# facebookresearch/gtn

Hardware: AMD Instinct MI355X
Metric: CTC forward+backward losses/sec (T=1000, C=256) (higher is better)
Workload: dtype f32; 1 GPU; BASELINE config C3: compose(ctc_target, emissions)+forwardScore CTC loss fwd+bwd, T=1000, C=256, U=100, batch=512 per GPU; global_batch=512, parallelism=dp1 (utterance sharding, all_gather of losses), rccl_ranks=0

## Files before the change

gtn_amd/_capi.py:

```python
import ctypes as C
import os

c_graph = C.c_void_p
c_graph_p = C.POINTER(C.c_void_p)
c_i32_p = C.POINTER(C.c_int)
c_i64_p = C.POINTER(C.c_int64)
c_u8_p = C.POINTER(C.c_uint8)
c_f32_p = C.POINTER(C.c_float)

GRAD_FN = C.CFUNCTYPE(C.c_int, C.c_void_p, c_graph_p, C.c_int, c_graph)
CTX_FREE = C.CFUNCTYPE(None, C.c_void_p)

OK, INVALID_ARGUMENT, LOGIC_ERROR, RUNTIME_ERROR, OUT_OF_RANGE, DEVICE_ERROR = range(6)

_SIGS = {
    "gtnx_set_device": [C.c_int],
    "gtnx_get_device": [c_i32_p],
    "gtnx_set_stream": [C.c_void_p],
    "gtnx_compose_mode": [C.c_int, C.POINTER(C.c_int)],
    "gtnx_synchronize": [],
    "gtnx_memory_stats": [C.POINTER(C.c_uint64), C.POINTER(C.c_uint64)],
    "gtnx_empty_cache": [],
    "gtnx_reclaim": [],
    "gtnx_graph_create": [C.c_int, c_graph_p],
    "gtnx_graph_copy": [c_graph, c_graph_p],
    "gtnx_graph_deep_copy": [c_graph, c_graph_p],
    "gtnx_graph_destroy": [c_graph],
    "gtnx_graph_add_node": [c_graph, C.c_int, C.c_int, c_i32_p],
    "gtnx_graph_add_arc": [c_graph, C.c_int, C.c_int, C.c_int, C.c_int, C.c_float, c_i32_p],
    "gtnx_graph_add_nodes": [c_graph, C.c_int, C.c_void_p, C.c_void_p],
    "gtnx_graph_add_arcs": [c_graph, C.c_int, C.c_void_p, C.c_void_p, C.c_void_p, C.c_void_p, C.c_void_p],
    "gtnx_graph_num_nodes": [c_graph, c_i64_p],
    "gtnx_graph_num_arcs": [c_graph, c_i64_p],
    "gtnx_graph_num_start": [c_graph, c_i64_p],
    "gtnx_graph_num_accept": [c_graph, c_i64_p],
    "gtnx_graph_item": [c_graph, c_f32_p],
    "gtnx_graph_arc_sort": [c_graph, C.c_int],
    "gtnx_graph_mark_arc_sorted": [c_graph, C.c_int],
    "gtnx_graph_ilabel_sorted": [c_graph, c_i32_p],
    "gtnx_graph_olabel_sorted": [c_graph, c_i32_p],
    "gtnx_graph_weights": [c_graph, C.c_int, C.POINTER(c_f32_p)],
    "gtnx_graph_get_weights": [c_graph, C.c_void_p],
    "gtnx_graph_set_weights": [c_graph, C.c_void_p],
    "gtnx_graph_set_weights_device": [c_graph, C.c_void_p],
    "gtnx_graph_weights_device": [c_graph, C.POINTER(C.c_void_p)],
    "gtnx_graph_labels_to_array": [c_graph, C.c_void_p, C.c_int],
    "gtnx_graph_get_start": [c_graph, C.c_void_p],
    "gtnx_graph_get_accept": [c_graph, C.c_void_p],
    "gtnx_graph_is_start": [c_graph, C.c_int, c_i32_p],
    "gtnx_graph_is_accept": [c_graph, C.c_int, c_i32_p],
    "gtnx_graph_make_accept": [c_graph, C.c_int],
    "gtnx_graph_num_out": [c_graph, C.c_int, c_i64_p],
    "gtnx_graph_num_in": [c_graph, C.c_int, c_i64_p],
    "gtnx_graph_get_out": [c_graph, C.c_int, C.c_void_p],
    "gtnx_graph_get_in": [c_graph, C.c_int, C.c_void_p],
    "gtnx_graph_get_arcs": [c_graph, C.c_void_p, C.c_void_p, C.c_void_p, C.c_void_p],
    "gtnx_graph_get_arc": [c_graph, C.c_int, c_i32_p, c_i32_p, c_i32_p, c_i32_p, c_f32_p],
    "gtnx_graph_set_weight": [c_graph, C.c_int, C.c_float],
    "gtnx_graph_calc_grad": [c_graph, c_i32_p],
    "gtnx_graph_set_calc_grad": [c_graph, C.c_int],
    "gtnx_graph_is_grad_available": [c_graph, c_i32_p],
    "gtnx_graph_grad": [c_graph, c_graph_p],
    "gtnx_graph_zero_grad": [c_graph],
    "gtnx_graph_add_grad": [c_graph, C.c_void_p, C.c_int64],
    "gtnx_graph_add_grad_graph": [c_graph, c_graph],
    "gtnx_graph_id": [c_graph, C.POINTER(C.c_size_t)],
    "gtnx_graph_create_op": [c_graph_p, C.c_int, GRAD_FN, C.c_void_p, CTX_FREE, c_graph_p],
    "gtnx_graph_num_inputs": [c_graph, c_i64_p],
    "gtnx_graph_get_input": [c_graph, C.c_int, c_graph_p],
    "gtnx_graph_set_inputs": [c_graph, c_graph_p, C.c_int],
    "gtnx_graph_set_grad_fn": [c_graph, GRAD_FN, C.c_void_p, CTX_FREE],
    "gtnx_graph_has_grad_fn": [c_graph, c_i32_p],
    "gtnx_scalar_graph": [C.c_float, C.c_int, c_graph_p],
    "gtnx_linear_graph": [C.c_int, C.c_int, C.c_int, c_graph_p],
    "gtnx_linear_graph_n": [C.c_int, C.c_int, C.c_int, C.c_int, C.c_void_p, c_graph_p],
    "gtnx_linear_graph_borrow_n": [C.c_int, C.c_int, C.c_int, C.c_int, C.c_void_p, c_graph_p],
    "gtnx_negate": [c_graph, c_graph_p],
    "gtnx_add": [c_graph, c_graph, c_graph_p],
    "gtnx_subtract": [c_graph, c_graph, c_graph_p],
    "gtnx_compose": [c_graph, c_graph, c_graph_p],
    "gtnx_intersect": [c_graph, c_graph, c_graph_p],
    "gtnx_forward_score": [c_graph, c_graph_p],
    "gtnx_viterbi_score": [c_graph, c_graph_p],
    "gtnx_viterbi_path": [c_graph, c_graph_p],
    "gtnx_negate_n": [c_graph_p, C.c_int, c_graph_p],
    "gtnx_add_n": [c_graph_p, C.c_int, c_graph_p, C.c_int, c_graph_p],
    "gtnx_subtract_n": [c_graph_p, C.c_int, c_graph_p, C.c_int, c_graph_p],
    "gtnx_compose_n": [c_graph_p, C.c_int, c_graph_p, C.c_int, c_graph_p],
    "gtnx_intersect_n": [c_graph_p, C.c_int, c_graph_p, C.c_int, c_graph_p],
    "gtnx_forward_score_n": [c_graph_p, C.c_int, c_graph_p],
    "gtnx_viterbi_score_n": [c_graph_p, C.c_int, c_graph_p],
    "gtnx_viterbi_path_n": [c_graph_p, C.c_int, c_graph_p],
    "gtnx_items_n": [c_graph_p, C.c_int, C.c_void_p],
    "gtnx_items_device_n": [c_graph_p, C.c_int, C.c_void_p],
    "gtnx_grads_device_n": [c_graph_p, C.c_int, C.c_void_p, C.c_void_p],
    "gtnx_grads_bind_device_n": [c_graph_p, C.c_int, C.c_void_p, C.c_void_p],
    "gtnx_clone": [c_graph, C.c_int, c_graph_p],
    "gtnx_concat": [c_graph_p, C.c_int, c_graph_p],
    "gtnx_closure": [c_graph, c_graph_p],
    "gtnx_union": [c_graph_p, C.c_int, c_graph_p],
    "gtnx_batch_from_graphs": [c_graph_p, C.c_int, c_graph_p],
    "gtnx_batch_ctc_targets": [C.c_void_p, C.c_void_p, C.c_int, C.c_int, C.c_int, c_graph_p],
    "gtnx_batch_asg_force_align": [C.c_void_p, C.c_void_p, C.c_int, c_graph, C.c_int, c_graph_p],
    "gtnx_batch_linear": [C.c_int, C.c_int, C.c_int, C.c_int, C.c_void_p, C.c_int, c_graph_p],
    "gtnx_batch_linear_rows": [C.c_int, C.c_int, C.c_int, C.c_void_p, C.c_int, C.c_void_p, C.c_int, c_graph_p],
    "gtnx_batch_destroy": [c_graph],
    "gtnx_batch_size": [c_graph, c_i32_p],
    "gtnx_batch_get": [c_graph, C.c_int, c_graph_p],
    "gtnx_batch_negate": [c_graph, c_graph_p],
    "gtnx_batch_add": [c_graph, c_graph, c_graph_p],
    "gtnx_batch_subtract": [c_graph, c_graph, c_graph_p],
    "gtnx_batch_subtract_into": [c_graph, c_graph, C.c_void_p, c_graph_p],
    "gtnx_batch_compose": [c_graph, c_graph, c_graph_p],
    "gtnx_batch_intersect": [c_graph, c_graph, c_graph_p],
    "gtnx_batch_forward_score": [c_graph, c_graph_p],
    "gtnx_batch_viterbi_score": [c_graph, c_graph_p],
    "gtnx_batch_viterbi_path": [c_graph, c_graph_p],
    "gtnx_batch_viterbi_align": [c_graph, C.c_void_p, C.c_void_p, C.c_int64, C.c_void_p, C.c_void_p],
    "gtnx_batch_align_stats": [c_i64_p, c_i64_p],
    "gtnx_batch_viterbi_decode": [c_graph, c_graph, C.c_void_p, C.c_void_p, C.c_int64, C.c_void_p, C.c_void_p,
                                  C.c_void_p],
    "gtnx_batch_decode_stats": [c_i64_p, c_i64_p],
    "gtnx_batch_full_connect_stats": [c_i64_p, c_i64_p],
    "gtnx_batch_linear_decode": [c_graph, C.c_void_p, C.c_int, C.c_void_p, C.c_int64, C.c_void_p, C.c_void_p,
                                 C.c_void_p, C.c_void_p],
    "gtnx_batch_linear_decode_stats": [c_i64_p, c_i64_p],
    "gtnx_batch_ctc_sample": [c_graph, C.c_void_p, C.c_int, C.c_int, C.c_uint64, C.c_float, C.c_void_p, C.c_int64,
                              C.c_void_p, C.c_void_p, C.c_void_p],
    "gtnx_batch_ctc_sample_stats": [c_i64_p, c_i64_p],
    "gtnx_batch_ctc_beam_decode": [c_graph, C.c_void_p, C.c_int, C.c_int, C.c_int, C.c_int, C.c_void_p, C.c_int64,
                                   C.c_void_p, C.c_void_p],
    "gtnx_batch_ctc_beam_decode_lm": [c_graph, C.c_void_p, C.c_int, C.c_int, C.c_int, C.c_int, C.c_void_p, C.c_float,
                                      C.c_float, C.c_void_p, C.c_int64, C.c_void_p, C.c_void_p, C.c_void_p],
    "gtnx_batch_ctc_beam_decode_graph": [c_graph, C.c_void_p, C.c_int, C.c_int, C.c_int, C.c_int, C.c_void_p, C.c_float,
                                         C.c_float, C.c_void_p, C.c_int64, C.c_void_p, C.c_void_p, C.c_void_p],
    "gtnx_lm_graph_create": [c_graph, C.POINTER(C.c_void_p)],
    "gtnx_lm_graph_destroy": [C.c_void_p],
    "gtnx_lm_graph_walk": [C.c_void_p, C.c_int, C.c_int, c_f32_p, c_i32_p],
    "gtnx_lm_graph_info": [C.c_void_p, C.c_void_p],
    "gtnx_batch_ctc_beam_stats": [c_i64_p, c_i64_p],
    "gtnx_batch_linear_shape": [c_graph, c_i32_p, c_i32_p],
    "gtnx_batch_edit_distance": [C.c_void_p, C.c_int64, C.c_void_p, C.c_void_p, C.c_int64, C.c_void_p, C.c_int, C.c_int,
                                 C.c_int, C.c_int, C.c_void_p, C.c_void_p],
    "gtnx_batch_edit_distance_stats": [c_i64_p, c_i64_p],
    "gtnx_batch_ctc_score": [c_graph, C.c_void_p, C.c_int, C.c_void_p, C.c_int64, C.c_void_p, C.c_int, C.c_int, C.c_int,
                             C.c_void_p],
    "gtnx_batch_ctc_score_grad": [c_graph, C.c_void_p, C.c_int, C.c_void_p, C.c_int64, C.c_void_p, C.c_int, C.c_int,
                                  C.c_int, C.c_void_p, C.c_void_p],
    "gtnx_batch_ctc_score_stats": [c_i64_p, c_i64_p],
    "gtnx_batch_ctc_token_align": [c_graph, C.c_void_p, C.c_int, C.c_void_p, C.c_int64, C.c_void_p, C.c_int, C.c_int,
                                   C.c_int, C.c_void_p, C.c_void_p, C.c_void_p, C.c_void_p, C.c_int64, C.c_void_p,
                                   C.c_int64],
    "gtnx_batch_ctc_token_align_stats": [c_i64_p, c_i64_p],
    "gtnx_batch_asg_score": [c_graph, C.c_void_p, C.c_void_p, C.c_void_p, C.c_int64, C.c_void_p, C.c_int, C.c_int,
                             C.c_int, C.c_void_p],
    "gtnx_batch_asg_score_grad": [c_graph, C.c_void_p, C.c_void_p, C.c_void_p, C.c_int64, C.c_void_p, C.c_int, C.c_int,
                                  C.c_int, C.c_void_p, C.c_void_p, C.c_void_p],
    "gtnx_batch_asg_score_stats": [c_i64_p, c_i64_p],
    "gtnx_batch_asg_token_align": [c_graph, C.c_void_p, C.c_void_p, C.c_void_p, C.c_int64, C.c_void_p, C.c_int, C.c_int,
                                   C.c_int, C.c_void_p, C.c_void_p, C.c_void_p, C.c_void_p, C.c_int64, C.c_void_p,
                                   C.c_int64],
    "gtnx_batch_asg_token_align_stats": [c_i64_p, c_i64_p],
    "gtnx_batch_asg_beam_decode": [c_graph, C.c_void_p, C.c_void_p, C.c_int, C.c_int, C.c_int, C.c_void_p, C.c_int64,
                                   C.c_void_p, C.c_void_p],
    "gtnx_batch_asg_beam_decode_graph": [c_graph, C.c_void_p, C.c_void_p, C.c_int, C.c_int, C.c_int, C.c_void_p,
                                         C.c_float, C.c_float, C.c_void_p, C.c_int64, C.c_void_p, C.c_void_p, C.c_void_p],
    "gtnx_batch_asg_beam_stats": [c_i64_p, c_i64_p],
    "gtnx_batch_backward": [c_graph, C.c_int],
    "gtnx_batch_items": [c_graph, C.c_void_p],
    "gtnx_batch_items_device": [c_graph, C.c_void_p],
    "gtnx_batch_grads_bind_device": [c_graph, C.c_void_p, C.c_void_p],
    "gtnx_batch_grads_device": [c_graph, C.c_void_p, C.c_void_p],
    "gtnx_backward": [c_graph, C.c_int],
    "gtnx_backward_with_grad": [c_graph, c_graph, C.c_int],
    "gtnx_backward_n": [c_graph_p, C.c_int, C.c_int],
    "gtnx_equal": [c_graph, c_graph, c_i32_p],
    "gtnx_isomorphic": [c_graph, c_graph, c_i32_p],
    "gtnx_remove": [c_graph, C.c_int, C.c_int, c_graph_p],
    "gtnx_graph_load_buffer": [C.c_void_p, C.c_size_t, c_graph_p],
    "gtnx_parallel_enter": [],
    "gtnx_parallel_leave": [],
    "gtnx_parallel_flush": [],
    "gtnx_prof_enable": [C.c_int],
    "gtnx_prof_reset": [],
    "gtnx_prof_get": [C.c_char_p, C.POINTER(C.c_double), c_i64_p, C.POINTER(C.c_double)],
# ... 54 lines not shown
```

gtn_amd/criteria/criteria_capi.cpp:

```cpp
#include <cstring>
#include <string>

#include <map>
#include <mutex>

#include "asg_criterion.h"
#include "ctc_criterion.h"
#include "edit_distance.h"

#define GTN_EXPORT extern "C" __attribute__((visibility("default")))

namespace {
thread_local std::string g_err;

template <class F>
int guarded(F&& body) {
  try {
    body();
    return 0;
  } catch (const std::exception& e) {
    g_err = e.what();
    return -1;
  }
}
// ... 44 lines not shown
  return guarded([&] {
    gtn::criteria::ctcDecodeBatch(emissions, B, T, C, blank, frames, labels, scores, collapsed, starts, lengths);
  });
}

GTN_EXPORT int gtn_ctc_sample_n(const void* emissions, int B, int T, int C, int blank, const int* frames,
                                int num_samples, unsigned long long seed, float temperature, void* tokens,
                                void* lengths, void* logq, void* labels) {
  return guarded([&] {
    gtn::criteria::ctcSampleBatch(emissions, B, T, C, blank, frames, num_samples, seed, temperature, tokens, lengths,
                                  logq, labels);
  });
}

GTN_EXPORT int gtn_ctc_beam_decode_n(const void* emissions, int B, int T, int C, int blank, const int* frames,
                                     int beam_size, int cutoff_top_n, int nbest, void* tokens, void* lengths,
                                     void* scores) {
  return guarded([&] {
    gtn::criteria::ctcBeamDecodeBatch(emissions, B, T, C, blank, frames, beam_size, cutoff_top_n, nbest, tokens, lengths,
                                      scores);
  });
}

GTN_EXPORT int gtn_ctc_beam_decode_lm_n(const void* emissions, int B, int T, int C, int blank, const int* frames,
                                        int beam_size, int cutoff_top_n, int nbest, const void* lm, float lm_weight,
                                        float insertion_bonus, void* tokens, void* lengths, void* scores,
                                        void* am_scores) {
  return guarded([&] {
    gtn::criteria::ctcBeamDecodeBatch(emissions, B, T, C, blank, frames, beam_size, cutoff_top_n, nbest, lm, lm_weight,
                                      insertion_bonus, tokens, lengths, scores, am_scores);
  });
}

GTN_EXPORT int gtn_ctc_beam_decode_graph_n(const void* emissions, int B, int T, int C, int blank, const int* frames,
                                           int beam_size, int cutoff_top_n, int nbest, void* lm_graph, float lm_weight,
                                           float insertion_bonus, void* tokens, void* lengths, void* scores,
                                           void* am_scores) {
  return guarded([&] {
    gtn::criteria::ctcBeamDecodeBatch(emissions, B, T, C, blank, frames, beam_size, cutoff_top_n, nbest,
                                      static_cast<gtnx_lm_graph_t>(lm_graph), lm_weight, insertion_bonus, tokens, lengths,
                                      scores, am_scores);
  });
}

GTN_EXPORT int gtn_ctc_score_n(const void* emissions, int B, int T, int C, int blank, const int* frames,
                               const void* tokens, const void* lengths, int N, int L, int max_length, void* scores) {
  return guarded([&] {
    if (!scores) throw std::invalid_argument("gtn_ctc_score_n: null scores");
    gtn::criteria::ctcScoreBatch(emissions, B, T, C, blank, frames, tokens, lengths, N, L, max_length, scores);
  });
}

GTN_EXPORT int gtn_ctc_score_grad_n(const void* emissions, int B, int T, int C, int blank, const int* frames,
                                    const void* tokens, const void* lengths, int N, int L, int max_length,
                                    const void* weights, void* grad) {
  return guarded([&] {
    if (!weights || !grad) throw std::invalid_argument("gtn_ctc_score_grad_n: null weights or grad");
    gtn::criteria::ctcScoreBatch(emissions, B, T, C, blank, frames, tokens, lengths, N, L, max_length, nullptr, weights,
                                 grad);
  });
}

GTN_EXPORT int gtn_ctc_token_align_n(const void* emissions, int B, int T, int C, int blank, const int* frames,
                                     const void* tokens, const void* lengths, int N, int L, int max_length,
                                     void* scores, void* starts, void* ends, void* token_scores, void* frame_tokens) {
  return guarded([&] {
    gtn::criteria::ctcTokenAlignBatch(emissions, B, T, C, blank, frames, tokens, lengths, N, L, max_length, scores,
                                      starts, ends, token_scores, frame_tokens);
  });
}

GTN_EXPORT int gtn_edit_distance_n(const void* hyp, const void* hyp_lengths, const void* ref, const void* ref_lengths,
                                   int B, int N, int L, int U, void* dist, void* ops) {
  return guarded([&] { gtn::criteria::editDistanceBatch(hyp, hyp_lengths, ref, ref_lengths, B, N, L, U, dist, ops); });
}

GTN_EXPORT int gtn_ctc_loss_target_grads_n(const void* emissions, const int* targets, const int* lengths, int B, int T,
                                           int C, int blank, void* loss, void* grad, void* target_grad,
                                           const int64_t* target_grad_offsets) {
  return guarded([&] {
    gtn::Batch ctcs;
    gtn::criteria::ctcLossBatch(emissions, targets, lengths, B, T, C, blank, loss, grad, true, nullptr, &ctcs);
    if (target_grad) ctcs.gradsToDevice(target_grad, target_grad_offsets);
  });
}

namespace {
void asg_loss_impl(const void* emissions, const int* targets, const int* lengths, int B, int T, int N, const void* trans_w,
                   const int* frames, void* loss, void* grad_em, void* grad_trans) {
  if (frames)
    for (int b = 0; b < B; ++b)
      if (frames[b] < 1 || frames[b] > T) throw std::invalid_argument("[gtn_asg_loss_frames_n] a frame count outside 1 .. T");
  std::lock_guard<std::mutex> lk(g_loss_transitions.mu);
  gtn::Graph& trans = transitions_for(g_loss_transitions, N, grad_trans != nullptr);
  trans.setCalcGrad(grad_trans != nullptr);
  trans.zeroGrad();
  trans.setWeightsDevice(trans_w);
  gtn::criteria::asgLossBatch(emissions, targets, lengths, B, T, N, trans, loss, grad_em, frames);
  if (grad_trans) {
    gtnx_graph_t h = trans.handle();
    int64_t off = 0;
    gtn::detail::check(gtnx_grads_device_n(&h, 1, grad_trans, &off));
  }
}
}

GTN_EXPORT int gtn_asg_loss_n(const void* emissions, const int* targets, const int* lengths, int B, int T, int N,
                              const void* trans_w, void* loss, void* grad_em, void* grad_trans) {
  return guarded([&] { asg_loss_impl(emissions, targets, lengths, B, T, N, trans_w, nullptr, loss, grad_em, grad_trans); });
}

GTN_EXPORT int gtn_asg_loss_frames_n(const void* emissions, const int* targets, const int* lengths, int B, int T, int N,
                                     const void* trans_w, const int* frames, void* loss, void* grad_em,
                                     void* grad_trans) {
  return guarded([&] {
    if (!frames) throw std::invalid_argument("[gtn_asg_loss_frames_n] null frame counts");
    asg_loss_impl(emissions, targets, lengths, B, T, N, trans_w, frames, loss, grad_em, grad_trans);
  });
}

GTN_EXPORT int gtn_asg_align_n(const void* emissions, const int* targets, const int* lengths, int B, int T, int N,
                               const void* trans_w, const int* frames, void* labels, void* tokens, void* scores) {
  return guarded([&] {
    std::lock_guard<std::mutex> lk(g_nograd_transitions.mu);
    gtn::Graph& trans = transitions_for(g_nograd_transitions, N, false);
    trans.setWeightsDevice(trans_w);
    gtn::criteria::asgAlignBatch(emissions, targets, lengths, B, T, N, trans, frames, labels, tokens, scores);
  });
}

GTN_EXPORT int gtn_asg_decode_n(const void* emissions, int B, int T, int N, const void* trans_w, const int* frames,
                                void* labels, void* scores, void* collapsed, void* lengths) {
  return guarded([&] {
    std::lock_guard<std::mutex> lk(g_nograd_transitions.mu);
    gtn::Graph& trans = transitions_for(g_nograd_transitions, N, false);
    trans.setWeightsDevice(trans_w);
    gtn::criteria::asgDecodeBatch(emissions, B, T, N, trans, frames, labels, scores, collapsed, lengths);
  });
}

GTN_EXPORT int gtn_asg_score_n(const void* emissions, int B, int T, int C, const void* table, const int* frames,
                               const void* tokens, const void* lengths, int N, int L, int max_length, void* scores) {
  return guarded([&] {
    if (!scores) throw std::invalid_argument("gtn_asg_score_n: null scores");
    gtn::criteria::asgScoreBatch(emissions, B, T, C, table, frames, tokens, lengths, N, L, max_length, scores);
  });
}

GTN_EXPORT int gtn_asg_beam_decode_n(const void* emissions, int B, int T, int C, const void* table, const int* frames,
                                     int beam_size, int cutoff_top_n, int nbest, void* tokens, void* lengths,
                                     void* scores) {
  return guarded([&] {
    gtn::criteria::asgBeamDecodeBatch(emissions, B, T, C, table, frames, beam_size, cutoff_top_n, nbest, tokens, lengths,
                                      scores);
  });
}

GTN_EXPORT int gtn_asg_beam_decode_graph_n(const void* emissions, int B, int T, int C, const void* table,
                                           const int* frames, int beam_size, int cutoff_top_n, int nbest, void* lm_graph,
                                           float lm_weight, float insertion_bonus, void* tokens, void* lengths,
                                           void* scores, void* am_scores) {
  return guarded([&] {
    gtn::criteria::asgBeamDecodeBatch(emissions, B, T, C, table, frames, beam_size, cutoff_top_n, nbest,
                                      static_cast<gtnx_lm_graph_t>(lm_graph), lm_weight, insertion_bonus, tokens, lengths,
                                      scores, am_scores);
  });
// ... 21 lines not shown
```

gtn_amd/criteria/ctc_criterion.h:

```cpp
#pragma once

#include <chrono>
#include <cstdint>
#include <stdexcept>
#include <vector>

#include "gtn/gtn.h"

namespace gtn {
namespace criteria {

inline Graph ctcTargetGraph(const std::vector<int>& target, int blank = 0, bool calcGrad = true) {
  const int L = 2 * (int)target.size() + 1;
  std::vector<uint8_t> st(L, 0), ac(L, 0);
  std::vector<int> src, dst, lab;
  src.reserve(3 * L);
  dst.reserve(3 * L);
  lab.reserve(3 * L);
  for (int l = 0; l < L; l++) {
    const int idx = (l - 1) / 2;
    st[l] = l == 0;
    ac[l] = l == L - 1 || l + 2 == L;
    const int label = l % 2 ? target[idx] : blank;
    src.push_back(l), dst.push_back(l), lab.push_back(label);
    if (l > 0) src.push_back(l - 1), dst.push_back(l), lab.push_back(label);
    if (l % 2 && l > 1 && label != target[idx - 1]) src.push_back(l - 2), dst.push_back(l), lab.push_back(label);
  }
  Graph ctc(calcGrad);
  detail::check(gtnx_graph_add_nodes(ctc.handle(), L, st.data(), ac.data()));
  detail::check(gtnx_graph_add_arcs(ctc.handle(), (int)src.size(), src.data(), dst.data(), lab.data(), lab.data(), nullptr));
  ctc.arcSort();
  return ctc;
}

struct CtcStepTimes {
  double build = 0, linear = 0, intersect = 0, forward = 0, backward = 0;
};

inline void ctcLossBatch(
    const void* emissions,
    const int* labels,
    const int* lengths,
    int B,
    int T,
    int C,
    int blank,
    void* lossDev,
    void* gradDev,
    bool targetGrad = true,
    CtcStepTimes* times = nullptr,
    Batch* targetsOut = nullptr,
    const int* frames = nullptr) {
  auto now = [] { return std::chrono::steady_clock::now(); };
  auto ms = [](auto a, auto b) { return std::chrono::duration<double, std::milli>(b - a).count(); };
  if (frames)
    for (int b = 0; b < B; ++b)
      if (frames[b] < 1 || frames[b] > T) throw std::invalid_argument("[ctcLossBatch] a frame count outside 1 .. T");
  auto t0 = now();
  Batch ctcs = Batch::ctcTargets(labels, lengths, B, blank, targetGrad);
  auto t1 = now();
  Batch ems = Batch::linear(B, T, C, emissions, gradDev != nullptr, true, frames);
  std::vector<int64_t> off(B);
  for (int b = 0; b < B; ++b) off[b] = (int64_t)b * T * C;
  if (gradDev) ems.bindGrads(gradDev, off.data());
  auto t2 = now();
  Batch comp = batched::intersect(ctcs, ems);
  auto t3 = now();
  Batch score = batched::forwardScore(comp);
  Batch norm = batched::forwardScore(ems);
  Batch losses = batched::subtract(norm, score, lossDev);
  auto t4 = now();
  if (gradDev) batched::backward(losses);
  auto t5 = now();
  if (times) *times = {ms(t0, t1), ms(t1, t2), ms(t2, t3), ms(t3, t4), ms(t4, t5)};
  losses.itemsToDevice(lossDev);
  if (gradDev) ems.gradsToDevice(gradDev, off.data());
  if (targetsOut) *targetsOut = std::move(ctcs);
}

inline void ctcLossBatch(
    const void* emissions,
    const std::vector<std::vector<int>>& targets,
    int T,
    int C,
    int blank,
    void* lossDev,
    void* gradDev,
    bool targetGrad = true,
    CtcStepTimes* times = nullptr) {
  std::vector<int> flat, len;
  for (auto& t : targets) {
    flat.insert(flat.end(), t.begin(), t.end());
    len.push_back((int)t.size());
  }
  ctcLossBatch(emissions, flat.data(), len.data(), (int)targets.size(), T, C, blank, lossDev, gradDev, targetGrad, times);
}

inline void ctcAlignBatch(
    const void* emissions,
    const int* targets,
    const int* lengths,
    int B,
    int T,
    int C,
    int blank,
    const int* frames,
    void* labels,
    void* tokens,
    void* scores) {
  Batch ctcs = Batch::ctcTargets(targets, lengths, B, blank, false);
  Batch ems = Batch::linear(B, T, C, emissions, false, true);
  Batch comp = batched::intersect(ctcs, ems);
  batched::viterbiAlign(comp, static_cast<int*>(labels), T, static_cast<int*>(tokens), static_cast<float*>(scores), frames);
}

inline void ctcDecodeBatch(
    const void* emissions,
    int B,
    int T,
    int C,
    int blank,
    const int* frames,
    void* labelsDev,
    void* scoresDev,
    void* collapsedDev,
    void* startsDev,
    void* lengthsDev) {
  Batch ems = Batch::linear(B, T, C, emissions, false, true);
  batched::linearDecode(ems, static_cast<int*>(labelsDev), T, static_cast<float*>(scoresDev), frames, blank,
                        static_cast<int*>(collapsedDev), static_cast<int*>(startsDev), static_cast<int*>(lengthsDev));
}

inline void ctcSampleBatch(
    const void* emissions,
    int B,
    int T,
    int C,
    int blank,
    const int* frames,
    int numSamples,
    uint64_t seed,
    float temperature,
    void* tokensDev,
    void* lengthsDev,
    void* logqDev,
    void* labelsDev) {
  Batch ems = Batch::linear(B, T, C, emissions, false, true);
  batched::ctcSample(ems, static_cast<int*>(tokensDev), T, static_cast<int*>(lengthsDev), static_cast<float*>(logqDev),
                     static_cast<int*>(labelsDev), blank, numSamples, seed, temperature, frames);
}

inline void ctcBeamDecodeBatch(
    const void* emissions,
    int B,
    int T,
    int C,
    int blank,
    const int* frames,
    int beamSize,
// ... 116 lines not shown
```

gtn_amd/csrc/band.hip:

```cpp
#include <hip/hip_runtime.h>

#include <algorithm>
#include <cstdlib>
#include <stdexcept>
#include <type_traits>

#include "kernels.h"

#ifdef GTNX_BAND_TIMING
__device__ long long g_band_timing[256];
#endif

namespace gtnx {
namespace {

constexpr float NEGF = -1.0e30f;
constexpr float DEADF = -1.0e29f;
constexpr float LOG2E = 1.44269504088896340736f;
constexpr double LN2 = 0.693147180559945309417;
constexpr int BW = 256;
constexpr int WG = 512;
constexpr int WGB = 768;
constexpr int NBE = 5;
constexpr int NBG = 7;
constexpr int NBGE = 8;
#ifndef GTNX_BWD_SPLIT
#define GTNX_BWD_SPLIT 0
#endif
#ifndef GTNX_FWD_COPY_DEPTH
#define GTNX_FWD_COPY_DEPTH 2
#endif
#ifndef GTNX_FWD_COPY_ROTATE
#define GTNX_FWD_COPY_ROTATE 1
#endif
#ifndef GTNX_FWD_DEPTH
#define GTNX_FWD_DEPTH 2
#endif

#ifdef GTNX_BAND_TIMING
#define GTNX_TM(slot)                 \
  do {                                \
    const long long now_ = clock64(); \
    tm_acc[slot] += now_ - tm_last;   \
    tm_last = now_;                   \
  } while (0)
#define GTNX_TM_INIT(base)                       \
  const int tm_base = base;                      \
  long long tm_acc[8] = {0, 0, 0, 0, 0, 0, 0, 0}; \
  long long tm_n = 0;                            \
  long long tm_last = clock64()
#define GTNX_TM_TICK() tm_n += 1
#define GTNX_TM_DUMP()                                                      \
  do {                                                                      \
    if (blockIdx.x == 0 && (threadIdx.x & 63) == 0) {                       \
      for (int i_ = 0; i_ < 7; ++i_) g_band_timing[tm_base + (threadIdx.x >> 6) * 7 + i_] += tm_acc[i_]; \
      if (threadIdx.x == 0) g_band_timing[tm_base + 127] += tm_n;           \
    }                                                                       \
  } while (0)
#else
#define GTNX_TM(slot) do { } while (0)
#define GTNX_TM_INIT(base) do { } while (0)
#define GTNX_TM_TICK() do { } while (0)
#define GTNX_TM_DUMP() do { } while (0)
#endif

__device__ __forceinline__ void lds_barrier() { asm volatile("s_waitcnt lgkmcnt(0)\n\ts_barrier" ::: "memory"); }
#ifdef GTNX_EXP_FAKE_MATH
__device__ __forceinline__ float ex2(float x) { return __builtin_fmaf(x, 0.001f, 1.0f); }
__device__ __forceinline__ float lg2(float x) { return __builtin_fmaf(x, 0.001f, -0.001f); }
#else
__device__ __forceinline__ float ex2(float x) { return __builtin_amdgcn_exp2f(x); }
__device__ __forceinline__ float lg2(float x) { return __builtin_amdgcn_logf(x); }
#endif

__device__ __forceinline__ void settle(float& x) { asm volatile("" : "+v"(x)); }
__device__ __forceinline__ void settle(int& x) { asm volatile("" : "+v"(x)); }
__device__ __forceinline__ float uniform(float x) {
  return __int_as_float(__builtin_amdgcn_readfirstlane(__float_as_int(x)));
}
__device__ __forceinline__ double uniform(double x) {
  const long long b = __double_as_longlong(x);
  const unsigned lo = __builtin_amdgcn_readfirstlane(unsigned(b)), hi = __builtin_amdgcn_readfirstlane(unsigned(b >> 32));
  return __longlong_as_double((long long)(((unsigned long long)hi << 32) | lo));
}

__device__ __forceinline__ float wave_shr1(float x, float fill) {
  return __int_as_float(__builtin_amdgcn_update_dpp(__float_as_int(fill), __float_as_int(x), 0x138, 0xf, 0xf, false));
}
__device__ __forceinline__ float wave_shl1(float x, float fill) {
  return __int_as_float(__builtin_amdgcn_update_dpp(__float_as_int(fill), __float_as_int(x), 0x130, 0xf, 0xf, false));
}
#define GTNX_DPP6(op)                                                         \
  "s_nop 1\n\t" op " %0, %0, %0 row_shr:1 row_mask:0xf bank_mask:0xf\n\t"     \
  "s_nop 1\n\t" op " %0, %0, %0 row_shr:2 row_mask:0xf bank_mask:0xf\n\t"     \
  "s_nop 1\n\t" op " %0, %0, %0 row_shr:4 row_mask:0xf bank_mask:0xf\n\t"     \
  "s_nop 1\n\t" op " %0, %0, %0 row_shr:8 row_mask:0xf bank_mask:0xf\n\t"     \
  "s_nop 1\n\t" op " %0, %0, %0 row_bcast:15 row_mask:0xa bank_mask:0xf\n\t"  \
  "s_nop 1\n\t" op " %0, %0, %0 row_bcast:31 row_mask:0xc bank_mask:0xf\n\t"  \
  "s_nop 1"
__device__ __forceinline__ float wave_max(float x) {
  asm volatile(GTNX_DPP6("v_max_f32_dpp") : "+v"(x));
  return __int_as_float(__builtin_amdgcn_readlane(__float_as_int(x), 63));
}
__device__ __forceinline__ float wave_sum63(float x) {
  asm volatile(GTNX_DPP6("v_add_f32_dpp") : "+v"(x));
  return x;
}
__device__ __forceinline__ float wave_sum(float x) {
  return __int_as_float(__builtin_amdgcn_readlane(__float_as_int(wave_sum63(x)), 63));
}
#define GTNX_DPP2(ctl)                                                  \
  "v_add_f32_dpp %0, %0, %0 " ctl "\n\tv_add_f32_dpp %1, %1, %1 " ctl "\n\ts_nop 0\n\t"
__device__ __forceinline__ void wave_sum63x2(float& a, float& b) {
  asm volatile("s_nop 1\n\t"
               GTNX_DPP2("row_shr:1 row_mask:0xf bank_mask:0xf")
               GTNX_DPP2("row_shr:2 row_mask:0xf bank_mask:0xf")
               GTNX_DPP2("row_shr:4 row_mask:0xf bank_mask:0xf")
               GTNX_DPP2("row_shr:8 row_mask:0xf bank_mask:0xf")
               GTNX_DPP2("row_bcast:15 row_mask:0xa bank_mask:0xf")
               GTNX_DPP2("row_bcast:31 row_mask:0xc bank_mask:0xf")
               : "+v"(a), "+v"(b));
}
__device__ __forceinline__ void row_sum15x2(float& a, float& b) {
  asm volatile("s_nop 1\n\t"
               GTNX_DPP2("row_shr:1 row_mask:0xf bank_mask:0xf")
               GTNX_DPP2("row_shr:2 row_mask:0xf bank_mask:0xf")
               GTNX_DPP2("row_shr:4 row_mask:0xf bank_mask:0xf")
               GTNX_DPP2("row_shr:8 row_mask:0xf bank_mask:0xf")
               : "+v"(a), "+v"(b));
}
#define GTNX_ROR4(op)                                                        \
  "s_nop 1\n\t" op " %0, %0, %0 row_ror:8 row_mask:0xf bank_mask:0xf\n\t"    \
  "s_nop 1\n\t" op " %0, %0, %0 row_ror:4 row_mask:0xf bank_mask:0xf\n\t"    \
  "s_nop 1\n\t" op " %0, %0, %0 row_ror:2 row_mask:0xf bank_mask:0xf\n\t"    \
  "s_nop 1\n\t" op " %0, %0, %0 row_ror:1 row_mask:0xf bank_mask:0xf\n\t"    \
  "s_nop 1"
__device__ __forceinline__ float row16_max(float x) {
  asm volatile(GTNX_ROR4("v_max_f32_dpp") : "+v"(x));
  return x;
}
__device__ __forceinline__ float row16_sum(float x) {
  asm volatile(GTNX_ROR4("v_add_f32_dpp") : "+v"(x));
  return x;
}
__device__ __forceinline__ float lse3(float x0, float x1, float x2) {
  const float mx = fmaxf(fmaxf(x0, x1), x2);
  const float md = __builtin_amdgcn_fmed3f(x0, x1, x2);
  const float mn = fminf(fminf(x0, x1), x2);
  return mx + lg2(1.0f + ex2(md - mx) + ex2(mn - mx));
}

template <int NPL>
struct NodeRegs {
  int lab[NPL];
  float wi[3][NPL];
  float wo[3][NPL];
  int ao[3][NPL];
  bool has_in[NPL];
  bool start[NPL], accept[NPL];
};
template <int NPL, bool WANT_OUT>
__device__ __forceinline__ void load_nodes(const BandPair& P, int m0, NodeRegs<NPL>& g) {
  const GTNX_G gtnx_i4* nodes = reinterpret_cast<const GTNX_G gtnx_i4*>(P.nodes);
#pragma unroll
  for (int j = 0; j < NPL; ++j) {
    const int m = m0 + j;
    g.lab[j] = 0;
    g.start[j] = g.accept[j] = g.has_in[j] = false;
#pragma unroll
    for (int k = 0; k < 3; ++k) {
      g.wi[k][j] = g.wo[k][j] = NEGF;
      g.ao[k][j] = -1;
    }
    if (m < P.N) {
      const gtnx_i4 q = nodes[m];
      g.lab[j] = q.x >= 0 ? q.x : 0;
      const uint8_t f = P.nflags[m];
      g.start[j] = (f & NF_START) != 0;
      g.accept[j] = (f & NF_ACCEPT) != 0;
      const int a[3] = {q.y, q.z, q.w};
#pragma unroll
      for (int k = 0; k < 3; ++k)
        if (a[k] >= 0) {
          g.has_in[j] = true;
          g.wi[k][j] = P.w ? fmaxf(P.w[a[k]] * LOG2E, NEGF) : 0.0f;
        }
    }
    if (WANT_OUT) {
#pragma unroll
      for (int k = 0; k < 3; ++k) {
        if (m + k < P.N) {
          const gtnx_i4 q = nodes[m + k];
          const int a = k == 0 ? q.y : (k == 1 ? q.z : q.w);
          if (a >= 0) {
            g.ao[k][j] = a;
            g.wo[k][j] = P.w ? fmaxf(P.w[a] * LOG2E, NEGF) : 0.0f;
          }
        }
      }
    }
  }
}

__device__ __forceinline__ float em2(float x) { return fmaxf(x * LOG2E, NEGF); }

__device__ __forceinline__ int row_of(int e, int W, float invW) {
  int r = int(float(e) * invW);
  if (r * W > e) --r;
  if ((r + 1) * W <= e) ++r;
  return r;
}

template <int NS, int LN = BW>
struct Stage {
  float v[NS];
  template <bool VEC>
  __device__ __forceinline__ void issue(const GTNX_G float* src, int cnt, int tid) {
    if (cnt <= 0) return;
#pragma unroll
    for (int i = 0; i < NS / 4; ++i) {
      if (i > 0 && 4 * i * LN >= cnt) break;
      const int e = min(4 * (i * LN + tid), cnt - 4);
      const gtnx_f4 q = *reinterpret_cast<const GTNX_G gtnx_f4*>(reinterpret_cast<const GTNX_G char*>(src) + unsigned(4 * e));
      v[4 * i] = q.x;
      v[4 * i + 1] = q.y;
      v[4 * i + 2] = q.z;
      v[4 * i + 3] = q.w;
    }
  }
  int off[NS / 4];
  __device__ __forceinline__ void init_offsets(int W, int stride, int K, int tid, bool reverse = true) {
    const float invW = 1.0f / float(W);
#pragma unroll
    for (int i = 0; i < NS / 4; ++i) {
      const int e = 4 * (i * LN + tid);
      const int r = row_of(min(e, 4096), W, invW);
      off[i] = (reverse ? K - 1 - r : r) * stride + (e - r * W);
    }
  }
  template <class F>
  __device__ __forceinline__ void each_vec(int cnt, int shift, int tid, F&& f) const {
#pragma unroll
    for (int i = 0; i < NS / 4; ++i) {
      if (i > 0 && 4 * i * LN >= cnt) break;
      if (4 * (i * LN + tid) < cnt) f(i, off[i] - shift, gtnx_f4{v[4 * i], v[4 * i + 1], v[4 * i + 2], v[4 * i + 3]});
    }
  }
  __device__ __forceinline__ void settle_all() {
#pragma unroll
    for (int i = 0; i < NS; ++i) asm volatile("" : "+v"(v[i]));
  }
  template <bool VEC, class F>
  __device__ __forceinline__ void each(int cnt, int W, int tid, F&& f) const {
    const float invW = 1.0f / float(W);
    if constexpr (VEC) {
#pragma unroll
      for (int i = 0; i < NS / 4; ++i) {
        if (i > 0 && 4 * i * LN >= cnt) break;
        const int e = 4 * (i * LN + tid);
        if (e < cnt) {
          const int r = row_of(e, W, invW);
          f(i, e, r, e - r * W, gtnx_f4{v[4 * i], v[4 * i + 1], v[4 * i + 2], v[4 * i + 3]});
        }
      }
    } else {
#pragma unroll
      for (int i = 0; i < NS / 4; ++i) {
        if (i > 0 && 4 * i * LN >= cnt) break;
        if (4 * (i * LN + tid) < cnt) {
          const int e = min(4 * (i * LN + tid), cnt - 4);
          const int r0 = row_of(e, W, invW), c0 = e - r0 * W;
#pragma unroll
          for (int k = 0; k < 4; ++k) {
            int r = r0, col = c0 + k;
            if (col >= W) {
              col -= W;
              ++r;
            }
            f(i, e + k, r, col, gtnx_f4{v[4 * i + k], 0.0f, 0.0f, 0.0f});
          }
        }
      }
    }
  }
};

struct BandLds {
  int CS;
  int o_ering, o_aring, o_oring, o_snode, o_misc, total;
};
__host__ __device__ inline BandLds band_lds(int C, int K, int NSmax, bool backward) {
  BandLds L;
  L.CS = C + 4;
  int o = 0;
  L.o_ering = o;
  o += (backward ? NBGE : NBE) * K * L.CS;
  o = (o + 3) & ~3;
  L.o_aring = o;
  o += backward ? NBE * K * NSmax : 0;
  o = (o + 3) & ~3;
  L.o_oring = o;
  o += backward ? max(NBG * K * NSmax, 2 * C) : 0;
  o = (o + 3) & ~3;
  L.o_snode = o;
  o += backward ? 512 : 0;
  L.o_misc = o;
  o += 160 + 32 + 8 + 2 * NBE * K * 4 + 40 * K + 8 + 512;
  L.total = o;
  return L;
}
struct BandMisc {
  double *offr, *red, *find, *aofr;
  float *bndr, *fin, *lsep;
};
template <int K>
__device__ __forceinline__ BandMisc band_misc(float* lds, const BandLds& L) {
  BandMisc m;
  m.offr = reinterpret_cast<double*>(lds + L.o_misc);
  m.red = m.offr + 80;
  m.find = m.red + 16;
  m.aofr = m.find + 4;
  m.bndr = lds + L.o_misc + 200 + 2 * NBE * K * 4;
  m.fin = m.bndr + 40 * K;
  m.lsep = m.fin + 8;
  return m;
}

__device__ __forceinline__ float wave_max_of(const float* v, int n) {
  float mx = v[0];
  for (int j = 1; j < n; ++j) mx = fmaxf(mx, v[j]);
  return wave_max(mx);
}

template <int NPL, bool UNIT, int K, bool VEC>
__global__ __launch_bounds__(WG) void band_forward_kernel(const BandPair* __restrict__ pairs, int NSmax) {
#define GTNX_BAND_PAIR pairs[blockIdx.x]
#include "band_forward_body.inc"
#undef GTNX_BAND_PAIR
}
template <int NPL, bool UNIT, int K, bool VEC>
__global__ __launch_bounds__(WG) void band_forward_one_kernel(BandPair one, int NSmax) {
#define GTNX_BAND_PAIR one
#include "band_forward_body.inc"
#undef GTNX_BAND_PAIR
}

__device__ __forceinline__ BandPair band_patched(BandPair P, const BandPatch& pt) {
  if (pt.on) {
    const int b = P.bidx;
    P.delta = pt.delta + b;
    P.delta_norm = pt.delta_norm ? pt.delta_norm + b : nullptr;
    P.rowlse = pt.rowlse ? pt.rowlse + int64_t(b) * pt.M : nullptr;
    P.norm = nullptr;
    P.em_copy = nullptr;
    P.grad_em = pt.grad_em ? pt.grad_em + int64_t(b) * pt.A : nullptr;
    P.grad_fixed = pt.grad_fixed ? pt.grad_fixed + P.goff : nullptr;
  }
  return P;
}
template <int NPL, bool UNIT, bool GRADG, int K, bool VEC, bool BIG>
__global__ __launch_bounds__(WGB, BIG ? 3 : 6) void band_backward_kernel(const BandPair* __restrict__ pairs, int NSmax, BandPatch patch) {
#define GTNX_BAND_PAIR band_patched(pairs[blockIdx.x], patch)
#include "band_backward_body.inc"
#undef GTNX_BAND_PAIR
}
template <int NPL, bool UNIT, bool GRADG, int K, bool VEC, bool BIG>
__global__ __launch_bounds__(WGB, BIG ? 3 : 6) void band_backward_one_kernel(BandPair one, int NSmax) {
#define GTNX_BAND_PAIR one
#include "band_backward_body.inc"
#undef GTNX_BAND_PAIR
}


__global__ __launch_bounds__(512) void ctc_targets_kernel(const CtcTargetArgs* __restrict__ args, int blank) {
  const CtcTargetArgs a = args[blockIdx.x];
  __shared__ __attribute__((aligned(16))) int tl[256 + 4];
  __shared__ __attribute__((aligned(16))) int tk[256 + 4];
  const int N = a.N, U = (N - 1) >> 1, m = threadIdx.x;
  if (m < 260) {
    const int v = m < U ? a.labels[m] : 0x7fffffff;
    tl[m] = v;
    tk[m] = (m > 0 && m < U && v != a.labels[m - 1]) ? 1 : 0;
  }
  __syncthreads();
  if (m >= N) return;
  const bool odd = (m & 1) != 0;
  const int my = odd ? tl[(m - 1) >> 1] : blank;
  const int skip = odd ? tk[(m - 1) >> 1] : 0;
  const int mi = (m - 1) >> 1;
  const int before = odd ? mi : (m >> 1);
  int rank = 0, skips = 0;
  for (int o = 0; o < U; o += 4) {
    const gtnx_i4 l4 = *reinterpret_cast<const gtnx_i4*>(tl + o), k4 = *reinterpret_cast<const gtnx_i4*>(tk + o);
    const int lo[4] = {l4.x, l4.y, l4.z, l4.w}, ko[4] = {k4.x, k4.y, k4.z, k4.w};
#pragma unroll
    for (int k = 0; k < 4; ++k) {
      const bool front = o + k < before;
      rank += (lo[k] < my || (lo[k] == my && front)) ? 1 : 0;
      skips += front ? ko[k] : 0;
    }
  }
  rank += blank < my ? U + 1 : (blank == my ? (m + 1) >> 1 : 0);
  const int base = (m > 0 ? 2 * m - 1 : 0) + skips;
  GTNX_G BandNode* nd = const_cast<GTNX_G BandNode*>(a.nodes);
  nd[m].lab = my;
  nd[m].aid[0] = base;
  nd[m].aid[1] = m > 0 ? base + 1 : -1;
  nd[m].aid[2] = skip ? base + 2 : -1;
  a.nflags[m] = uint8_t((m == 0 ? NF_START : 0) | (m + 2 >= N ? NF_ACCEPT : 0));
  a.snode[rank] = m;
  a.slab[rank] = my;
  if (m == N - 1 && a.n_arcs) a.n_arcs[0] = base + 1 + (m > 0 ? 1 : 0) + skip;
}

__global__ __launch_bounds__(512) void band_viterbi_kernel(const BandDecode* __restrict__ pairs) {
  const BandDecode P = pairs[blockIdx.x];
  const int T = P.T, C = P.C, N = P.N, NS = P.NS;
  extern __shared__ float lds[];
  const float NINF = -__builtin_inff();
  float* a0 = lds;
  float* a1 = lds + 516;
  float* stage = lds + 1032;
  const int m = threadIdx.x;
  const GTNX_G gtnx_i4* nodes = reinterpret_cast<const GTNX_G gtnx_i4*>(P.nodes);
  int lab = 0;
  float wi[3] = {NINF, NINF, NINF};
  bool accept = false, start = false;
  if (m < N) {
    const gtnx_i4 q = nodes[m];
    lab = q.x >= 0 ? q.x : 0;
    const int a[3] = {q.y, q.z, q.w};
#pragma unroll
    for (int k = 0; k < 3; ++k)
      if (a[k] >= 0) wi[k] = P.w ? P.w[a[k]] : 0.0f;
    const uint8_t f = P.nflags[m];
    start = (f & NF_START) != 0;
    accept = (f & NF_ACCEPT) != 0;
  }
  if (m < 2) a0[m] = a1[m] = NINF;
  a0[2 + m] = start ? 0.0f : NINF;
  a1[2 + m] = NINF;
  int tie = 0;
  const int R = max(1, min(64, P.stage_floats / C));
  float* cur = a0;
  float* nxt = a1;
  __syncthreads();
  for (int t0 = 0; t0 < T; t0 += R) {
    const int rows = min(R, T - t0);
    for (int e = threadIdx.x; e < rows * C; e += blockDim.x) stage[e] = P.em[int64_t(t0) * C + e];
    __syncthreads();
    for (int i = 0; i < rows; ++i) {
      const float e = stage[i * C + lab];
      const float c0 = cur[2 + m] + (wi[0] + e), c1 = cur[1 + m] + (wi[1] + e), c2 = cur[m] + (wi[2] + e);
      float best = c0;
      int k = 0;
      if (c1 > best) best = c1, k = 1;
      if (c2 > best) best = c2, k = 2;
      if (best > NINF && ((k != 0 && c0 == best) || (k != 1 && c1 == best) || (k != 2 && c2 == best))) tie = 1;
      if (m < NS) P.bp[int64_t(t0 + i) * NS + m] = uint8_t(best > NINF ? k : 3);
      nxt[2 + m] = m < N ? best : NINF;
      __syncthreads();
      float* sw = cur;
      cur = nxt;
      nxt = sw;
    }
  }
  __shared__ float red_v[8];
  __shared__ int red_m[8], s_best, s_tie;
  float v = accept ? cur[2 + m] : NINF;
  int bm = (m < N && accept && v > NINF) ? m : 1 << 30;
  const float wmx = wave_max(v);
  if (!(v == wmx)) bm = 1 << 30;
  int cnt = (bm != (1 << 30)) ? 1 : 0;
  for (int o = 32; o > 0; o >>= 1) {
    bm = min(bm, __shfl_xor(bm, o));
    cnt += __shfl_xor(cnt, o);
  }
  if ((threadIdx.x & 63) == 0) {
    red_v[threadIdx.x >> 6] = wmx;
    red_m[threadIdx.x >> 6] = bm;
  }
  if (cnt > 1) tie = 1;
  if (threadIdx.x == 0) s_tie = 0;
  __syncthreads();
  if (threadIdx.x == 0) {
    float bv = NINF;
    int bn = -1;
    for (int w = 0; w < 8; ++w) {
      if (red_m[w] == (1 << 30)) continue;
      if (red_v[w] > bv) bv = red_v[w], bn = red_m[w];
      else if (red_v[w] == bv && bv > NINF) s_tie = 1;
    }
    s_best = bn;
    P.score[0] = bv;
  }
// ... 505 lines not shown
```

gtn_amd/csrc/band_backward_body.inc:

```
  constexpr int RNk = K >= 4 ? 4 : K;
  constexpr int NP = K / RNk;
  const BandPair P = GTNX_BAND_PAIR;
  const int T = P.T, C = P.C, NS = P.NS;
  extern __shared__ float lds[];
  const BandLds L = band_lds(C, K, NSmax, true);
  float* ering = lds + L.o_ering;
  float* aring = lds + L.o_aring;
  float* oring = lds + L.o_oring;
  int* snode = reinterpret_cast<int*>(lds + L.o_snode);
  const BandMisc M = band_misc<K>(lds, L);
  float* lser = M.lsep;
  const int CS = L.CS;
  const int wv = __builtin_amdgcn_readfirstlane(threadIdx.x >> 6);
  const bool sweeper = wv < 4;
  const int l = threadIdx.x & 63;
  const int nblocks = (T + K - 1) / K;
  const int nticks = nblocks + 5;
  const GTNX_G double* ao = P.aoff;
  const double z2 = uniform(ao[0]);
  const bool dead = !(z2 > double(DEADF));
  const float ds = uniform(P.delta[0]);
  const bool want_em = P.grad_em != nullptr;
  GTNX_TM_INIT(128);
  constexpr bool SPLIT = !BIG && K >= 2 && GTNX_BWD_SPLIT;
// ... 28 lines not shown
  auto rowsum_do = [&](const RowSumRegs& R, int c, int cg , int r, auto steady_tag) -> float {
    constexpr bool STEADY = decltype(steady_tag)::value;
    if (!want_em || (K < 4 && r >= K)) return 0.0f;
    if constexpr (!STEADY) {
      if (r >= rows_of_k(c)) return 0.0f;
    }
    const bool dead_r = STEADY ? false : dead;
    const float* ob = oring + (cg * K + r) * NSmax;
    gtnx_f4 v[NPL];
#pragma unroll
    for (int q = 0; q < NPL; ++q) v[q] = *reinterpret_cast<const gtnx_f4*>(ob + min(256 * q + 4 * l, NSmax - 4));
    const float em_hot = ering[(ge_of(c) * K + r) * CS + max(P.hot, 0)];
    const float ls_hot = lser[cg * K + r];
    float all = (v[0].x * R.in[0] + v[0].y * R.in[0]) + (v[0].z * R.in[0] + v[0].w * R.in[0]);
    float hotp = (v[0].x * R.hot[0].x + v[0].y * R.hot[0].y) + (v[0].z * R.hot[0].z + v[0].w * R.hot[0].w);
#pragma unroll
    for (int q = 1; q < NPL; ++q) {
      all += (v[q].x * R.in[q] + v[q].y * R.in[q]) + (v[q].z * R.in[q] + v[q].w * R.in[q]);
      hotp += (v[q].x * R.hot[q].x + v[q].y * R.hot[q].y) + (v[q].z * R.hot[q].z + v[q].w * R.hot[q].w);
    }
    if (dead_r) all = hotp = 0.0f;
    wave_sum63x2(all, hotp);
    all = __int_as_float(__builtin_amdgcn_readlane(__float_as_int(all), 63));
    const bool have = all != 0.0f && !dead_r;
    const float f = have ? ds * __builtin_amdgcn_rcpf(all) : 1.0f;
    if (l == 63 && P.hot >= 0) {
      const float sm = dn_k * ex2(em_hot - ls_hot);
      P.grad_em[int64_t(T - 1 - c * K - r) * C + P.hot] = (dead_r ? 0.0f : hotp * f) + sm;
    }
    if (l == 0) rnorm_k[cg * K + r] = f;
    return have ? f : 0.0f;
  };
#ifndef GTNX_BWD_ROWSUM4
#define GTNX_BWD_ROWSUM4 1
#endif
  constexpr bool RS4 = !BIG && !SPLIT && K == 4 && NPL == 1 && GTNX_BWD_ROWSUM4;
  struct RowSum4Regs {
    float in;
    gtnx_f4 hot[4];
    int po;
    int eo, go;
  };
  auto rowsum4_init = [&](RowSum4Regs& R) {
    const int r = l >> 4, nb = 16 * (l & 15);
    R.in = nb < NSmax ? 1.0f : 0.0f;
    R.po = r * NSmax + min(nb, NSmax - 16);
#pragma unroll
    for (int k = 0; k < 4; ++k) {
      float hm[4];
#pragma unroll
      for (int e = 0; e < 4; ++e) {
        const int m = nb + 4 * k + e;
        int lab = -1;
        if (m < P.N) lab = P.nodes[m].lab;
        settle(lab);
        hm[e] = (P.hot >= 0 && lab == P.hot) ? 1.0f : 0.0f;
      }
      R.hot[k] = gtnx_f4{hm[0], hm[1], hm[2], hm[3]};
    }
    R.eo = r * CS + max(P.hot, 0);
    R.go = (K - 1 - r) * C + max(P.hot, 0);
  };
  auto rowsum4_do = [&](const RowSum4Regs& R, int c, int cg , auto steady_tag) {
    constexpr bool STEADY = decltype(steady_tag)::value;
    const int rows = STEADY ? K : rows_of_k(c);
    if (!want_em || rows <= 0) return;
    const bool dead_r = STEADY ? false : dead;
    typedef float f2v __attribute__((ext_vector_type(2)));
    const float* ob = oring + cg * K * NSmax + R.po;
    gtnx_f4 v[4];
#pragma unroll
    for (int k = 0; k < 4; ++k) v[k] = *reinterpret_cast<const gtnx_f4*>(ob + 4 * k);
    const float em_hot = ering[ge_of(c) * K * CS + R.eo];
    const float ls_hot = lser[cg * K + (l >> 4)];
    f2v a2 = f2v{v[0].x, v[0].y} + f2v{v[0].z, v[0].w};
    f2v h2 = f2v{v[0].x, v[0].y} * f2v{R.hot[0].x, R.hot[0].y};
    h2 = __builtin_elementwise_fma(f2v{v[0].z, v[0].w}, f2v{R.hot[0].z, R.hot[0].w}, h2);
#pragma unroll
    for (int k = 1; k < 4; ++k) {
      a2 += f2v{v[k].x, v[k].y} + f2v{v[k].z, v[k].w};
      h2 = __builtin_elementwise_fma(f2v{v[k].x, v[k].y}, f2v{R.hot[k].x, R.hot[k].y}, h2);
      h2 = __builtin_elementwise_fma(f2v{v[k].z, v[k].w}, f2v{R.hot[k].z, R.hot[k].w}, h2);
    }
    float all = (a2.x + a2.y) * R.in, hotp = h2.x + h2.y;
    if (dead_r) all = hotp = 0.0f;
    row_sum15x2(all, hotp);
    const bool have = all != 0.0f && !dead_r;
    const float f = have ? ds * __builtin_amdgcn_rcpf(all) : 1.0f;
    if ((l & 15) == 15 && (STEADY || (l >> 4) < rows)) {
      if (P.hot >= 0) {
        const float sm = dn_k * ex2(em_hot - ls_hot);
        const GTNX_G char* gb = reinterpret_cast<const GTNX_G char*>(P.grad_em + int64_t(T - c * K - K) * C);
        *reinterpret_cast<GTNX_G float*>(const_cast<GTNX_G char*>(gb) + unsigned(4 * R.go)) = (dead_r ? 0.0f : hotp * f) + sm;
      }
      rnorm_k[cg * K + (l >> 4)] = f;
    }
  };
  constexpr int NCS = 8 / K;
  struct DrainRegs {
    int s[NCS], e[NCS], n0[NCS], n1[NCS];
    float m0[NCS], m1[NCS];
    bool more_any;
  };
  auto drain_init = [&](DrainRegs& D, int hid) {
    const int* cls = reinterpret_cast<const int*>(oring);
#pragma unroll
    for (int q = 0; q < NCS; ++q) {
      const int cc = hid + q * BW;
      D.s[q] = D.e[q] = 0;
      if (cc < C && cc != P.hot) {
        D.s[q] = cls[cc];
        D.e[q] = cls[C + cc];
      }
      const int cnt = D.e[q] - D.s[q];
      D.n0[q] = cnt > 0 ? snode[D.s[q]] : 0;
      D.n1[q] = cnt > 1 ? snode[D.s[q] + 1] : 0;
      D.m0[q] = cnt > 0 ? 1.0f : 0.0f;
      D.m1[q] = cnt > 1 ? 1.0f : 0.0f;
    }
    D.more_any = false;
#pragma unroll
    for (int q = 0; q < NCS; ++q) D.more_any = D.more_any || __builtin_amdgcn_ballot_w64(D.e[q] - D.s[q] > 2) != 0;
  };
  auto drain_rows = [&](const DrainRegs& D, int hid, int c, int cg , auto full_tag, auto dead_tag, auto r0_tag, auto r1_tag) {
    constexpr bool FULL = decltype(full_tag)::value;
    constexpr bool DEADU = decltype(dead_tag)::value;
    constexpr int R0 = decltype(r0_tag)::value, R1 = decltype(r1_tag)::value;
    const int rows = FULL ? K : rows_of_k(c);
    const float* ob = oring + cg * K * NSmax;
    const float* eb = ering + ge_of(c) * K * CS;
    const float* lb = lser + cg * K;
    const float* fb = rnorm_k + cg * K;
    GTNX_G float* dst = P.grad_em + int64_t(T - 1 - c * K) * C;
#pragma unroll
    for (int q = 0; q < NCS; ++q) {
      if (q > 0 && q * BW >= C) break;
      const int cc = hid + q * BW;
      const bool mine = cc < C && cc != P.hot;
      float p0[K], p1[K], e[K], ls[K], f[K];
#pragma unroll
      for (int r = R0; r < R1; ++r) {
        if constexpr (!DEADU) {
          p0[r] = ob[r * NSmax + D.n0[q]];
          p1[r] = ob[r * NSmax + D.n1[q]];
        }
        e[r] = eb[r * CS + min(cc, C - 1)];
      }
      if constexpr (K == 4) {
        const gtnx_f4 l4 = *reinterpret_cast<const gtnx_f4*>(lb), f4 = *reinterpret_cast<const gtnx_f4*>(fb);
        ls[0] = l4.x, ls[1] = l4.y, ls[2] = l4.z, ls[3] = l4.w;
        f[0] = f4.x, f[1] = f4.y, f[2] = f4.z, f[3] = f4.w;
      } else {
#pragma unroll
        for (int r = R0; r < R1; ++r) {
          ls[r] = lb[r];
          f[r] = fb[r];
        }
      }
      float sum[K];
      if constexpr (!DEADU) {
#pragma unroll
      for (int r = R0; r < R1; ++r) sum[r] = p0[r] * D.m0[q] + p1[r] * D.m1[q];
      }
      if (!DEADU && D.more_any) {
        for (int i = D.s[q] + 2; i < D.e[q]; ++i) {
          const float* o = ob + snode[i];
#pragma unroll
// ... 509 lines not shown
```

gtn_amd/csrc/band_forward_body.inc:

```
#ifndef GTNX_FWD_SHIFT_ROWS
#define GTNX_FWD_SHIFT_ROWS 4
#endif
  constexpr int RNk = K >= GTNX_FWD_SHIFT_ROWS ? GTNX_FWD_SHIFT_ROWS : (K >= 4 ? 4 : K);
  constexpr int NP = K / RNk;
  constexpr int D = 8 / K > GTNX_FWD_DEPTH ? 8 / K : GTNX_FWD_DEPTH;
  const BandPair P = GTNX_BAND_PAIR;
  const int T = P.T, C = P.C, NS = P.NS;
  extern __shared__ float lds[];
  const BandLds L = band_lds(C, K, NSmax, false);
  float* ering = lds + L.o_ering;
  const BandMisc M = band_misc<K>(lds, L);
  const int CS = L.CS;
  const int wv = __builtin_amdgcn_readfirstlane(threadIdx.x >> 6);
  const bool sweeper = wv < 4;
  const int l = threadIdx.x & 63;
  const int nblocks = (T + K - 1) / K;
  const int nticks = nblocks + 3;
  GTNX_TM_INIT(0);

  if (sweeper) {
    __builtin_amdgcn_s_setprio(1);
    const int w = wv;
    const int m0 = threadIdx.x * NPL;
    NodeRegs<NPL> g;
// ... 87 lines not shown
              if (UNIT) {
                x0 = a[j];
                x1 = s1;
                x2 = s2 + g.wi[2][j];
              } else {
                x0 = a[j] + g.wi[0][j];
                x1 = s1 + g.wi[1][j];
                x2 = s2 + g.wi[2][j];
              }
              nw[j] = lse3(x0, x1, x2) + ev[i][j];
            }
            if ((i + 1) % RNk == 0) {
              const float mx = wave_max_of(nw, NPL);
              if (mx > DEADF) {
#pragma unroll
                for (int j = 0; j < NPL; ++j) nw[j] -= mx;
                off += double(mx);
              } else if (w > 0) {
                off = offp[(i + 1) / RNk];
              }
              if (l == 0) {
                const int p = (t0 + i + 1) / RNk;
                off_own[p & 15] = off;
                P.aoff[1 + p * 4 + w] = off;
              }
            }
#pragma unroll
            for (int j = 0; j < NPL; ++j) hist[i][j] = a[j] = nw[j];
          }
        }
        {
          const GTNX_G char* const brow = arow;
          arow += int64_t(NS) * 4 * rows;
#ifdef GTNX_EXP_NO_ALPHA_STORE
          if (writer && beta < 0) {
#else
          if (writer) {
#endif
#pragma unroll
            for (int i = 0; i < K; ++i)
              if (FULL || i < rows) {
                const GTNX_G char* ri = brow + int64_t(NS) * 4 * (i + 1);
#pragma unroll
                for (int j = 0; j < NPL; ++j) *reinterpret_cast<GTNX_G float*>(const_cast<GTNX_G char*>(ri) + (aoffb + 4u * j)) = hist[i][j];
              }
          }
        }
        if (NPL == 1 ? l >= 62 : l == 63) {
#pragma unroll
          for (int i = 0; i < K; ++i)
            if (FULL || i < rows) {
              float* bp = bnd_own + ((((beta & 3) * K + i + 1) & (4 * K - 1))) * 2;
              if (NPL == 1) {
                bp[63 - l] = hist[i][0];
              } else {
                bp[0] = hist[i][NPL - 1];
                bp[1] = hist[i][0];
              }
            }
        }
      };
      if (beta >= 0 && beta < nblocks) {
        if (beta * K + K <= T) block(std::true_type{});
        else block(std::false_type{});
      }
      GTNX_TM(5);
      lds_barrier();
      GTNX_TM(6);
      GTNX_TM_TICK();
    }
    float f = NEGF;
#pragma unroll
    for (int j = 0; j < NPL; ++j) f = fmaxf(f, g.accept[j] ? a[j] : NEGF);
    const float mx = wave_max(f);
    float s = 0.0f;
#pragma unroll
    for (int j = 0; j < NPL; ++j) s += g.accept[j] ? ex2(a[j] - mx) : 0.0f;
    s = wave_sum(s);
    if (l == 0) {
      M.fin[2 * w] = mx;
      M.fin[2 * w + 1] = s;
      M.find[w] = off;
    }
  } else {
    const int hid = threadIdx.x - BW;
    constexpr bool vec = VEC;
    const bool want_lse = P.norm != nullptr || P.rowlse != nullptr;
    Stage<8> st[D];
    auto rows_of = [&](int c) { return c < nblocks ? min(K, T - c * K) : 0; };
    auto issue = [&](Stage<8>& s, int c) { s.template issue<VEC>(P.em + int64_t(c) * K * C, rows_of(c) * C, hid); };
    GTNX_G float* const em_copy = P.em_copy;
    auto land = [&](const Stage<8>& s, int c, int c5 , auto copy_tag) {
      constexpr bool COPY = decltype(copy_tag)::value;
      float* base = ering + c5 * K * CS;
      GTNX_G float* cdst = em_copy + int64_t(c) * K * C;
      s.template each<VEC>(rows_of(c) * C, C, hid, [&](int, int e, int r, int col, gtnx_f4 q) {
        float* d = base + r * CS + col;
        if (vec) *reinterpret_cast<gtnx_f4*>(d) = gtnx_f4{em2(q.x), em2(q.y), em2(q.z), em2(q.w)};
        else d[0] = em2(q.x);
        if (COPY) {
          if (vec) __builtin_nontemporal_store(q, reinterpret_cast<GTNX_G gtnx_f4*>(cdst + e));
          else __builtin_nontemporal_store(q.x, cdst + e);
        }
      });
    };
    constexpr int LPR = BW / K, G16 = LPR / 16;
    const int EPL = (C + LPR - 1) / LPR;
    double normacc = 0.0;
    auto lse_a_n = [&](int c, int c5 , auto nconst) {
      constexpr int NE = decltype(nconst)::value;
      const int rows = rows_of(c), rr = hid / LPR, sub = hid - rr * LPR;
      if (rows <= 0) return;
      const float* e = ering + (c5 * K + min(rr, rows - 1)) * CS + sub * EPL;
      float x[NE];
      float m = NEGF;
      if (VEC && (EPL & 3) == 0) {
#pragma unroll
        for (int i = 0; i < NE; i += 4) {
          const bool in = i < EPL && sub * EPL + i < C;
          const gtnx_f4 q = in ? *reinterpret_cast<const gtnx_f4*>(e + i) : gtnx_f4{NEGF, NEGF, NEGF, NEGF};
          x[i] = q.x, x[i + 1] = q.y, x[i + 2] = q.z, x[i + 3] = q.w;
          m = fmaxf(fmaxf(m, fmaxf(q.x, q.y)), fmaxf(q.z, q.w));
        }
      } else {
#pragma unroll
        for (int i = 0; i < NE; ++i) {
          x[i] = (i < EPL && sub * EPL + i < C) ? e[i] : NEGF;
          m = fmaxf(m, x[i]);
        }
      }
      m = row16_max(m);
      float sum = 0.0f;
#pragma unroll
      for (int i = 0; i < NE; ++i) sum += (i < EPL) ? ex2(x[i] - m) : 0.0f;
      sum = row16_sum(sum);
      if ((hid & 15) == 0 && rr < rows) {
        float* p = M.lsep + (c & 1) * 256 + (rr * 8 + (sub >> 4)) * 2;
        p[0] = m;
        p[1] = sum;
      }
    };
    auto lse_a = [&](int c, int c5) {
      if (EPL <= 4) lse_a_n(c, c5, std::integral_constant<int, 4>{});
      else if (EPL <= 8) lse_a_n(c, c5, std::integral_constant<int, 8>{});
      else lse_a_n(c, c5, std::integral_constant<int, 16>{});
    };
    auto lse_b = [&](int c) {
      const int rows = rows_of(c);
      if (hid < rows) {
        const float* p = M.lsep + (c & 1) * 256 + hid * 16;
        float Mx = p[0];
#pragma unroll
        for (int k = 1; k < G16; ++k) Mx = fmaxf(Mx, p[2 * k]);
        float S = 0.0f;
#pragma unroll
        for (int k = 0; k < G16; ++k) S += p[2 * k + 1] * ex2(p[2 * k] - Mx);
        const float l2 = Mx + lg2(S);
        if (P.rowlse) P.rowlse[c * K + hid] = l2;
        normacc += double(l2);
      }
    };
    auto run = [&](auto copy_tag) {
      issue(st[0], 0);
      land(st[0], 0, 0, copy_tag);
#pragma unroll
      for (int c = 1; c <= D; ++c) issue(st[c % D], c);
// ... 87 lines not shown
```

gtn_amd/csrc/batch.cpp:

```cpp
#include "batch.h"

#include <algorithm>
#include <atomic>
#include <cstdlib>
#include <cstring>
#include <limits>
#include <unordered_map>
#include <unordered_set>

namespace gtnx {

namespace {

std::atomic<uint64_t> g_batch_seq{1};

struct CompMode {
  int old;
  CompMode() : old(compose_mode_hint(2)) {}
  ~CompMode() { compose_mode_hint(old); }
};

BatchP make_batch(Batch::Kind k, int n, bool cg) {
  auto b = std::make_shared<Batch>();
  b->kind = k;
// ... 362 lines not shown
  std::vector<uint8_t> st(size_t(L), 0), ac(size_t(L), 0);
  std::vector<int> src, dst, lab;
  src.reserve(size_t(3 * L));
  dst.reserve(size_t(3 * L));
  lab.reserve(size_t(3 * L));
  for (int l = 0; l < L; ++l) {
    const int idx = (l - 1) / 2;
    st[size_t(l)] = l == 0;
    ac[size_t(l)] = l == L - 1 || l + 2 == L;
    const int label = l % 2 ? t[idx] : blank;
    src.push_back(l), dst.push_back(l), lab.push_back(label);
    if (l > 0) src.push_back(l - 1), dst.push_back(l), lab.push_back(label);
    if (l % 2 && l > 1 && label != t[idx - 1]) src.push_back(l - 2), dst.push_back(l), lab.push_back(label);
  }
  Graph g(cg);
  g.add_nodes(L, st.data(), ac.data());
  g.add_arcs(int(src.size()), src.data(), dst.data(), lab.data(), lab.data(), nullptr);
  g.arc_sort(false);
  return g;
}
}

BatchP batch_ctc_targets(const int* labels, const int* lengths, int n, int blank, bool calc_grad) {
  GTNX_HOST_T("batch.ctc_targets");
  if (n < 0) throw_invalid("[gtnx_batch_ctc_targets] negative batch size");
  BatchP b = make_batch(Batch::CTC_TARGETS, n, calc_grad);
  b->blank = blank;
  b->lab_off.resize(size_t(n) + 1);
  b->lab_off[0] = 0;
  for (int i = 0; i < n; ++i) {
    if (lengths[i] < 0) throw_invalid("[gtnx_batch_ctc_targets] negative length");
    b->lab_off[size_t(i) + 1] = b->lab_off[size_t(i)] + lengths[i];
    b->max_nodes = std::max(b->max_nodes, 2 * lengths[i] + 1);
  }
  const size_t total = size_t(b->lab_off[size_t(n)]);
  b->labels.assign(labels, labels + total);
  int mn = blank;
  b->max_label = blank;
  for (size_t i = 0; i < total; ++i) {
    b->max_label = std::max(b->max_label, labels[i]);
    mn = std::min(mn, labels[i]);
  }
  if (mn < 0 || b->max_nodes > band_max_nodes() || n == 0) {
    std::vector<Graph> gs;
    gs.reserve(size_t(n));
    for (int i = 0; i < n; ++i)
      gs.push_back(ctc_target_graph_host(labels + b->lab_off[size_t(i)], lengths[i], blank, calc_grad));
    return batch_from_graphs(std::move(gs));
  }
  Runtime& rt = Runtime::get();
  const size_t lab_bytes = align_up(sizeof(int) * (total ? total : 1), 256);
  const size_t arg_bytes = align_up(sizeof(CtcTargetArgs) * size_t(n), 256);
  size_t bytes = lab_bytes + arg_bytes;
  b->rec_off.resize(size_t(n));
  for (int i = 0; i < n; ++i) {
    const size_t N = size_t(2 * lengths[i] + 1);
    b->rec_off[size_t(i)] = bytes;
    bytes += align_up(sizeof(BandNode) * N, 64) + align_up(N, 64) + 2 * align_up(4 * N, 64) + 64;
  }
  b->rec_mem = rt.alloc(bytes);
  PinnedMemP pin = rt.alloc_pinned(lab_bytes + arg_bytes);
  std::memcpy(pin->ptr, labels, sizeof(int) * total);
  CtcTargetArgs* args = reinterpret_cast<CtcTargetArgs*>(static_cast<char*>(pin->ptr) + lab_bytes);
  for (int i = 0; i < n; ++i) {
    const size_t N = size_t(2 * lengths[i] + 1);
    char* base = b->rec_mem->as<char>(b->rec_off[size_t(i)]);
    CtcTargetArgs& a = args[size_t(i)];
    a.labels = b->rec_mem->as<int>() + b->lab_off[size_t(i)];
    a.nodes = reinterpret_cast<BandNode*>(base);
    base += align_up(sizeof(BandNode) * N, 64);
    a.nflags = reinterpret_cast<uint8_t*>(base);
    base += align_up(N, 64);
    a.snode = reinterpret_cast<int*>(base);
    base += align_up(4 * N, 64);
    a.slab = reinterpret_cast<int*>(base);
    base += align_up(4 * N, 64);
    a.n_arcs = reinterpret_cast<int*>(base);
    a.N = int(N);
    a.pad = 0;
  }
  rt.h2d_pinned(b->rec_mem->ptr, pin->ptr, lab_bytes + arg_bytes);
  launch_ctc_targets(reinterpret_cast<const CtcTargetArgs*>(b->rec_mem->as<char>(lab_bytes)), n, blank, rt.stream());
  return b;
}


BatchP batch_asg_force_align(const int* labels, const int* lengths, int n, Graph& transitions, int n_labels) {
  if (n < 0) throw_invalid("[gtnx_batch_asg_force_align] negative batch size");
  if (transitions.num_nodes() != int64_t(n_labels) + 1 || transitions.num_arcs() != int64_t(n_labels) * (n_labels + 1))
    throw_invalid("[gtnx_batch_asg_force_align] the transitions graph must have the asgTransitions(N) layout");
  BatchP b = make_batch(Batch::CTC_TARGETS, n, transitions.calc_grad());
  b->fal = true;
  b->trans = transitions;
  b->trans_labels = n_labels;
  b->lab_off.resize(size_t(n) + 1);
  b->lab_off[0] = 0;
  int max_u = 0;
  for (int i = 0; i < n; ++i) {
    if (lengths[i] < 0) throw_invalid("[gtnx_batch_asg_force_align] negative length");
    b->lab_off[size_t(i) + 1] = b->lab_off[size_t(i)] + lengths[i];
    max_u = std::max(max_u, lengths[i]);
  }
  b->max_nodes = max_u + 1;
  const size_t total = size_t(b->lab_off[size_t(n)]);
  b->labels.assign(labels, labels + total);
  int mn = 0;
  for (size_t i = 0; i < total; ++i) {
    b->max_label = std::max(b->max_label, labels[i]);
    mn = std::min(mn, labels[i]);
  }
  if (mn < 0 || b->max_label >= n_labels || b->max_nodes > band_max_nodes() || n == 0) {
    b->kind = Batch::GRAPHS;
    batch_materialise(*b);
    return b;
  }
  Runtime& rt = Runtime::get();
  std::vector<Weights*> ws{transitions.w.get()};
  ensure_weights_device_batch(ws);
  size_t bytes = align_up(sizeof(int) * (total ? total : 1), 256);
  b->rec_off.resize(size_t(n));
  b->w_off.resize(size_t(n));
  b->map_off.resize(size_t(n));
  for (int i = 0; i < n; ++i) {
    const size_t N = size_t(lengths[i]) + 1, A = 2 * size_t(lengths[i]);
    b->rec_off[size_t(i)] = bytes;
    bytes += align_up(sizeof(BandNode) * N, 64) + align_up(N, 64) + 2 * align_up(4 * N, 64);
    b->w_off[size_t(i)] = bytes;
    bytes += align_up(4 * (A ? A : 1), 64);
    b->map_off[size_t(i)] = bytes;
    bytes += align_up(4 * (A ? A : 1), 64);
  }
  b->rec_mem = rt.alloc(bytes);
  {
    PinnedMemP pin = rt.alloc_pinned(sizeof(int) * (total ? total : 1));
    std::memcpy(pin->ptr, labels, sizeof(int) * total);
    rt.h2d_pinned(b->rec_mem->ptr, pin->ptr, sizeof(int) * total);
  }
  std::vector<AsgFalArgs> args;
  args.resize(size_t(n));
  for (int i = 0; i < n; ++i) {
    const size_t N = size_t(lengths[i]) + 1;
    char* base = b->rec_mem->as<char>(b->rec_off[size_t(i)]);
    AsgFalArgs& a = args[size_t(i)];
    a.labels = b->rec_mem->as<int>() + b->lab_off[size_t(i)];
    a.trans_w = transitions.w->dev;
    a.nodes = reinterpret_cast<BandNode*>(base);
    base += align_up(sizeof(BandNode) * N, 64);
    a.nflags = reinterpret_cast<uint8_t*>(base);
    base += align_up(N, 64);
    a.snode = reinterpret_cast<int*>(base);
    base += align_up(4 * N, 64);
    a.slab = reinterpret_cast<int*>(base);
    a.w = b->rec_mem->as<float>(b->w_off[size_t(i)]);
    a.arc_map = b->rec_mem->as<int>(b->map_off[size_t(i)]);
    a.U = lengths[i];
    a.pad = 0;
  }
  DevMemP d = upload_vec(args);
  launch_asg_fal_targets(d->as<AsgFalArgs>(), n, n_labels, rt.stream());
  auto op = std::make_shared<BFalOp>();
  op->seq = g_batch_seq.fetch_add(1);
  b->op = op;
  return b;
}

BatchP batch_linear(int n, int M, int C, bool calc_grad, const void* dev, bool borrow, const int* rows) {
// ... 782 lines not shown
```

gtn_amd/csrc/batch.h:

```cpp
#pragma once

#include <memory>
#include <vector>

#include "ops.h"

namespace gtnx {

struct Batch;
using BatchP = std::shared_ptr<Batch>;

struct BatchOp {
  uint64_t seq = 0;
  std::vector<BatchP> inputs;
  virtual void backward(Batch& out) = 0;
  virtual ~BatchOp() {}
};

struct Batch {
  enum Kind { GRAPHS, CTC_TARGETS, LINEAR, PRODUCT, SCALAR };
  Kind kind = GRAPHS;
  int n = 0;
  bool calc_grad = false;

  bool materialised = false;
  std::vector<Graph> graphs;
  bool leaf = false;
  struct Origin {
    std::shared_ptr<void> home;
    size_t begin, end;
  };
  std::vector<Origin> origins;
  void (*give_back)(const std::shared_ptr<void>& home, std::vector<Graph>* part) = nullptr;
  std::vector<float> host_vals;
  bool host_vals_valid = false;
  PinnedMemP host_pin;
  void* host_ev = nullptr;

  std::vector<int> labels, lab_off;
  int blank = 0;
  int max_label = -1, max_nodes = 0;
  DevMemP rec_mem;
  std::vector<size_t> rec_off;
  bool fal = false;
  Graph trans;
  int trans_labels = 0;
  std::vector<size_t> w_off, map_off;
  int M = 0, C = 0;
  DevMemP w_mem;
  float* w_dev = nullptr;
  std::shared_ptr<PendingCopy> w_pend;
  DevMemP nc_mem;
  float* nc_norm = nullptr;
  float* nc_rowlse = nullptr;
  std::vector<int> rows;
  int64_t pad_floats = 0;
  DevMemP pad_mem;
  int rows_of(int b) const { return rows.empty() ? M : rows[size_t(b)]; }
  BatchP fixed, chain;
  bool chain_first = false, intersect = false;
  bool wide = false;
  bool full = false;
  DevMemP v_mem;
  float* v_dev = nullptr;

  std::shared_ptr<BatchOp> op;
  bool tape_cleared = false;
  DevMemP g_mem;
  float* g_dev = nullptr;
  std::vector<int64_t> g_off;
  DevMemP dest_mem;
  float* dest = nullptr;

  int64_t elem_size(int b) const;
  ~Batch();
};

BatchP batch_from_graphs(std::vector<Graph> gs);
BatchP batch_ctc_targets(const int* labels, const int* lengths, int n, int blank, bool calc_grad);
BatchP batch_asg_force_align(const int* labels, const int* lengths, int n, Graph& transitions, int n_labels);
BatchP batch_linear(int n, int M, int C, bool calc_grad, const void* dev, bool borrow, const int* rows = nullptr);
BatchP batch_compose(const BatchP& a, const BatchP& b, bool intersect);
BatchP batch_shortest_distance(const BatchP& x, bool tropical);
void batch_full_connect_stats(int64_t* fast, int64_t* fallback);
BatchP batch_viterbi_path(const BatchP& x);
void batch_viterbi_align(const BatchP& x, const int* frames, int* labels_dev, int64_t row_stride, int* tokens_dev,
                         float* scores_dev);
void batch_align_stats(int64_t* fast, int64_t* fallback);
void batch_viterbi_decode(const BatchP& ems, Graph& transitions, const int* frames, int* labels_dev, int64_t row_stride,
                          float* scores_dev, int* collapsed_dev, int* lengths_dev);
void batch_decode_stats(int64_t* fast, int64_t* fallback);
void batch_linear_decode(const BatchP& ems, const int* frames, int blank, int* labels_dev, int64_t row_stride,
                         float* scores_dev, int* collapsed_dev, int* starts_dev, int* lengths_dev);
void batch_linear_decode_stats(int64_t* fast, int64_t* fallback);
void batch_ctc_sample(const BatchP& ems, const int* frames, int blank, int N, uint64_t seed, float temperature,
                      int* tokens_dev, int64_t row_stride, int* lengths_dev, float* logq_dev, int* labels_dev);
void batch_ctc_sample_stats(int64_t* calls, int64_t* utterances);
void batch_ctc_beam_decode(const BatchP& ems, const int* frames, int blank, int beam, int topn, int nbest,
                           int* tokens_dev, int64_t row_stride, int* lengths_dev, float* scores_dev);
struct CtcBeamLm {
  const float* table_dev;
  float weight, bonus;
  float* am_scores_dev;
  const void* graph = nullptr;
};
void batch_ctc_beam_decode(const BatchP& ems, const int* frames, int blank, int beam, int topn, int nbest,
                           const CtcBeamLm* lm, int* tokens_dev, int64_t row_stride, int* lengths_dev, float* scores_dev);
void batch_ctc_beam_stats(int64_t* calls, int64_t* utterances);
void batch_asg_beam_decode(const BatchP& ems, const int* frames, const float* table_dev, int beam, int topn, int nbest,
                           int* tokens_dev, int64_t row_stride, int* lengths_dev, float* scores_dev);
struct AsgBeamLm {
  const void* graph;
  float weight, bonus;
  float* am_scores_dev;
};
void batch_asg_beam_decode(const BatchP& ems, const int* frames, const float* table_dev, int beam, int topn, int nbest,
                           const AsgBeamLm* lm, int* tokens_dev, int64_t row_stride, int* lengths_dev,
                           float* scores_dev);
void batch_asg_beam_stats(int64_t* calls, int64_t* utterances);
void batch_edit_distance(const int* hyp_dev, int64_t hyp_stride, const int* hyp_len_dev, const int* ref_dev,
                         int64_t ref_stride, const int* ref_len_dev, int B, int N, int L, int U, int* dist_dev,
                         int* ops_dev);
void batch_edit_distance_stats(int64_t* calls, int64_t* pairs);
void batch_ctc_score(const BatchP& ems, const int* frames, int blank, const int* tokens_dev, int64_t row_stride,
                     const int* lengths_dev, int N, int L, int max_length, float* scores_dev);
void batch_ctc_score_grad(const BatchP& ems, const int* frames, int blank, const int* tokens_dev, int64_t row_stride,
                          const int* lengths_dev, int N, int L, int max_length, const float* weights_dev,
                          float* grad_dev);
void batch_ctc_score_stats(int64_t* calls, int64_t* pairs);
void batch_ctc_token_align(const BatchP& ems, const int* frames, int blank, const int* tokens_dev, int64_t row_stride,
                           const int* lengths_dev, int N, int L, int max_length, float* scores_dev, int* starts_dev,
                           int* ends_dev, float* token_scores_dev, int64_t out_stride, int* frame_tokens_dev,
                           int64_t frame_stride);
void batch_ctc_token_align_stats(int64_t* calls, int64_t* pairs);
void batch_asg_score(const BatchP& ems, const int* frames, const float* table_dev, const int* tokens_dev,
                     int64_t row_stride, const int* lengths_dev, int N, int L, int max_length, float* scores_dev);
void batch_asg_score_grad(const BatchP& ems, const int* frames, const float* table_dev, const int* tokens_dev,
                          int64_t row_stride, const int* lengths_dev, int N, int L, int max_length,
                          const float* weights_dev, float* grad_em_dev, float* grad_table_dev);
void batch_asg_score_stats(int64_t* calls, int64_t* pairs);
void batch_asg_token_align(const BatchP& ems, const int* frames, const float* table_dev, const int* tokens_dev,
                           int64_t row_stride, const int* lengths_dev, int N, int L, int max_length, float* scores_dev,
                           int* starts_dev, int* ends_dev, float* token_scores_dev, int64_t out_stride,
                           int* frame_tokens_dev, int64_t frame_stride);
void batch_asg_token_align_stats(int64_t* calls, int64_t* pairs);
BatchP batch_scalar(ScalarKind k, const BatchP& a, const BatchP& b, void* items_dev = nullptr);
void batch_backward(const BatchP& root, bool retain);
void batch_items_host(const BatchP& x, float* out);
void batch_items_device(const BatchP& x, void* dev_out);
void batch_grads_device(const BatchP& x, void* dev_out, const int64_t* offsets);
void batch_grads_bind(const BatchP& x, void* dev_out, const int64_t* offsets);
Graph batch_get(const BatchP& x, int i);
float batch_item_host(const BatchP& x, int i);
void batch_prefetch_items(const BatchP& x);
BatchP batch_ctc_targets_from_graphs(const std::vector<Graph>& gs);
BatchP batch_linear_from_graphs(const std::vector<Graph>& gs);
void batch_materialise(Batch& x);

}
```

gtn_amd/csrc/capi.cpp:

```cpp
#include <atomic>
#include <chrono>
#include <condition_variable>
#include <cstdlib>
#include <cstring>
#include <mutex>
#include <string>
#include <vector>

#include "batch.h"
#include "lm_graph.h"
#include "ops.h"
#include "ops_internal.h"
#include "region.h"

#define GTNX_API extern "C" __attribute__((visibility("default")))

using namespace gtnx;

namespace {
thread_local std::string g_err;

gtnx_status_t fail(gtnx_status_t s, const std::string& m) {
  g_err = m;
  return s;
// ... 663 lines not shown
BINARY_FN(gtnx_intersect, op_compose(va, vb, true), RO_INTERSECT)
UNARY_FN(gtnx_forward_score, op_shortest_distance(v, false), true, RO_FS)
UNARY_FN(gtnx_viterbi_score, op_shortest_distance(v, true), true, RO_VS)
UNARY_FN(gtnx_viterbi_path, op_viterbi_path(v), true, RO_VP)

GTNX_API gtnx_status_t gtnx_items_n(const gtnx_graph_t* g, int n, float* out) {
  return guard([&] {
    bool all = n > 0;
    for (int i = 0; i < n && all; ++i) {
      Graph& raw = RAW(g[i]);
      all = raw.s->pending && region_item(raw, out + i);
    }
    if (all) return;
    auto v = vec(g, n);
    items_host(v, out);
  });
}
GTNX_API gtnx_status_t gtnx_items_device_n(const gtnx_graph_t* g, int n, void* out) {
  return guard([&] {
    std::vector<Graph*> hs(static_cast<size_t>(n > 0 ? n : 0));
    for (int i = 0; i < n; ++i) hs[size_t(i)] = &RAW(g[i]);
    if (region_items_device(hs.data(), n, out)) return;
    auto v = vec(g, n);
    items_device(v, out);
  });
}
GTNX_API gtnx_status_t gtnx_grads_device_n(const gtnx_graph_t* g, int n, void* out, const int64_t* offsets) {
  return guard([&] {
    auto v = vec(g, n);
    grads_device(v, out, offsets);
  });
}
GTNX_API gtnx_status_t gtnx_grads_bind_device_n(const gtnx_graph_t* g, int n, void* out, const int64_t* offsets) {
  return guard([&] {
    auto v = vec(g, n);
    grads_bind_device(v, out, offsets);
  });
}

GTNX_API gtnx_status_t gtnx_clone(gtnx_graph_t g, int projection, gtnx_graph_t* out) {
  return guard([&] {
    if (projection < 0 || projection > 2) throw_invalid("[gtnx_clone] projection must be 0, 1 or 2");
    std::vector<Graph> v{G(g)};
    *out = H(op_rational(RAT_CLONE, v, projection));
  });
}
GTNX_API gtnx_status_t gtnx_concat(const gtnx_graph_t* g, int n, gtnx_graph_t* out) {
  return guard([&] {
    auto v = vec(g, n);
    *out = H(op_rational(RAT_CONCAT, v, 0));
  });
}
GTNX_API gtnx_status_t gtnx_closure(gtnx_graph_t g, gtnx_graph_t* out) {
  return guard([&] {
    std::vector<Graph> v{G(g)};
    *out = H(op_rational(RAT_CLOSURE, v, 0));
  });
}
GTNX_API gtnx_status_t gtnx_union(const gtnx_graph_t* g, int n, gtnx_graph_t* out) {
  return guard([&] {
    auto v = vec(g, n);
    *out = H(op_rational(RAT_UNION, v, 0));
  });
}

GTNX_API gtnx_status_t gtnx_remove(gtnx_graph_t g, int ilabel, int olabel, gtnx_graph_t* out) {
  return guard([&] { *out = H(op_remove(G(g), ilabel, olabel)); });
}

namespace {
inline BatchP& BH(gtnx_batch_t h) {
  if (!h) throw_invalid("null batch handle");
  return *reinterpret_cast<BatchP*>(h);
}
inline gtnx_batch_t HB(BatchP b) { return reinterpret_cast<gtnx_batch_t>(new BatchP(std::move(b))); }
}
GTNX_API gtnx_status_t gtnx_batch_from_graphs(const gtnx_graph_t* g, int n, gtnx_batch_t* out) {
  return guard([&] { *out = HB(batch_from_graphs(vec(g, n, true))); });
}
GTNX_API gtnx_status_t gtnx_batch_ctc_targets(const int* labels, const int* lengths, int n, int blank, int cg,
                                              gtnx_batch_t* out) {
  return guard([&] { *out = HB(batch_ctc_targets(labels, lengths, n, blank, cg != 0)); });
}
GTNX_API gtnx_status_t gtnx_batch_asg_force_align(const int* labels, const int* lengths, int n, gtnx_graph_t transitions,
                                                  int n_labels, gtnx_batch_t* out) {
  return guard([&] { *out = HB(batch_asg_force_align(labels, lengths, n, G(transitions), n_labels)); });
}
GTNX_API gtnx_status_t gtnx_batch_linear(int n, int M, int N, int cg, const void* dev, int borrow, gtnx_batch_t* out) {
  return guard([&] { *out = HB(batch_linear(n, M, N, cg != 0, dev, borrow != 0)); });
}
GTNX_API gtnx_status_t gtnx_batch_linear_rows(int n, int M, int N, const int* rows, int cg, const void* dev, int borrow,
                                             gtnx_batch_t* out) {
  return guard([&] { *out = HB(batch_linear(n, M, N, cg != 0, dev, borrow != 0, rows)); });
}
GTNX_API gtnx_status_t gtnx_batch_destroy(gtnx_batch_t b) {
  return guard([&] {
    auto* p = reinterpret_cast<BatchP*>(b);
    if (!p) return;
    if (Runtime::initialized())
      Runtime::get().defer_delete(p, [](void* q) { delete static_cast<BatchP*>(q); },
                                  (*p && (*p)->materialised) ? size_t((*p)->n > 0 ? (*p)->n : 1) : 1);
    else
      delete p;
  });
}
GTNX_API gtnx_status_t gtnx_batch_size(gtnx_batch_t b, int* out) {
  return guard([&] { *out = BH(b)->n; });
}
GTNX_API gtnx_status_t gtnx_batch_get(gtnx_batch_t b, int i, gtnx_graph_t* out) {
  return guard([&] { *out = H(batch_get(BH(b), i)); });
}
GTNX_API gtnx_status_t gtnx_batch_negate(gtnx_batch_t a, gtnx_batch_t* out) {
  return guard([&] { *out = HB(batch_scalar(SK_NEGATE, BH(a), nullptr)); });
}
GTNX_API gtnx_status_t gtnx_batch_add(gtnx_batch_t a, gtnx_batch_t b, gtnx_batch_t* out) {
  return guard([&] { *out = HB(batch_scalar(SK_ADD, BH(a), BH(b))); });
}
GTNX_API gtnx_status_t gtnx_batch_subtract(gtnx_batch_t a, gtnx_batch_t b, gtnx_batch_t* out) {
  return guard([&] { *out = HB(batch_scalar(SK_SUBTRACT, BH(a), BH(b))); });
}
GTNX_API gtnx_status_t gtnx_batch_subtract_into(gtnx_batch_t a, gtnx_batch_t b, void* items_device, gtnx_batch_t* out) {
  return guard([&] { *out = HB(batch_scalar(SK_SUBTRACT, BH(a), BH(b), items_device)); });
}
GTNX_API gtnx_status_t gtnx_batch_compose(gtnx_batch_t a, gtnx_batch_t b, gtnx_batch_t* out) {
  return guard([&] { *out = HB(batch_compose(BH(a), BH(b), false)); });
}
GTNX_API gtnx_status_t gtnx_batch_intersect(gtnx_batch_t a, gtnx_batch_t b, gtnx_batch_t* out) {
  return guard([&] { *out = HB(batch_compose(BH(a), BH(b), true)); });
}
GTNX_API gtnx_status_t gtnx_batch_forward_score(gtnx_batch_t a, gtnx_batch_t* out) {
  return guard([&] { *out = HB(batch_shortest_distance(BH(a), false)); });
}
GTNX_API gtnx_status_t gtnx_batch_viterbi_score(gtnx_batch_t a, gtnx_batch_t* out) {
  return guard([&] { *out = HB(batch_shortest_distance(BH(a), true)); });
}
GTNX_API gtnx_status_t gtnx_batch_full_connect_stats(int64_t* fast, int64_t* fallback) {
  return guard([&] { batch_full_connect_stats(fast, fallback); });
}
GTNX_API gtnx_status_t gtnx_batch_viterbi_path(gtnx_batch_t a, gtnx_batch_t* out) {
  return guard([&] { *out = HB(batch_viterbi_path(BH(a))); });
}
GTNX_API gtnx_status_t gtnx_batch_viterbi_align(gtnx_batch_t a, const int* frames, void* labels_device, int64_t row_stride,
                                                void* tokens_device, void* scores_device) {
  return guard([&] {
    batch_viterbi_align(BH(a), frames, static_cast<int*>(labels_device), row_stride, static_cast<int*>(tokens_device),
                        static_cast<float*>(scores_device));
  });
}
GTNX_API gtnx_status_t gtnx_batch_align_stats(int64_t* fast, int64_t* fallback) {
  return guard([&] { batch_align_stats(fast, fallback); });
}
GTNX_API gtnx_status_t gtnx_batch_viterbi_decode(gtnx_batch_t ems, gtnx_graph_t transitions, const int* frames,
                                                 void* labels_device, int64_t row_stride, void* scores_device,
                                                 void* collapsed_device, void* lengths_device) {
  return guard([&] {
    batch_viterbi_decode(BH(ems), G(transitions), frames, static_cast<int*>(labels_device), row_stride,
                         static_cast<float*>(scores_device), static_cast<int*>(collapsed_device),
                         static_cast<int*>(lengths_device));
  });
}
GTNX_API gtnx_status_t gtnx_batch_decode_stats(int64_t* fast, int64_t* fallback) {
  return guard([&] { batch_decode_stats(fast, fallback); });
}
GTNX_API gtnx_status_t gtnx_batch_linear_decode(gtnx_batch_t ems, const int* frames, int blank, void* labels_device,
                                                int64_t row_stride, void* scores_device, void* collapsed_device,
                                                void* starts_device, void* lengths_device) {
// ... 325 lines not shown
```

gtn_amd/csrc/kernels.h:

```cpp
#pragma once

#include <hip/hip_runtime.h>

#include <cstdint>

#include <atomic>
#include <cstdint>
struct gtnx_first_on_device {
  std::atomic<uint64_t>& done;
  uint64_t bit;
  bool first;
  explicit gtnx_first_on_device(std::atomic<uint64_t>& d) : done(d) {
    int dev = 0;
    (void)hipGetDevice(&dev);
    bit = uint64_t(1) << (dev & 63);
    first = !(done.load(std::memory_order_acquire) & bit);
  }
  gtnx_first_on_device(const gtnx_first_on_device&) = delete;
  ~gtnx_first_on_device() {
    if (first) done.fetch_or(bit, std::memory_order_acq_rel);
  }
  explicit operator bool() const { return first; }
};

// ... 392 lines not shown
  const GTNX_G uint8_t* nflags;
  const GTNX_G float* em;
  GTNX_G unsigned* bp;
  GTNX_G int* labels;
  GTNX_G int* tokens;
  GTNX_G float* score;
  int N, T, T_full, C;
  int p, pad;
};
int align_npl(int max_nodes);
bool band_align_ok(int max_nodes, int max_labels, int vec);
void launch_band_align(const AlignArgs* d_args, int n, int max_nodes, hipStream_t st);
struct AsgAlignArgs {
  const GTNX_G BandNode* nodes;
  const GTNX_G uint8_t* nflags;
  const GTNX_G float* w;
  const GTNX_G float* em;
  GTNX_G unsigned* bp;
  GTNX_G int* labels;
  GTNX_G int* tokens;
  GTNX_G float* score;
  int N, T, T_full, C;
};
int asg_align_npl(int max_nodes);
int asg_align_max_labels();
bool asg_align_ok(int max_nodes, int max_labels, int vec);
size_t asg_align_plane_bytes(int T, int npl);
void launch_asg_align(const AsgAlignArgs* d_args, int n, int max_nodes, hipStream_t st);
struct RationalSeg {
  DGraph g;
  int node_off, arc_off;
  int conn_off;
  int keep_start, keep_accept;
  int pad;
};
struct RationalOut {
  int N, A;
  GTNX_G int* src;
  GTNX_G int* dst;
  GTNX_G int* il;
  GTNX_G int* ol;
  GTNX_G float* w;
  GTNX_G uint8_t* nflags;
  GTNX_G int* start_list;
  GTNX_G int* accept_list;
  GTNX_G int* out_off;
  GTNX_G int* out_list;
  GTNX_G int* in_off;
  GTNX_G int* in_list;
};
size_t rational_csr_temp_bytes(int N, int A);
void launch_rational_build(const RationalSeg* d_segs, int nseg, int max_A, int max_N, int max_conn, const RationalOut& out,
                           int projection, int closure, void* temp, hipStream_t st);
void launch_rational_adjacency(const RationalOut& out, void* temp, hipStream_t st);
struct RemoveArgs {
  DGraph g;
  int ilabel, olabel;
  const GTNX_G int* new_id;
  const GTNX_G int* roots;
  int K, root0, rows;
  GTNX_G int* stamp;
  GTNX_G int* queue;
  GTNX_G int* arc_cnt;
  const GTNX_G int* arc_off;
  RationalOut out;
};
void launch_remove_keep(const DGraph& g, int ilabel, int olabel, int* keep, hipStream_t st);
void launch_remove_roots(const int* keep, const int* new_id, int N, int* roots, hipStream_t st);
void launch_remove_walk(const RemoveArgs& a, bool emit, hipStream_t st);
size_t scan_temp_bytes(int n);
void launch_exclusive_scan(const int* in, int* out, int n, void* temp, size_t temp_bytes, hipStream_t st);
void launch_rational_load(const void* rows, const float* w, const uint8_t* flags, const RationalOut& out, void* temp,
                          hipStream_t st);
struct CtcTargetArgs {
  const GTNX_G int* labels;
  GTNX_G BandNode* nodes;
  GTNX_G uint8_t* nflags;
  GTNX_G int* snode;
  GTNX_G int* slab;
  GTNX_G int* n_arcs;
  int N, pad;
};
void launch_ctc_targets(const CtcTargetArgs* d_args, int n, int blank, hipStream_t st);
struct AsgFalArgs {
  const GTNX_G int* labels;
  const GTNX_G float* trans_w;
  GTNX_G BandNode* nodes;
  GTNX_G uint8_t* nflags;
  GTNX_G int* snode;
  GTNX_G int* slab;
  GTNX_G float* w;
  GTNX_G int* arc_map;
  int U, pad;
};
void launch_asg_fal_targets(const AsgFalArgs* d_args, int n, int n_labels, hipStream_t st);
void launch_asg_fal_scatter(const float* g, const int* maps, const int64_t* tab , int n_seq, int64_t longest,
                            float* trans_grad, hipStream_t st);
int band_max_nodes();
int band_max_labels();
int band_min_labels();
int band_npl(int max_nodes);
int band_row_stride(int N, int npl);
int band_forward_lgrn(int C);
bool band_one_ok(int npl, int C, int max_NS, bool vec, bool backward);
void launch_band_forward(const BandPair* d_pairs, int n, int npl, int C, int max_NS, bool unit, bool vec, hipStream_t st,
                         const BandPair* one = nullptr);
void launch_band_backward(const BandPair* d_pairs, int n, int npl, int C, int max_NS, bool unit, bool gradg, bool vec,
                          hipStream_t st, const BandPair* one = nullptr, const BandPatch* patch = nullptr);
void launch_lazy_dense_prep(const LazyGroup& g, float* E, float* cmax, hipStream_t st);
void launch_lazy_dense_step(const LazyGroup& g, int t, int backward, hipStream_t st, const float* vin = nullptr,
                            float* vout = nullptr);
void launch_lazy_dense_fixed_grad(const LazyGroup& g, hipStream_t st);
size_t maxplus_w_floats(const LazyGroup& g);
void launch_maxplus_prep(const LazyGroup& g, hipStream_t st);
void launch_maxplus_step(const LazyGroup& g, int t, hipStream_t st);
void launch_maxplus_path(const LazyGroup& g, int* path_arc, int* path_il, int* path_ol, float* path_w, int* path_len,
                         hipStream_t st);
void launch_asg_decode(const LazyGroup& g, const int* d_frames, int* labels, int64_t row_stride, float* scores,
                       int* collapsed, int* lengths, hipStream_t st);
void launch_lazy_mfma_prep(const LazyGroup& g, hipStream_t st);
void launch_lazy_mfma_init(const LazyGroup& g, int which, hipStream_t st);
void launch_lazy_mfma_step(const LazyGroup& g, int t, int backward, hipStream_t st);
size_t lazy_mfma_chain_sync_ints(const LazyGroup& g);
bool launch_lazy_mfma_chain(const LazyGroup& g, int backward, int* zeroed_sync, int cus, hipStream_t st);
void launch_lazy_mfma_keys(float* keys, int64_t n, hipStream_t st);
void launch_lazy_mfma_rowmax(const LazyGroup& g, int which, hipStream_t st);
void launch_lazy_mfma_score(const LazyGroup& g, hipStream_t st);
size_t lazy_mfma_fixed_grad_scratch_bytes(const LazyGroup& g);
void launch_lazy_mfma_fixed_grad(const LazyGroup& g, void* pair_consts , hipStream_t st, void* partials = nullptr,
                                 size_t partials_bytes = 0);

void launch_fill_i32(int* p, int v, size_t n, hipStream_t st);
void launch_fill_f32(float* p, float v, size_t n, hipStream_t st);
void launch_scalar_seed(float* root, float* g0, float s0, int acc0, float* g1, float s1, int acc1, size_t n, hipStream_t st);
struct ScalarArgs {
  const GTNX_G float* a;
  const GTNX_G float* b;
  GTNX_G float* out;
  GTNX_G float* mirror;
};
void launch_scalar_combine(const ScalarArgs* d_args, int n, float sa, float sb, hipStream_t st);
void launch_copy_small(void* dst, const void* src, size_t bytes, hipStream_t st);
void launch_scalar_combine_one(const ScalarArgs& a, float sa, float sb, hipStream_t st);
struct ScalarFanArgs {
  const GTNX_G float* d;
  GTNX_G float* seed;
  GTNX_G float* o0;
  GTNX_G float* o1;
};
void launch_scalar_fan(const ScalarFanArgs* d_args, int n, float s0, float s1, hipStream_t st);
void launch_scalar_fan_one(const ScalarFanArgs& a, float s0, float s1, hipStream_t st);
struct AxpyArgs {
  GTNX_G float* dst;
  const GTNX_G float* src;
  int64_t n;
  float scale;
};
void launch_axpy_batch(const AxpyArgs* d_args, int n, int64_t maxn, int atomic, hipStream_t st);
struct CopySeg {
  void* dst;
  const void* src;
  int64_t bytes;
};
void launch_copy_segments(const CopySeg* d_segs, int n, int64_t max_bytes, hipStream_t st);
void launch_gather_scalars(const float* const* d_ptrs, float* out, int n, hipStream_t st);
void launch_vec_axpby(float* out, const float* a, const float* b, size_t n, float sa, float sb, int accumulate, hipStream_t st);
// ... 186 lines not shown
```

include/gtn/batch.h:

```cpp
#pragma once
#include <cstdint>
#include <utility>
#include <vector>

#include "gtn/functions.h"

namespace gtn {

class Batch {
 public:
  Batch() = default;
  explicit Batch(const std::vector<Graph>& graphs) {
    auto h = detail::handles(graphs);
    detail::check(gtnx_batch_from_graphs(h.data(), static_cast<int>(h.size()), &h_));
  }
  Batch(const Batch&) = delete;
  Batch& operator=(const Batch&) = delete;
  Batch(Batch&& o) noexcept : h_(o.h_) { o.h_ = nullptr; }
  Batch& operator=(Batch&& o) noexcept {
    if (this != &o) {
      reset();
      h_ = o.h_;
      o.h_ = nullptr;
    }
// ... 160 lines not shown
    detail::check(gtnx_lm_graph_walk(h_, state, label, &w, &nx));
    if (weight) *weight = w;
    if (nextState) *nextState = nx;
    return nx >= 0;
  }
  Info info() const {
    gtnx_lm_graph_info_t i;
    detail::check(gtnx_lm_graph_info(h_, &i));
    return Info{i.num_states, i.num_arcs, i.start_state, i.longest_epsilon_chain};
  }
  gtnx_lm_graph_t handle() const { return h_; }

 private:
  gtnx_lm_graph_t h_ = nullptr;
};
inline void ctcBeamDecode(const Batch& ems, const LmGraph& lm, float lmWeight, float insertionBonus, int* tokensDevice,
                          int64_t rowStride, int* lengthsDevice, float* scoresDevice, float* amScoresDevice = nullptr,
                          int blank = 0, int beamSize = 16, int cutoffTopN = 16, int nbest = 1,
                          const int* frames = nullptr) {
  detail::check(gtnx_batch_ctc_beam_decode_graph(ems.handle(), frames, blank, beamSize, cutoffTopN, nbest, lm.handle(),
                                                 lmWeight, insertionBonus, tokensDevice, rowStride, lengthsDevice,
                                                 scoresDevice, amScoresDevice));
}
inline void editDistance(const int* hypDevice, int64_t hypStride, const int* hypLengthsDevice, const int* refDevice,
                         int64_t refStride, const int* refLengthsDevice, int B, int N, int L, int U, int* distDevice,
                         int* opsDevice = nullptr) {
  detail::check(gtnx_batch_edit_distance(hypDevice, hypStride, hypLengthsDevice, refDevice, refStride, refLengthsDevice,
                                         B, N, L, U, distDevice, opsDevice));
}
inline void ctcScore(const Batch& ems, const int* tokensDevice, int64_t rowStride, const int* lengthsDevice, int N, int L,
                     int maxLength, float* scoresDevice, int blank = 0, const int* frames = nullptr) {
  detail::check(gtnx_batch_ctc_score(ems.handle(), frames, blank, tokensDevice, rowStride, lengthsDevice, N, L, maxLength,
                                     scoresDevice));
}
inline void ctcScoreGrad(const Batch& ems, const int* tokensDevice, int64_t rowStride, const int* lengthsDevice, int N,
                         int L, int maxLength, const float* weightsDevice, float* gradDevice, int blank = 0,
                         const int* frames = nullptr) {
  detail::check(gtnx_batch_ctc_score_grad(ems.handle(), frames, blank, tokensDevice, rowStride, lengthsDevice, N, L,
                                          maxLength, weightsDevice, gradDevice));
}
inline void asgScore(const Batch& ems, const float* tableDevice, const int* tokensDevice, int64_t rowStride,
                     const int* lengthsDevice, int N, int L, int maxLength, float* scoresDevice,
                     const int* frames = nullptr) {
  detail::check(gtnx_batch_asg_score(ems.handle(), frames, tableDevice, tokensDevice, rowStride, lengthsDevice, N, L,
                                     maxLength, scoresDevice));
}
inline void asgScoreGrad(const Batch& ems, const float* tableDevice, const int* tokensDevice, int64_t rowStride,
                         const int* lengthsDevice, int N, int L, int maxLength, const float* weightsDevice,
                         float* gradEmissionsDevice, float* gradTableDevice, const int* frames = nullptr) {
  detail::check(gtnx_batch_asg_score_grad(ems.handle(), frames, tableDevice, tokensDevice, rowStride, lengthsDevice, N,
                                          L, maxLength, weightsDevice, gradEmissionsDevice, gradTableDevice));
}
inline void asgBeamDecode(const Batch& ems, const float* tableDevice, int* tokensDevice, int64_t rowStride,
                          int* lengthsDevice, float* scoresDevice, int beamSize = 16, int cutoffTopN = 16, int nbest = 1,
                          const int* frames = nullptr) {
  detail::check(gtnx_batch_asg_beam_decode(ems.handle(), frames, tableDevice, beamSize, cutoffTopN, nbest, tokensDevice,
                                           rowStride, lengthsDevice, scoresDevice));
}
inline void asgBeamDecode(const Batch& ems, const float* tableDevice, const LmGraph& lm, float lmWeight,
                          float insertionBonus, int* tokensDevice, int64_t rowStride, int* lengthsDevice,
                          float* scoresDevice, float* amScoresDevice = nullptr, int beamSize = 16, int cutoffTopN = 16,
                          int nbest = 1, const int* frames = nullptr) {
  detail::check(gtnx_batch_asg_beam_decode_graph(ems.handle(), frames, tableDevice, beamSize, cutoffTopN, nbest,
                                                 lm.handle(), lmWeight, insertionBonus, tokensDevice, rowStride,
                                                 lengthsDevice, scoresDevice, amScoresDevice));
}
inline void ctcTokenAlign(const Batch& ems, const int* tokensDevice, int64_t rowStride, const int* lengthsDevice, int N,
                          int L, int maxLength, float* scoresDevice, int* startsDevice, int* endsDevice,
                          float* tokenScoresDevice, int64_t outStride, int* frameTokensDevice = nullptr,
                          int64_t frameStride = 0, int blank = 0, const int* frames = nullptr) {
  detail::check(gtnx_batch_ctc_token_align(ems.handle(), frames, blank, tokensDevice, rowStride, lengthsDevice, N, L,
                                           maxLength, scoresDevice, startsDevice, endsDevice, tokenScoresDevice,
                                           outStride, frameTokensDevice, frameStride));
}
inline void asgTokenAlign(const Batch& ems, const float* tableDevice, const int* tokensDevice, int64_t rowStride,
                          const int* lengthsDevice, int N, int L, int maxLength, float* scoresDevice, int* startsDevice,
                          int* endsDevice, float* tokenScoresDevice, int64_t outStride,
                          int* frameTokensDevice = nullptr, int64_t frameStride = 0, const int* frames = nullptr) {
  detail::check(gtnx_batch_asg_token_align(ems.handle(), frames, tableDevice, tokensDevice, rowStride, lengthsDevice, N,
                                           L, maxLength, scoresDevice, startsDevice, endsDevice, tokenScoresDevice,
                                           outStride, frameTokensDevice, frameStride));
}
inline void backward(const Batch& a, bool retainGraph = false) { detail::check(gtnx_batch_backward(a.handle(), retainGraph)); }
}

}
```

include/gtn_amd.h:

```cpp
#ifndef GTN_AMD_H
#define GTN_AMD_H

#include <stddef.h>
#include <stdint.h>

#ifdef __cplusplus
extern "C" {
#endif

typedef int gtnx_status_t;
#define GTNX_OK 0
#define GTNX_INVALID_ARGUMENT 1
#define GTNX_LOGIC_ERROR 2
#define GTNX_RUNTIME_ERROR 3
#define GTNX_OUT_OF_RANGE 4
#define GTNX_DEVICE_ERROR 5

typedef struct gtnx_graph_s* gtnx_graph_t;

#define GTNX_EPSILON (-1)

const char* gtnx_last_error(void);
const char* gtnx_version(void);
const char* gtnx_backend(void);
// ... 27 lines not shown
gtnx_status_t gtnx_graph_num_start(gtnx_graph_t g, int64_t* out);
gtnx_status_t gtnx_graph_num_accept(gtnx_graph_t g, int64_t* out);
gtnx_status_t gtnx_graph_item(gtnx_graph_t g, float* out);
gtnx_status_t gtnx_graph_arc_sort(gtnx_graph_t g, int olabel);
gtnx_status_t gtnx_graph_mark_arc_sorted(gtnx_graph_t g, int olabel);
gtnx_status_t gtnx_graph_ilabel_sorted(gtnx_graph_t g, int* out);
gtnx_status_t gtnx_graph_olabel_sorted(gtnx_graph_t g, int* out);
gtnx_status_t gtnx_graph_weights(gtnx_graph_t g, int mutable_, float** out);
gtnx_status_t gtnx_graph_get_weights(gtnx_graph_t g, float* out);
gtnx_status_t gtnx_graph_set_weights(gtnx_graph_t g, const float* weights);
gtnx_status_t gtnx_graph_set_weights_device(gtnx_graph_t g, const void* device_weights);
gtnx_status_t gtnx_graph_weights_device(gtnx_graph_t g, void** out);
gtnx_status_t gtnx_graph_labels_to_array(gtnx_graph_t g, int* out, int ilabel);
gtnx_status_t gtnx_graph_get_start(gtnx_graph_t g, int* out);
gtnx_status_t gtnx_graph_get_accept(gtnx_graph_t g, int* out);
gtnx_status_t gtnx_graph_is_start(gtnx_graph_t g, int node, int* out);
gtnx_status_t gtnx_graph_is_accept(gtnx_graph_t g, int node, int* out);
gtnx_status_t gtnx_graph_make_accept(gtnx_graph_t g, int node);
gtnx_status_t gtnx_graph_num_out(gtnx_graph_t g, int node, int64_t* out);
gtnx_status_t gtnx_graph_num_in(gtnx_graph_t g, int node, int64_t* out);
gtnx_status_t gtnx_graph_get_out(gtnx_graph_t g, int node, int* out);
gtnx_status_t gtnx_graph_get_in(gtnx_graph_t g, int node, int* out);
gtnx_status_t gtnx_graph_get_arcs(gtnx_graph_t g, int* src, int* dst, int* ilabel, int* olabel);
gtnx_status_t gtnx_graph_get_arc(gtnx_graph_t g, int arc, int* src, int* dst,
                                 int* ilabel, int* olabel, float* weight);
gtnx_status_t gtnx_graph_set_weight(gtnx_graph_t g, int arc, float weight);
gtnx_status_t gtnx_graph_calc_grad(gtnx_graph_t g, int* out);
gtnx_status_t gtnx_graph_set_calc_grad(gtnx_graph_t g, int calc_grad);
gtnx_status_t gtnx_graph_is_grad_available(gtnx_graph_t g, int* out);
gtnx_status_t gtnx_graph_grad(gtnx_graph_t g, gtnx_graph_t* out);
gtnx_status_t gtnx_graph_zero_grad(gtnx_graph_t g);
gtnx_status_t gtnx_graph_add_grad(gtnx_graph_t g, const float* host_grad, int64_t n);
gtnx_status_t gtnx_graph_add_grad_graph(gtnx_graph_t g, gtnx_graph_t other);
gtnx_status_t gtnx_graph_id(gtnx_graph_t g, uintptr_t* out);
typedef gtnx_status_t (*gtnx_grad_fn)(void* ctx, gtnx_graph_t* inputs, int n_inputs, gtnx_graph_t deltas);
gtnx_status_t gtnx_graph_create_op(gtnx_graph_t* inputs, int n_inputs, gtnx_grad_fn grad_fn,
                                   void* ctx, void (*ctx_free)(void*), gtnx_graph_t* out);
gtnx_status_t gtnx_graph_num_inputs(gtnx_graph_t g, int64_t* out);
gtnx_status_t gtnx_graph_get_input(gtnx_graph_t g, int i, gtnx_graph_t* out);
gtnx_status_t gtnx_graph_set_inputs(gtnx_graph_t g, const gtnx_graph_t* inputs, int n);
gtnx_status_t gtnx_graph_set_grad_fn(gtnx_graph_t g, gtnx_grad_fn grad_fn, void* ctx,
                                     void (*ctx_free)(void*));
gtnx_status_t gtnx_graph_has_grad_fn(gtnx_graph_t g, int* out);

gtnx_status_t gtnx_scalar_graph(float value, int calc_grad, gtnx_graph_t* out);
gtnx_status_t gtnx_linear_graph(int M, int N, int calc_grad, gtnx_graph_t* out);
gtnx_status_t gtnx_linear_graph_n(int B, int M, int N, int calc_grad,
                                  const void* device_weights, gtnx_graph_t* out );
gtnx_status_t gtnx_linear_graph_borrow_n(int B, int M, int N, int calc_grad,
                                         const void* device_weights, gtnx_graph_t* out );

gtnx_status_t gtnx_negate(gtnx_graph_t g, gtnx_graph_t* out);
gtnx_status_t gtnx_add(gtnx_graph_t a, gtnx_graph_t b, gtnx_graph_t* out);
gtnx_status_t gtnx_subtract(gtnx_graph_t a, gtnx_graph_t b, gtnx_graph_t* out);
gtnx_status_t gtnx_compose(gtnx_graph_t a, gtnx_graph_t b, gtnx_graph_t* out);
gtnx_status_t gtnx_intersect(gtnx_graph_t a, gtnx_graph_t b, gtnx_graph_t* out);
gtnx_status_t gtnx_forward_score(gtnx_graph_t g, gtnx_graph_t* out);
gtnx_status_t gtnx_viterbi_score(gtnx_graph_t g, gtnx_graph_t* out);
gtnx_status_t gtnx_viterbi_path(gtnx_graph_t g, gtnx_graph_t* out);

gtnx_status_t gtnx_negate_n(const gtnx_graph_t* g, int n, gtnx_graph_t* out);
gtnx_status_t gtnx_add_n(const gtnx_graph_t* a, int na, const gtnx_graph_t* b, int nb, gtnx_graph_t* out);
gtnx_status_t gtnx_subtract_n(const gtnx_graph_t* a, int na, const gtnx_graph_t* b, int nb, gtnx_graph_t* out);
gtnx_status_t gtnx_compose_n(const gtnx_graph_t* a, int na, const gtnx_graph_t* b, int nb, gtnx_graph_t* out);
gtnx_status_t gtnx_intersect_n(const gtnx_graph_t* a, int na, const gtnx_graph_t* b, int nb, gtnx_graph_t* out);
gtnx_status_t gtnx_forward_score_n(const gtnx_graph_t* g, int n, gtnx_graph_t* out);
gtnx_status_t gtnx_viterbi_score_n(const gtnx_graph_t* g, int n, gtnx_graph_t* out);
gtnx_status_t gtnx_viterbi_path_n(const gtnx_graph_t* g, int n, gtnx_graph_t* out);
gtnx_status_t gtnx_items_n(const gtnx_graph_t* g, int n, float* out);
gtnx_status_t gtnx_items_device_n(const gtnx_graph_t* g, int n, void* device_out);
gtnx_status_t gtnx_grads_device_n(const gtnx_graph_t* g, int n, void* device_out, const int64_t* offsets);
gtnx_status_t gtnx_grads_bind_device_n(const gtnx_graph_t* g, int n, void* device_out, const int64_t* offsets);

gtnx_status_t gtnx_clone(gtnx_graph_t g, int projection , gtnx_graph_t* out);
gtnx_status_t gtnx_concat(const gtnx_graph_t* g, int n, gtnx_graph_t* out);
gtnx_status_t gtnx_closure(gtnx_graph_t g, gtnx_graph_t* out);
gtnx_status_t gtnx_union(const gtnx_graph_t* g, int n, gtnx_graph_t* out);
gtnx_status_t gtnx_remove(gtnx_graph_t g, int ilabel, int olabel, gtnx_graph_t* out);

typedef struct gtnx_batch_s* gtnx_batch_t;
gtnx_status_t gtnx_batch_from_graphs(const gtnx_graph_t* g, int n, gtnx_batch_t* out);
gtnx_status_t gtnx_batch_ctc_targets(const int* labels, const int* lengths, int n, int blank, int calc_grad,
                                     gtnx_batch_t* out);
gtnx_status_t gtnx_batch_asg_force_align(const int* labels, const int* lengths, int n, gtnx_graph_t transitions,
                                         int n_labels, gtnx_batch_t* out);
gtnx_status_t gtnx_batch_linear(int n, int M, int N, int calc_grad, const void* device_weights, int borrow,
                                gtnx_batch_t* out);
gtnx_status_t gtnx_batch_linear_rows(int n, int M, int N, const int* rows, int calc_grad, const void* device_weights,
                                     int borrow, gtnx_batch_t* out);
gtnx_status_t gtnx_batch_destroy(gtnx_batch_t b);
gtnx_status_t gtnx_batch_size(gtnx_batch_t b, int* out);
gtnx_status_t gtnx_batch_get(gtnx_batch_t b, int i, gtnx_graph_t* out);
gtnx_status_t gtnx_batch_negate(gtnx_batch_t a, gtnx_batch_t* out);
gtnx_status_t gtnx_batch_add(gtnx_batch_t a, gtnx_batch_t b, gtnx_batch_t* out);
gtnx_status_t gtnx_batch_subtract(gtnx_batch_t a, gtnx_batch_t b, gtnx_batch_t* out);
gtnx_status_t gtnx_batch_subtract_into(gtnx_batch_t a, gtnx_batch_t b, void* items_device, gtnx_batch_t* out);
gtnx_status_t gtnx_batch_compose(gtnx_batch_t a, gtnx_batch_t b, gtnx_batch_t* out);
gtnx_status_t gtnx_batch_intersect(gtnx_batch_t a, gtnx_batch_t b, gtnx_batch_t* out);
gtnx_status_t gtnx_batch_forward_score(gtnx_batch_t a, gtnx_batch_t* out);
gtnx_status_t gtnx_batch_viterbi_score(gtnx_batch_t a, gtnx_batch_t* out);
gtnx_status_t gtnx_batch_viterbi_path(gtnx_batch_t a, gtnx_batch_t* out);
gtnx_status_t gtnx_batch_viterbi_align(gtnx_batch_t a, const int* frames, void* labels_device, int64_t row_stride,
                                       void* tokens_device, void* scores_device);
gtnx_status_t gtnx_batch_align_stats(int64_t* fast, int64_t* fallback);
gtnx_status_t gtnx_batch_viterbi_decode(gtnx_batch_t ems, gtnx_graph_t transitions, const int* frames,
                                        void* labels_device, int64_t row_stride, void* scores_device,
                                        void* collapsed_device, void* lengths_device);
gtnx_status_t gtnx_batch_decode_stats(int64_t* fast, int64_t* fallback);
gtnx_status_t gtnx_batch_full_connect_stats(int64_t* fast, int64_t* fallback);
gtnx_status_t gtnx_batch_linear_decode(gtnx_batch_t ems, const int* frames, int blank, void* labels_device,
                                       int64_t row_stride, void* scores_device, void* collapsed_device,
                                       void* starts_device, void* lengths_device);
gtnx_status_t gtnx_batch_linear_decode_stats(int64_t* fast, int64_t* fallback);
gtnx_status_t gtnx_batch_ctc_sample(gtnx_batch_t ems, const int* frames, int blank, int num_samples, uint64_t seed,
                                    float temperature, void* tokens_device, int64_t row_stride, void* lengths_device,
                                    void* logq_device , void* labels_device );
gtnx_status_t gtnx_batch_ctc_sample_stats(int64_t* calls, int64_t* utterances);
gtnx_status_t gtnx_batch_ctc_beam_decode(gtnx_batch_t ems, const int* frames, int blank, int beam_size,
                                         int cutoff_top_n, int nbest, void* tokens_device, int64_t row_stride,
                                         void* lengths_device, void* scores_device);
gtnx_status_t gtnx_batch_ctc_beam_decode_lm(gtnx_batch_t ems, const int* frames, int blank, int beam_size,
                                            int cutoff_top_n, int nbest, const void* lm_device, float lm_weight,
                                            float insertion_bonus, void* tokens_device, int64_t row_stride,
                                            void* lengths_device, void* scores_device,
                                            void* am_scores_device );
typedef struct gtnx_lm_graph_s* gtnx_lm_graph_t;
typedef struct {
  int64_t num_states;
  int64_t num_arcs;
  int32_t start_state;
  int32_t longest_epsilon_chain;
} gtnx_lm_graph_info_t;
gtnx_status_t gtnx_lm_graph_create(gtnx_graph_t g, gtnx_lm_graph_t* out);
gtnx_status_t gtnx_lm_graph_destroy(gtnx_lm_graph_t lm);
gtnx_status_t gtnx_lm_graph_walk(gtnx_lm_graph_t lm, int state, int label, float* weight, int* next_state);
gtnx_status_t gtnx_lm_graph_info(gtnx_lm_graph_t lm, gtnx_lm_graph_info_t* out);
gtnx_status_t gtnx_batch_ctc_beam_decode_graph(gtnx_batch_t ems, const int* frames, int blank, int beam_size,
                                               int cutoff_top_n, int nbest, gtnx_lm_graph_t lm_graph, float lm_weight,
                                               float insertion_bonus, void* tokens_device, int64_t row_stride,
                                               void* lengths_device, void* scores_device,
                                               void* am_scores_device );
gtnx_status_t gtnx_batch_ctc_beam_stats(int64_t* calls, int64_t* utterances);
gtnx_status_t gtnx_batch_edit_distance(const void* hyp_device, int64_t hyp_stride, const void* hyp_lengths_device,
                                       const void* ref_device, int64_t ref_stride, const void* ref_lengths_device,
                                       int B, int N, int L, int U, void* dist_device, void* ops_device);
gtnx_status_t gtnx_batch_edit_distance_stats(int64_t* calls, int64_t* pairs);
gtnx_status_t gtnx_batch_ctc_score(gtnx_batch_t ems, const int* frames, int blank, const void* tokens_device,
                                   int64_t row_stride, const void* lengths_device, int N, int L, int max_length,
                                   void* scores_device);
gtnx_status_t gtnx_batch_ctc_score_grad(gtnx_batch_t ems, const int* frames, int blank, const void* tokens_device,
                                        int64_t row_stride, const void* lengths_device, int N, int L, int max_length,
                                        const void* weights_device, void* grad_device);
gtnx_status_t gtnx_batch_ctc_score_stats(int64_t* calls, int64_t* pairs);
gtnx_status_t gtnx_batch_ctc_token_align(gtnx_batch_t ems, const int* frames, int blank, const void* tokens_device,
                                         int64_t row_stride, const void* lengths_device, int N, int L, int max_length,
                                         void* scores_device, void* starts_device, void* ends_device,
                                         void* token_scores_device, int64_t out_stride, void* frame_tokens_device,
                                         int64_t frame_stride);
gtnx_status_t gtnx_batch_ctc_token_align_stats(int64_t* calls, int64_t* pairs);
gtnx_status_t gtnx_batch_asg_score(gtnx_batch_t ems, const int* frames, const void* table_device,
                                   const void* tokens_device, int64_t row_stride, const void* lengths_device, int N,
                                   int L, int max_length, void* scores_device);
gtnx_status_t gtnx_batch_asg_score_grad(gtnx_batch_t ems, const int* frames, const void* table_device,
                                        const void* tokens_device, int64_t row_stride, const void* lengths_device,
                                        int N, int L, int max_length, const void* weights_device,
                                        void* grad_emissions_device, void* grad_table_device);
// ... 55 lines not shown
```

Measured before the change: 936,700 losses/s.

## Fuse CTC target build, forward and backward into one step kernel

Adds a fused CTC loss step path that builds the CTC target records, runs the banded forward pass and then the backward pass inside a single kernel launch per utterance. The loss is written directly and emission gradients are produced without building intermediate graph batches. It targets the per-stage host work, separate launches and global round trips of the graph-based pipeline. It is taken by default when all frames are full and the shape fits a supported cell, with an environment switch to disable it. It adds a large template kernel with high LDS use and a separate code path to keep consistent with the general one.

```diff
diff --git a/gtn_amd/_capi.py b/gtn_amd/_capi.py
--- a/gtn_amd/_capi.py
+++ b/gtn_amd/_capi.py
@@ -101,6 +101,10 @@
     "gtnx_union": [c_graph_p, C.c_int, c_graph_p],
     "gtnx_batch_from_graphs": [c_graph_p, C.c_int, c_graph_p],
     "gtnx_batch_ctc_targets": [C.c_void_p, C.c_void_p, C.c_int, C.c_int, C.c_int, c_graph_p],
+    "gtnx_batch_ctc_loss_step": [C.c_void_p, C.c_void_p, C.c_void_p, C.c_int, C.c_int, C.c_int, C.c_int, C.c_void_p,
+                                 C.c_void_p, C.c_int, C.c_void_p],
+    "gtnx_batch_ctc_loss_step_ok": [C.c_void_p, C.c_void_p, C.c_int, C.c_int, C.c_int, C.c_int, C.c_void_p, C.c_void_p,
+                                    C.POINTER(C.c_int)],
     "gtnx_batch_asg_force_align": [C.c_void_p, C.c_void_p, C.c_int, c_graph, C.c_int, c_graph_p],
     "gtnx_batch_linear": [C.c_int, C.c_int, C.c_int, C.c_int, C.c_void_p, C.c_int, c_graph_p],
     "gtnx_batch_linear_rows": [C.c_int, C.c_int, C.c_int, C.c_void_p, C.c_int, C.c_void_p, C.c_int, c_graph_p],
diff --git a/gtn_amd/criteria/criteria_capi.cpp b/gtn_amd/criteria/criteria_capi.cpp
--- a/gtn_amd/criteria/criteria_capi.cpp
+++ b/gtn_amd/criteria/criteria_capi.cpp
@@ -150,6 +150,15 @@
     gtn::Batch ctcs;
     gtn::criteria::ctcLossBatch(emissions, targets, lengths, B, T, C, blank, loss, grad, true, nullptr, &ctcs);
     if (target_grad) ctcs.gradsToDevice(target_grad, target_grad_offsets);
+  });
+}
+
+GTN_EXPORT int gtn_ctc_loss_step_n(const void* emissions, const int* targets, const int* lengths, int B, int T, int C,
+                                   int blank, const int* frames, void* loss, void* grad, int target_grad,
+                                   void* target_grad_dev) {
+  return guarded([&] {
+    gtn::criteria::ctcLossBatch(emissions, targets, lengths, B, T, C, blank, loss, grad, target_grad != 0, nullptr, nullptr,
+                                frames, target_grad_dev);
   });
 }
 
diff --git a/gtn_amd/criteria/ctc_criterion.h b/gtn_amd/criteria/ctc_criterion.h
--- a/gtn_amd/criteria/ctc_criterion.h
+++ b/gtn_amd/criteria/ctc_criterion.h
@@ -2,6 +2,7 @@
 
 #include <chrono>
 #include <cstdint>
+#include <cstdlib>
 #include <stdexcept>
 #include <vector>
 
@@ -50,12 +51,28 @@
     bool targetGrad = true,
     CtcStepTimes* times = nullptr,
     Batch* targetsOut = nullptr,
-    const int* frames = nullptr) {
+    const int* frames = nullptr,
+    void* targetGradDev = nullptr) {
   auto now = [] { return std::chrono::steady_clock::now(); };
   auto ms = [](auto a, auto b) { return std::chrono::duration<double, std::milli>(b - a).count(); };
   if (frames)
     for (int b = 0; b < B; ++b)
       if (frames[b] < 1 || frames[b] > T) throw std::invalid_argument("[ctcLossBatch] a frame count outside 1 .. T");
+  if (gradDev && !targetsOut && B > 0) {
+    bool full = true;
+    for (int b = 0; frames && b < B && full; ++b) full = frames[b] == T;
+    const char* sw = std::getenv("GTNX_CTC_STEP_FUSED");
+    int ok = 0;
+    if (full && !(sw && sw[0] == '0' && sw[1] == 0))
+      detail::check(gtnx_batch_ctc_loss_step_ok(labels, lengths, B, T, C, blank, emissions, gradDev, &ok));
+    if (ok) {
+      auto t0 = now();
+      detail::check(gtnx_batch_ctc_loss_step(emissions, labels, lengths, B, T, C, blank, lossDev, gradDev, targetGrad ? 1 : 0,
+                                             targetGrad ? targetGradDev : nullptr));
+      if (times) *times = {0, 0, 0, ms(t0, now()), 0};
+      return;
+    }
+  }
   auto t0 = now();
   Batch ctcs = Batch::ctcTargets(labels, lengths, B, blank, targetGrad);
   auto t1 = now();
@@ -75,6 +92,18 @@
   if (times) *times = {ms(t0, t1), ms(t1, t2), ms(t2, t3), ms(t3, t4), ms(t4, t5)};
   losses.itemsToDevice(lossDev);
   if (gradDev) ems.gradsToDevice(gradDev, off.data());
+  if (targetGradDev && targetGrad && gradDev) {
+    std::vector<int64_t> goff(static_cast<size_t>(B));
+    int64_t run = 0, lo = 0;
+    for (int b = 0; b < B; ++b) {
+      const int U = lengths[b];
+      goff[static_cast<size_t>(b)] = run;
+      run += 4 * int64_t(U) + 1;
+      for (int u = 1; u < U; ++u) run += labels[lo + u] != labels[lo + u - 1] ? 1 : 0;
+      lo += U;
+    }
+    ctcs.gradsToDevice(targetGradDev, goff.data());
+  }
   if (targetsOut) *targetsOut = std::move(ctcs);
 }
 
diff --git a/gtn_amd/csrc/band.hip b/gtn_amd/csrc/band.hip
--- a/gtn_amd/csrc/band.hip
+++ b/gtn_amd/csrc/band.hip
@@ -14,323 +14,7 @@
 namespace gtnx {
 namespace {
 
-constexpr float NEGF = -1.0e30f;
-constexpr float DEADF = -1.0e29f;
-constexpr float LOG2E = 1.44269504088896340736f;
-constexpr double LN2 = 0.693147180559945309417;
-constexpr int BW = 256;
-constexpr int WG = 512;
-constexpr int WGB = 768;
-constexpr int NBE = 5;
-constexpr int NBG = 7;
-constexpr int NBGE = 8;
-#ifndef GTNX_BWD_SPLIT
-#define GTNX_BWD_SPLIT 0
-#endif
-#ifndef GTNX_FWD_COPY_DEPTH
-#define GTNX_FWD_COPY_DEPTH 2
-#endif
-#ifndef GTNX_FWD_COPY_ROTATE
-#define GTNX_FWD_COPY_ROTATE 1
-#endif
-#ifndef GTNX_FWD_DEPTH
-#define GTNX_FWD_DEPTH 2
-#endif
-
-#ifdef GTNX_BAND_TIMING
-#define GTNX_TM(slot)                 \
-  do {                                \
-    const long long now_ = clock64(); \
-    tm_acc[slot] += now_ - tm_last;   \
-    tm_last = now_;                   \
-  } while (0)
-#define GTNX_TM_INIT(base)                       \
-  const int tm_base = base;                      \
-  long long tm_acc[8] = {0, 0, 0, 0, 0, 0, 0, 0}; \
-  long long tm_n = 0;                            \
-  long long tm_last = clock64()
-#define GTNX_TM_TICK() tm_n += 1
-#define GTNX_TM_DUMP()                                                      \
-  do {                                                                      \
-    if (blockIdx.x == 0 && (threadIdx.x & 63) == 0) {                       \
-      for (int i_ = 0; i_ < 7; ++i_) g_band_timing[tm_base + (threadIdx.x >> 6) * 7 + i_] += tm_acc[i_]; \
-      if (threadIdx.x == 0) g_band_timing[tm_base + 127] += tm_n;           \
-    }                                                                       \
-  } while (0)
-#else
-#define GTNX_TM(slot) do { } while (0)
-#define GTNX_TM_INIT(base) do { } while (0)
-#define GTNX_TM_TICK() do { } while (0)
-#define GTNX_TM_DUMP() do { } while (0)
-#endif
-
-__device__ __forceinline__ void lds_barrier() { asm volatile("s_waitcnt lgkmcnt(0)\n\ts_barrier" ::: "memory"); }
-#ifdef GTNX_EXP_FAKE_MATH
-__device__ __forceinline__ float ex2(float x) { return __builtin_fmaf(x, 0.001f, 1.0f); }
-__device__ __forceinline__ float lg2(float x) { return __builtin_fmaf(x, 0.001f, -0.001f); }
-#else
-__device__ __forceinline__ float ex2(float x) { return __builtin_amdgcn_exp2f(x); }
-__device__ __forceinline__ float lg2(float x) { return __builtin_amdgcn_logf(x); }
-#endif
-
-__device__ __forceinline__ void settle(float& x) { asm volatile("" : "+v"(x)); }
-__device__ __forceinline__ void settle(int& x) { asm volatile("" : "+v"(x)); }
-__device__ __forceinline__ float uniform(float x) {
-  return __int_as_float(__builtin_amdgcn_readfirstlane(__float_as_int(x)));
-}
-__device__ __forceinline__ double uniform(double x) {
-  const long long b = __double_as_longlong(x);
-  const unsigned lo = __builtin_amdgcn_readfirstlane(unsigned(b)), hi = __builtin_amdgcn_readfirstlane(unsigned(b >> 32));
-  return __longlong_as_double((long long)(((unsigned long long)hi << 32) | lo));
-}
-
-__device__ __forceinline__ float wave_shr1(float x, float fill) {
-  return __int_as_float(__builtin_amdgcn_update_dpp(__float_as_int(fill), __float_as_int(x), 0x138, 0xf, 0xf, false));
-}
-__device__ __forceinline__ float wave_shl1(float x, float fill) {
-  return __int_as_float(__builtin_amdgcn_update_dpp(__float_as_int(fill), __float_as_int(x), 0x130, 0xf, 0xf, false));
-}
-#define GTNX_DPP6(op)                                                         \
-  "s_nop 1\n\t" op " %0, %0, %0 row_shr:1 row_mask:0xf bank_mask:0xf\n\t"     \
-  "s_nop 1\n\t" op " %0, %0, %0 row_shr:2 row_mask:0xf bank_mask:0xf\n\t"     \
-  "s_nop 1\n\t" op " %0, %0, %0 row_shr:4 row_mask:0xf bank_mask:0xf\n\t"     \
-  "s_nop 1\n\t" op " %0, %0, %0 row_shr:8 row_mask:0xf bank_mask:0xf\n\t"     \
-  "s_nop 1\n\t" op " %0, %0, %0 row_bcast:15 row_mask:0xa bank_mask:0xf\n\t"  \
-  "s_nop 1\n\t" op " %0, %0, %0 row_bcast:31 row_mask:0xc bank_mask:0xf\n\t"  \
-  "s_nop 1"
-__device__ __forceinline__ float wave_max(float x) {
-  asm volatile(GTNX_DPP6("v_max_f32_dpp") : "+v"(x));
-  return __int_as_float(__builtin_amdgcn_readlane(__float_as_int(x), 63));
-}
-__device__ __forceinline__ float wave_sum63(float x) {
-  asm volatile(GTNX_DPP6("v_add_f32_dpp") : "+v"(x));
-  return x;
-}
-__device__ __forceinline__ float wave_sum(float x) {
-  return __int_as_float(__builtin_amdgcn_readlane(__float_as_int(wave_sum63(x)), 63));
-}
-#define GTNX_DPP2(ctl)                                                  \
-  "v_add_f32_dpp %0, %0, %0 " ctl "\n\tv_add_f32_dpp %1, %1, %1 " ctl "\n\ts_nop 0\n\t"
-__device__ __forceinline__ void wave_sum63x2(float& a, float& b) {
-  asm volatile("s_nop 1\n\t"
-               GTNX_DPP2("row_shr:1 row_mask:0xf bank_mask:0xf")
-               GTNX_DPP2("row_shr:2 row_mask:0xf bank_mask:0xf")
-               GTNX_DPP2("row_shr:4 row_mask:0xf bank_mask:0xf")
-               GTNX_DPP2("row_shr:8 row_mask:0xf bank_mask:0xf")
-               GTNX_DPP2("row_bcast:15 row_mask:0xa bank_mask:0xf")
-               GTNX_DPP2("row_bcast:31 row_mask:0xc bank_mask:0xf")
-               : "+v"(a), "+v"(b));
-}
-__device__ __forceinline__ void row_sum15x2(float& a, float& b) {
-  asm volatile("s_nop 1\n\t"
-               GTNX_DPP2("row_shr:1 row_mask:0xf bank_mask:0xf")
-               GTNX_DPP2("row_shr:2 row_mask:0xf bank_mask:0xf")
-               GTNX_DPP2("row_shr:4 row_mask:0xf bank_mask:0xf")
-               GTNX_DPP2("row_shr:8 row_mask:0xf bank_mask:0xf")
-               : "+v"(a), "+v"(b));
-}
-#define GTNX_ROR4(op)                                                        \
-  "s_nop 1\n\t" op " %0, %0, %0 row_ror:8 row_mask:0xf bank_mask:0xf\n\t"    \
-  "s_nop 1\n\t" op " %0, %0, %0 row_ror:4 row_mask:0xf bank_mask:0xf\n\t"    \
-  "s_nop 1\n\t" op " %0, %0, %0 row_ror:2 row_mask:0xf bank_mask:0xf\n\t"    \
-  "s_nop 1\n\t" op " %0, %0, %0 row_ror:1 row_mask:0xf bank_mask:0xf\n\t"    \
-  "s_nop 1"
-__device__ __forceinline__ float row16_max(float x) {
-  asm volatile(GTNX_ROR4("v_max_f32_dpp") : "+v"(x));
-  return x;
-}
-__device__ __forceinline__ float row16_sum(float x) {
-  asm volatile(GTNX_ROR4("v_add_f32_dpp") : "+v"(x));
-  return x;
-}
-__device__ __forceinline__ float lse3(float x0, float x1, float x2) {
-  const float mx = fmaxf(fmaxf(x0, x1), x2);
-  const float md = __builtin_amdgcn_fmed3f(x0, x1, x2);
-  const float mn = fminf(fminf(x0, x1), x2);
-  return mx + lg2(1.0f + ex2(md - mx) + ex2(mn - mx));
-}
-
-template <int NPL>
-struct NodeRegs {
-  int lab[NPL];
-  float wi[3][NPL];
-  float wo[3][NPL];
-  int ao[3][NPL];
-  bool has_in[NPL];
-  bool start[NPL], accept[NPL];
-};
-template <int NPL, bool WANT_OUT>
-__device__ __forceinline__ void load_nodes(const BandPair& P, int m0, NodeRegs<NPL>& g) {
-  const GTNX_G gtnx_i4* nodes = reinterpret_cast<const GTNX_G gtnx_i4*>(P.nodes);
-#pragma unroll
-  for (int j = 0; j < NPL; ++j) {
-    const int m = m0 + j;
-    g.lab[j] = 0;
-    g.start[j] = g.accept[j] = g.has_in[j] = false;
-#pragma unroll
-    for (int k = 0; k < 3; ++k) {
-      g.wi[k][j] = g.wo[k][j] = NEGF;
-      g.ao[k][j] = -1;
-    }
-    if (m < P.N) {
-      const gtnx_i4 q = nodes[m];
-      g.lab[j] = q.x >= 0 ? q.x : 0;
-      const uint8_t f = P.nflags[m];
-      g.start[j] = (f & NF_START) != 0;
-      g.accept[j] = (f & NF_ACCEPT) != 0;
-      const int a[3] = {q.y, q.z, q.w};
-#pragma unroll
-      for (int k = 0; k < 3; ++k)
-        if (a[k] >= 0) {
-          g.has_in[j] = true;
-          g.wi[k][j] = P.w ? fmaxf(P.w[a[k]] * LOG2E, NEGF) : 0.0f;
-        }
-    }
-    if (WANT_OUT) {
-#pragma unroll
-      for (int k = 0; k < 3; ++k) {
-        if (m + k < P.N) {
-          const gtnx_i4 q = nodes[m + k];
-          const int a = k == 0 ? q.y : (k == 1 ? q.z : q.w);
-          if (a >= 0) {
-            g.ao[k][j] = a;
-            g.wo[k][j] = P.w ? fmaxf(P.w[a] * LOG2E, NEGF) : 0.0f;
-          }
-        }
-      }
-    }
-  }
-}
-
-__device__ __forceinline__ float em2(float x) { return fmaxf(x * LOG2E, NEGF); }
-
-__device__ __forceinline__ int row_of(int e, int W, float invW) {
-  int r = int(float(e) * invW);
-  if (r * W > e) --r;
-  if ((r + 1) * W <= e) ++r;
-  return r;
-}
-
-template <int NS, int LN = BW>
-struct Stage {
-  float v[NS];
-  template <bool VEC>
-  __device__ __forceinline__ void issue(const GTNX_G float* src, int cnt, int tid) {
-    if (cnt <= 0) return;
-#pragma unroll
-    for (int i = 0; i < NS / 4; ++i) {
-      if (i > 0 && 4 * i * LN >= cnt) break;
-      const int e = min(4 * (i * LN + tid), cnt - 4);
-      const gtnx_f4 q = *reinterpret_cast<const GTNX_G gtnx_f4*>(reinterpret_cast<const GTNX_G char*>(src) + unsigned(4 * e));
-      v[4 * i] = q.x;
-      v[4 * i + 1] = q.y;
-      v[4 * i + 2] = q.z;
-      v[4 * i + 3] = q.w;
-    }
-  }
-  int off[NS / 4];
-  __device__ __forceinline__ void init_offsets(int W, int stride, int K, int tid, bool reverse = true) {
-    const float invW = 1.0f / float(W);
-#pragma unroll
-    for (int i = 0; i < NS / 4; ++i) {
-      const int e = 4 * (i * LN + tid);
-      const int r = row_of(min(e, 4096), W, invW);
-      off[i] = (reverse ? K - 1 - r : r) * stride + (e - r * W);
-    }
-  }
-  template <class F>
-  __device__ __forceinline__ void each_vec(int cnt, int shift, int tid, F&& f) const {
-#pragma unroll
-    for (int i = 0; i < NS / 4; ++i) {
-      if (i > 0 && 4 * i * LN >= cnt) break;
-      if (4 * (i * LN + tid) < cnt) f(i, off[i] - shift, gtnx_f4{v[4 * i], v[4 * i + 1], v[4 * i + 2], v[4 * i + 3]});
-    }
-  }
-  __device__ __forceinline__ void settle_all() {
-#pragma unroll
-    for (int i = 0; i < NS; ++i) asm volatile("" : "+v"(v[i]));
-  }
-  template <bool VEC, class F>
-  __device__ __forceinline__ void each(int cnt, int W, int tid, F&& f) const {
-    const float invW = 1.0f / float(W);
-    if constexpr (VEC) {
-#pragma unroll
-      for (int i = 0; i < NS / 4; ++i) {
-        if (i > 0 && 4 * i * LN >= cnt) break;
-        const int e = 4 * (i * LN + tid);
-        if (e < cnt) {
-          const int r = row_of(e, W, invW);
-          f(i, e, r, e - r * W, gtnx_f4{v[4 * i], v[4 * i + 1], v[4 * i + 2], v[4 * i + 3]});
-        }
-      }
-    } else {
-#pragma unroll
-      for (int i = 0; i < NS / 4; ++i) {
-        if (i > 0 && 4 * i * LN >= cnt) break;
-        if (4 * (i * LN + tid) < cnt) {
-          const int e = min(4 * (i * LN + tid), cnt - 4);
-          const int r0 = row_of(e, W, invW), c0 = e - r0 * W;
-#pragma unroll
-          for (int k = 0; k < 4; ++k) {
-            int r = r0, col = c0 + k;
-            if (col >= W) {
-              col -= W;
-              ++r;
-            }
-            f(i, e + k, r, col, gtnx_f4{v[4 * i + k], 0.0f, 0.0f, 0.0f});
-          }
-        }
-      }
-    }
-  }
-};
-
-struct BandLds {
-  int CS;
-  int o_ering, o_aring, o_oring, o_snode, o_misc, total;
-};
-__host__ __device__ inline BandLds band_lds(int C, int K, int NSmax, bool backward) {
-  BandLds L;
-  L.CS = C + 4;
-  int o = 0;
-  L.o_ering = o;
-  o += (backward ? NBGE : NBE) * K * L.CS;
-  o = (o + 3) & ~3;
-  L.o_aring = o;
-  o += backward ? NBE * K * NSmax : 0;
-  o = (o + 3) & ~3;
-  L.o_oring = o;
-  o += backward ? max(NBG * K * NSmax, 2 * C) : 0;
-  o = (o + 3) & ~3;
-  L.o_snode = o;
-  o += backward ? 512 : 0;
-  L.o_misc = o;
-  o += 160 + 32 + 8 + 2 * NBE * K * 4 + 40 * K + 8 + 512;
-  L.total = o;
-  return L;
-}
-struct BandMisc {
-  double *offr, *red, *find, *aofr;
-  float *bndr, *fin, *lsep;
-};
-template <int K>
-__device__ __forceinline__ BandMisc band_misc(float* lds, const BandLds& L) {
-  BandMisc m;
-  m.offr = reinterpret_cast<double*>(lds + L.o_misc);
-  m.red = m.offr + 80;
-  m.find = m.red + 16;
-  m.aofr = m.find + 4;
-  m.bndr = lds + L.o_misc + 200 + 2 * NBE * K * 4;
-  m.fin = m.bndr + 40 * K;
-  m.lsep = m.fin + 8;
-  return m;
-}
-
-__device__ __forceinline__ float wave_max_of(const float* v, int n) {
-  float mx = v[0];
-  for (int j = 1; j < n; ++j) mx = fmaxf(mx, v[j]);
-  return wave_max(mx);
-}
+#include "band_device.inc"
 
 template <int NPL, bool UNIT, int K, bool VEC>
 __global__ __launch_bounds__(WG) void band_forward_kernel(const BandPair* __restrict__ pairs, int NSmax) {
@@ -376,41 +60,7 @@
   const CtcTargetArgs a = args[blockIdx.x];
   __shared__ __attribute__((aligned(16))) int tl[256 + 4];
   __shared__ __attribute__((aligned(16))) int tk[256 + 4];
-  const int N = a.N, U = (N - 1) >> 1, m = threadIdx.x;
-  if (m < 260) {
-    const int v = m < U ? a.labels[m] : 0x7fffffff;
-    tl[m] = v;
-    tk[m] = (m > 0 && m < U && v != a.labels[m - 1]) ? 1 : 0;
-  }
-  __syncthreads();
-  if (m >= N) return;
-  const bool odd = (m & 1) != 0;
-  const int my = odd ? tl[(m - 1) >> 1] : blank;
-  const int skip = odd ? tk[(m - 1) >> 1] : 0;
-  const int mi = (m - 1) >> 1;
-  const int before = odd ? mi : (m >> 1);
-  int rank = 0, skips = 0;
-  for (int o = 0; o < U; o += 4) {
-    const gtnx_i4 l4 = *reinterpret_cast<const gtnx_i4*>(tl + o), k4 = *reinterpret_cast<const gtnx_i4*>(tk + o);
-    const int lo[4] = {l4.x, l4.y, l4.z, l4.w}, ko[4] = {k4.x, k4.y, k4.z, k4.w};
-#pragma unroll
-    for (int k = 0; k < 4; ++k) {
-      const bool front = o + k < before;
-      rank += (lo[k] < my || (lo[k] == my && front)) ? 1 : 0;
-      skips += front ? ko[k] : 0;
-    }
-  }
-  rank += blank < my ? U + 1 : (blank == my ? (m + 1) >> 1 : 0);
-  const int base = (m > 0 ? 2 * m - 1 : 0) + skips;
-  GTNX_G BandNode* nd = const_cast<GTNX_G BandNode*>(a.nodes);
-  nd[m].lab = my;
-  nd[m].aid[0] = base;
-  nd[m].aid[1] = m > 0 ? base + 1 : -1;
-  nd[m].aid[2] = skip ? base + 2 : -1;
-  a.nflags[m] = uint8_t((m == 0 ? NF_START : 0) | (m + 2 >= N ? NF_ACCEPT : 0));
-  a.snode[rank] = m;
-  a.slab[rank] = my;
-  if (m == N - 1 && a.n_arcs) a.n_arcs[0] = base + 1 + (m > 0 ? 1 : 0) + skip;
+  ctc_target_records(a, blank, tl, tk);
 }
 
 __global__ __launch_bounds__(512) void band_viterbi_kernel(const BandDecode* __restrict__ pairs) {
diff --git a/gtn_amd/csrc/band_backward_body.inc b/gtn_amd/csrc/band_backward_body.inc
--- a/gtn_amd/csrc/band_backward_body.inc
+++ b/gtn_amd/csrc/band_backward_body.inc
@@ -134,7 +134,14 @@
       h2 = __builtin_elementwise_fma(f2v{v[k].x, v[k].y}, f2v{R.hot[k].x, R.hot[k].y}, h2);
       h2 = __builtin_elementwise_fma(f2v{v[k].z, v[k].w}, f2v{R.hot[k].z, R.hot[k].w}, h2);
     }
-    float all = (a2.x + a2.y) * R.in, hotp = h2.x + h2.y;
+#ifdef GTNX_BWD_RS4_LEAN
+    int nb_l = 16 * (l & 15);
+    settle(nb_l);
+    const float r_in = nb_l < NSmax ? 1.0f : 0.0f;
+#else
+    const float r_in = R.in;
+#endif
+    float all = (a2.x + a2.y) * r_in, hotp = h2.x + h2.y;
     if (dead_r) all = hotp = 0.0f;
     row_sum15x2(all, hotp);
     const bool have = all != 0.0f && !dead_r;
diff --git a/gtn_amd/csrc/band_device.inc b/gtn_amd/csrc/band_device.inc
--- /dev/null
+++ b/gtn_amd/csrc/band_device.inc
@@ -0,0 +1,355 @@
+constexpr float NEGF = -1.0e30f;
+constexpr float DEADF = -1.0e29f;
+constexpr float LOG2E = 1.44269504088896340736f;
+constexpr double LN2 = 0.693147180559945309417;
+constexpr int BW = 256;
+constexpr int WG = 512;
+constexpr int WGB = 768;
+constexpr int NBE = 5;
+constexpr int NBG = 7;
+constexpr int NBGE = 8;
+#ifndef GTNX_BWD_SPLIT
+#define GTNX_BWD_SPLIT 0
+#endif
+#ifndef GTNX_FWD_COPY_DEPTH
+#define GTNX_FWD_COPY_DEPTH 2
+#endif
+#ifndef GTNX_FWD_COPY_ROTATE
+#define GTNX_FWD_COPY_ROTATE 1
+#endif
+#ifndef GTNX_FWD_DEPTH
+#define GTNX_FWD_DEPTH 2
+#endif
+
+#ifdef GTNX_BAND_TIMING
+#define GTNX_TM(slot)                 \
+  do {                                \
+    const long long now_ = clock64(); \
+    tm_acc[slot] += now_ - tm_last;   \
+    tm_last = now_;                   \
+  } while (0)
+#define GTNX_TM_INIT(base)                       \
+  const int tm_base = base;                      \
+  long long tm_acc[8] = {0, 0, 0, 0, 0, 0, 0, 0}; \
+  long long tm_n = 0;                            \
+  long long tm_last = clock64()
+#define GTNX_TM_TICK() tm_n += 1
+#define GTNX_TM_DUMP()                                                      \
+  do {                                                                      \
+    if (blockIdx.x == 0 && (threadIdx.x & 63) == 0) {                       \
+      for (int i_ = 0; i_ < 7; ++i_) g_band_timing[tm_base + (threadIdx.x >> 6) * 7 + i_] += tm_acc[i_]; \
+      if (threadIdx.x == 0) g_band_timing[tm_base + 127] += tm_n;           \
+    }                                                                       \
+  } while (0)
+#else
+#define GTNX_TM(slot) do { } while (0)
+#define GTNX_TM_INIT(base) do { } while (0)
+#define GTNX_TM_TICK() do { } while (0)
+#define GTNX_TM_DUMP() do { } while (0)
+#endif
+
+__device__ __forceinline__ void lds_barrier() { asm volatile("s_waitcnt lgkmcnt(0)\n\ts_barrier" ::: "memory"); }
+#ifdef GTNX_EXP_FAKE_MATH
+__device__ __forceinline__ float ex2(float x) { return __builtin_fmaf(x, 0.001f, 1.0f); }
+__device__ __forceinline__ float lg2(float x) { return __builtin_fmaf(x, 0.001f, -0.001f); }
+#else
+__device__ __forceinline__ float ex2(float x) { return __builtin_amdgcn_exp2f(x); }
+__device__ __forceinline__ float lg2(float x) { return __builtin_amdgcn_logf(x); }
+#endif
+
+__device__ __forceinline__ void settle(float& x) { asm volatile("" : "+v"(x)); }
+__device__ __forceinline__ void settle(int& x) { asm volatile("" : "+v"(x)); }
+__device__ __forceinline__ float uniform(float x) {
+  return __int_as_float(__builtin_amdgcn_readfirstlane(__float_as_int(x)));
+}
+__device__ __forceinline__ double uniform(double x) {
+  const long long b = __double_as_longlong(x);
+  const unsigned lo = __builtin_amdgcn_readfirstlane(unsigned(b)), hi = __builtin_amdgcn_readfirstlane(unsigned(b >> 32));
+  return __longlong_as_double((long long)(((unsigned long long)hi << 32) | lo));
+}
+
+__device__ __forceinline__ float wave_shr1(float x, float fill) {
+  return __int_as_float(__builtin_amdgcn_update_dpp(__float_as_int(fill), __float_as_int(x), 0x138, 0xf, 0xf, false));
+}
+__device__ __forceinline__ float wave_shl1(float x, float fill) {
+  return __int_as_float(__builtin_amdgcn_update_dpp(__float_as_int(fill), __float_as_int(x), 0x130, 0xf, 0xf, false));
+}
+#define GTNX_DPP6(op)                                                         \
+  "s_nop 1\n\t" op " %0, %0, %0 row_shr:1 row_mask:0xf bank_mask:0xf\n\t"     \
+  "s_nop 1\n\t" op " %0, %0, %0 row_shr:2 row_mask:0xf bank_mask:0xf\n\t"     \
+  "s_nop 1\n\t" op " %0, %0, %0 row_shr:4 row_mask:0xf bank_mask:0xf\n\t"     \
+  "s_nop 1\n\t" op " %0, %0, %0 row_shr:8 row_mask:0xf bank_mask:0xf\n\t"     \
+  "s_nop 1\n\t" op " %0, %0, %0 row_bcast:15 row_mask:0xa bank_mask:0xf\n\t"  \
+  "s_nop 1\n\t" op " %0, %0, %0 row_bcast:31 row_mask:0xc bank_mask:0xf\n\t"  \
+  "s_nop 1"
+__device__ __forceinline__ float wave_max(float x) {
+  asm volatile(GTNX_DPP6("v_max_f32_dpp") : "+v"(x));
+  return __int_as_float(__builtin_amdgcn_readlane(__float_as_int(x), 63));
+}
+__device__ __forceinline__ float wave_sum63(float x) {
+  asm volatile(GTNX_DPP6("v_add_f32_dpp") : "+v"(x));
+  return x;
+}
+__device__ __forceinline__ float wave_sum(float x) {
+  return __int_as_float(__builtin_amdgcn_readlane(__float_as_int(wave_sum63(x)), 63));
+}
+#define GTNX_DPP2(ctl)                                                  \
+  "v_add_f32_dpp %0, %0, %0 " ctl "\n\tv_add_f32_dpp %1, %1, %1 " ctl "\n\ts_nop 0\n\t"
+__device__ __forceinline__ void wave_sum63x2(float& a, float& b) {
+  asm volatile("s_nop 1\n\t"
+               GTNX_DPP2("row_shr:1 row_mask:0xf bank_mask:0xf")
+               GTNX_DPP2("row_shr:2 row_mask:0xf bank_mask:0xf")
+               GTNX_DPP2("row_shr:4 row_mask:0xf bank_mask:0xf")
+               GTNX_DPP2("row_shr:8 row_mask:0xf bank_mask:0xf")
+               GTNX_DPP2("row_bcast:15 row_mask:0xa bank_mask:0xf")
+               GTNX_DPP2("row_bcast:31 row_mask:0xc bank_mask:0xf")
+               : "+v"(a), "+v"(b));
+}
+__device__ __forceinline__ void row_sum15x2(float& a, float& b) {
+  asm volatile("s_nop 1\n\t"
+               GTNX_DPP2("row_shr:1 row_mask:0xf bank_mask:0xf")
+               GTNX_DPP2("row_shr:2 row_mask:0xf bank_mask:0xf")
+               GTNX_DPP2("row_shr:4 row_mask:0xf bank_mask:0xf")
+               GTNX_DPP2("row_shr:8 row_mask:0xf bank_mask:0xf")
+               : "+v"(a), "+v"(b));
+}
+#define GTNX_ROR4(op)                                                        \
+  "s_nop 1\n\t" op " %0, %0, %0 row_ror:8 row_mask:0xf bank_mask:0xf\n\t"    \
+  "s_nop 1\n\t" op " %0, %0, %0 row_ror:4 row_mask:0xf bank_mask:0xf\n\t"    \
+  "s_nop 1\n\t" op " %0, %0, %0 row_ror:2 row_mask:0xf bank_mask:0xf\n\t"    \
+  "s_nop 1\n\t" op " %0, %0, %0 row_ror:1 row_mask:0xf bank_mask:0xf\n\t"    \
+  "s_nop 1"
+__device__ __forceinline__ float row16_max(float x) {
+  asm volatile(GTNX_ROR4("v_max_f32_dpp") : "+v"(x));
+  return x;
+}
+__device__ __forceinline__ float row16_sum(float x) {
+  asm volatile(GTNX_ROR4("v_add_f32_dpp") : "+v"(x));
+  return x;
+}
+__device__ __forceinline__ float lse3(float x0, float x1, float x2) {
+  const float mx = fmaxf(fmaxf(x0, x1), x2);
+  const float md = __builtin_amdgcn_fmed3f(x0, x1, x2);
+  const float mn = fminf(fminf(x0, x1), x2);
+  return mx + lg2(1.0f + ex2(md - mx) + ex2(mn - mx));
+}
+
+template <int NPL>
+struct NodeRegs {
+  int lab[NPL];
+  float wi[3][NPL];
+  float wo[3][NPL];
+  int ao[3][NPL];
+  bool has_in[NPL];
+  bool start[NPL], accept[NPL];
+};
+template <int NPL, bool WANT_OUT>
+__device__ __forceinline__ void load_nodes(const BandPair& P, int m0, NodeRegs<NPL>& g) {
+  const GTNX_G gtnx_i4* nodes = reinterpret_cast<const GTNX_G gtnx_i4*>(P.nodes);
+#pragma unroll
+  for (int j = 0; j < NPL; ++j) {
+    const int m = m0 + j;
+    g.lab[j] = 0;
+    g.start[j] = g.accept[j] = g.has_in[j] = false;
+#pragma unroll
+    for (int k = 0; k < 3; ++k) {
+      g.wi[k][j] = g.wo[k][j] = NEGF;
+      g.ao[k][j] = -1;
+    }
+    if (m < P.N) {
+      const gtnx_i4 q = nodes[m];
+      g.lab[j] = q.x >= 0 ? q.x : 0;
+      const uint8_t f = P.nflags[m];
+      g.start[j] = (f & NF_START) != 0;
+      g.accept[j] = (f & NF_ACCEPT) != 0;
+      const int a[3] = {q.y, q.z, q.w};
+#pragma unroll
+      for (int k = 0; k < 3; ++k)
+        if (a[k] >= 0) {
+          g.has_in[j] = true;
+          g.wi[k][j] = P.w ? fmaxf(P.w[a[k]] * LOG2E, NEGF) : 0.0f;
+        }
+    }
+    if (WANT_OUT) {
+#pragma unroll
+      for (int k = 0; k < 3; ++k) {
+        if (m + k < P.N) {
+          const gtnx_i4 q = nodes[m + k];
+          const int a = k == 0 ? q.y : (k == 1 ? q.z : q.w);
+          if (a >= 0) {
+            g.ao[k][j] = a;
+            g.wo[k][j] = P.w ? fmaxf(P.w[a] * LOG2E, NEGF) : 0.0f;
+          }
+        }
+      }
+    }
+  }
+}
+
+__device__ __forceinline__ float em2(float x) { return fmaxf(x * LOG2E, NEGF); }
+
+__device__ __forceinline__ int row_of(int e, int W, float invW) {
+  int r = int(float(e) * invW);
+  if (r * W > e) --r;
+  if ((r + 1) * W <= e) ++r;
+  return r;
+}
+
+template <int NS, int LN = BW>
+struct Stage {
+  float v[NS];
+  template <bool VEC>
+  __device__ __forceinline__ void issue(const GTNX_G float* src, int cnt, int tid) {
+    if (cnt <= 0) return;
+#pragma unroll
+    for (int i = 0; i < NS / 4; ++i) {
+      if (i > 0 && 4 * i * LN >= cnt) break;
+      const int e = min(4 * (i * LN + tid), cnt - 4);
+      const gtnx_f4 q = *reinterpret_cast<const GTNX_G gtnx_f4*>(reinterpret_cast<const GTNX_G char*>(src) + unsigned(4 * e));
+      v[4 * i] = q.x;
+      v[4 * i + 1] = q.y;
+      v[4 * i + 2] = q.z;
+      v[4 * i + 3] = q.w;
+    }
+  }
+  int off[NS / 4];
+  __device__ __forceinline__ void init_offsets(int W, int stride, int K, int tid, bool reverse = true) {
+    const float invW = 1.0f / float(W);
+#pragma unroll
+    for (int i = 0; i < NS / 4; ++i) {
+      const int e = 4 * (i * LN + tid);
+      const int r = row_of(min(e, 4096), W, invW);
+      off[i] = (reverse ? K - 1 - r : r) * stride + (e - r * W);
+    }
+  }
+  template <class F>
+  __device__ __forceinline__ void each_vec(int cnt, int shift, int tid, F&& f) const {
+#pragma unroll
+    for (int i = 0; i < NS / 4; ++i) {
+      if (i > 0 && 4 * i * LN >= cnt) break;
+      if (4 * (i * LN + tid) < cnt) f(i, off[i] - shift, gtnx_f4{v[4 * i], v[4 * i + 1], v[4 * i + 2], v[4 * i + 3]});
+    }
+  }
+  __device__ __forceinline__ void settle_all() {
+#pragma unroll
+    for (int i = 0; i < NS; ++i) asm volatile("" : "+v"(v[i]));
+  }
+  template <bool VEC, class F>
+  __device__ __forceinline__ void each(int cnt, int W, int tid, F&& f) const {
+    const float invW = 1.0f / float(W);
+    if constexpr (VEC) {
+#pragma unroll
+      for (int i = 0; i < NS / 4; ++i) {
+        if (i > 0 && 4 * i * LN >= cnt) break;
+        const int e = 4 * (i * LN + tid);
+        if (e < cnt) {
+          const int r = row_of(e, W, invW);
+          f(i, e, r, e - r * W, gtnx_f4{v[4 * i], v[4 * i + 1], v[4 * i + 2], v[4 * i + 3]});
+        }
+      }
+    } else {
+#pragma unroll
+      for (int i = 0; i < NS / 4; ++i) {
+        if (i > 0 && 4 * i * LN >= cnt) break;
+        if (4 * (i * LN + tid) < cnt) {
+          const int e = min(4 * (i * LN + tid), cnt - 4);
+          const int r0 = row_of(e, W, invW), c0 = e - r0 * W;
+#pragma unroll
+          for (int k = 0; k < 4; ++k) {
+            int r = r0, col = c0 + k;
+            if (col >= W) {
+              col -= W;
+              ++r;
+            }
+            f(i, e + k, r, col, gtnx_f4{v[4 * i + k], 0.0f, 0.0f, 0.0f});
+          }
+        }
+      }
+    }
+  }
+};
+
+struct BandLds {
+  int CS;
+  int o_ering, o_aring, o_oring, o_snode, o_misc, total;
+};
+__host__ __device__ inline BandLds band_lds(int C, int K, int NSmax, bool backward) {
+  BandLds L;
+  L.CS = C + 4;
+  int o = 0;
+  L.o_ering = o;
+  o += (backward ? NBGE : NBE) * K * L.CS;
+  o = (o + 3) & ~3;
+  L.o_aring = o;
+  o += backward ? NBE * K * NSmax : 0;
+  o = (o + 3) & ~3;
+  L.o_oring = o;
+  o += backward ? max(NBG * K * NSmax, 2 * C) : 0;
+  o = (o + 3) & ~3;
+  L.o_snode = o;
+  o += backward ? 512 : 0;
+  L.o_misc = o;
+  o += 160 + 32 + 8 + 2 * NBE * K * 4 + 40 * K + 8 + 512;
+  L.total = o;
+  return L;
+}
+struct BandMisc {
+  double *offr, *red, *find, *aofr;
+  float *bndr, *fin, *lsep;
+};
+template <int K>
+__device__ __forceinline__ BandMisc band_misc(float* lds, const BandLds& L) {
+  BandMisc m;
+  m.offr = reinterpret_cast<double*>(lds + L.o_misc);
+  m.red = m.offr + 80;
+  m.find = m.red + 16;
+  m.aofr = m.find + 4;
+  m.bndr = lds + L.o_misc + 200 + 2 * NBE * K * 4;
+  m.fin = m.bndr + 40 * K;
+  m.lsep = m.fin + 8;
+  return m;
+}
+
+__device__ __forceinline__ float wave_max_of(const float* v, int n) {
+  float mx = v[0];
+  for (int j = 1; j < n; ++j) mx = fmaxf(mx, v[j]);
+  return wave_max(mx);
+}
+
+__device__ __forceinline__ void ctc_target_records(const CtcTargetArgs& a, int blank, int* tl, int* tk) {
+  const int N = a.N, U = (N - 1) >> 1, m = threadIdx.x;
+  if (m < 260) {
+    const int v = m < U ? a.labels[m] : 0x7fffffff;
+    tl[m] = v;
+    tk[m] = (m > 0 && m < U && v != a.labels[m - 1]) ? 1 : 0;
+  }
+  __syncthreads();
+  if (m >= N) return;
+  const bool odd = (m & 1) != 0;
+  const int my = odd ? tl[(m - 1) >> 1] : blank;
+  const int skip = odd ? tk[(m - 1) >> 1] : 0;
+  const int mi = (m - 1) >> 1;
+  const int before = odd ? mi : (m >> 1);
+  int rank = 0, skips = 0;
+  for (int o = 0; o < U; o += 4) {
+    const gtnx_i4 l4 = *reinterpret_cast<const gtnx_i4*>(tl + o), k4 = *reinterpret_cast<const gtnx_i4*>(tk + o);
+    const int lo[4] = {l4.x, l4.y, l4.z, l4.w}, ko[4] = {k4.x, k4.y, k4.z, k4.w};
+#pragma unroll
+    for (int k = 0; k < 4; ++k) {
+      const bool front = o + k < before;
+      rank += (lo[k] < my || (lo[k] == my && front)) ? 1 : 0;
+      skips += front ? ko[k] : 0;
+    }
+  }
+  rank += blank < my ? U + 1 : (blank == my ? (m + 1) >> 1 : 0);
+  const int base = (m > 0 ? 2 * m - 1 : 0) + skips;
+  GTNX_G BandNode* nd = const_cast<GTNX_G BandNode*>(a.nodes);
+  nd[m].lab = my;
+  nd[m].aid[0] = base;
+  nd[m].aid[1] = m > 0 ? base + 1 : -1;
+  nd[m].aid[2] = skip ? base + 2 : -1;
+  a.nflags[m] = uint8_t((m == 0 ? NF_START : 0) | (m + 2 >= N ? NF_ACCEPT : 0));
+  a.snode[rank] = m;
+  a.slab[rank] = my;
+  if (m == N - 1 && a.n_arcs) a.n_arcs[0] = base + 1 + (m > 0 ? 1 : 0) + skip;
+}
diff --git a/gtn_amd/csrc/band_forward_body.inc b/gtn_amd/csrc/band_forward_body.inc
--- a/gtn_amd/csrc/band_forward_body.inc
+++ b/gtn_amd/csrc/band_forward_body.inc
@@ -193,6 +193,11 @@
       M.fin[2 * w + 1] = s;
       M.find[w] = off;
     }
+#ifdef GTNX_FWD_IDLE_FROM
+  } else if (wv >= GTNX_FWD_IDLE_FROM) {
+    lds_barrier();
+    for (int tau = 0; tau < nticks; ++tau) lds_barrier();
+#endif
   } else {
     const int hid = threadIdx.x - BW;
     constexpr bool vec = VEC;
diff --git a/gtn_amd/csrc/batch.cpp b/gtn_amd/csrc/batch.cpp
--- a/gtn_amd/csrc/batch.cpp
+++ b/gtn_amd/csrc/batch.cpp
@@ -468,6 +468,125 @@
   rt.h2d_pinned(b->rec_mem->ptr, pin->ptr, lab_bytes + arg_bytes);
   launch_ctc_targets(reinterpret_cast<const CtcTargetArgs*>(b->rec_mem->as<char>(lab_bytes)), n, blank, rt.stream());
   return b;
+}
+
+namespace {
+void ctc_step_validate(const void* emissions, const int* labels, const int* lengths, int n, int T, int C, const void* loss,
+                       const void* grad) {
+  if (n <= 0) throw_invalid("[gtnx_batch_ctc_loss_step] the batch size must be positive");
+  if (!emissions || !lengths || !loss || !grad) throw_invalid("[gtnx_batch_ctc_loss_step] null emissions, lengths, loss or gradient");
+  if (T < 1 || C < 1) throw_invalid("[gtnx_batch_ctc_loss_step] T and C must be positive");
+  int64_t total = 0;
+  for (int i = 0; i < n; ++i) {
+    if (lengths[i] < 0) throw_invalid("[gtnx_batch_ctc_loss_step] negative length");
+    total += lengths[i];
+  }
+  if (total > 0 && !labels) throw_invalid("[gtnx_batch_ctc_loss_step] null labels");
+}
+}
+
+bool ctc_step_fused_ok(const int* labels, const int* lengths, int n, int T, int C, int blank, const void* emissions,
+                       const void* grad) {
+  if (n <= 0 || !lengths || !emissions || !grad) return false;
+  if (T < 1 || T > (1 << 20) || C < band_min_labels() || C % 4 != 0) return false;
+  if (blank < 0 || blank >= C) return false;
+  if ((reinterpret_cast<uintptr_t>(emissions) & 15) != 0 || (reinterpret_cast<uintptr_t>(grad) & 15) != 0) return false;
+  int max_len = 0;
+  int64_t total = 0;
+  for (int i = 0; i < n; ++i) {
+    if (lengths[i] < 0) return false;
+    max_len = std::max(max_len, lengths[i]);
+    total += lengths[i];
+  }
+  if (2 * max_len + 1 > 256) return false;
+  if (total > 0 && !labels) return false;
+  for (int64_t i = 0; i < total; ++i)
+    if (labels[i] < 0 || labels[i] >= C) return false;
+  if (total * 3 + 2 * int64_t(n) > (int64_t(1) << 30)) return false;
+  static const size_t pinned_lim = [] {
+    const char* e = std::getenv("GTNX_H2D_KERNEL_BYTES");
+    return e ? size_t(std::atol(e)) : size_t(1) << 20;
+  }();
+  if (align_up(sizeof(int) * 4 * size_t(n), 256) + sizeof(int) * size_t(total ? total : 1) > pinned_lim) return false;
+  return ctc_step_cell(C, band_row_stride(2 * max_len + 1, 1));
+}
+
+void batch_ctc_loss_step(const void* emissions, const int* labels, const int* lengths, int n, int T, int C, int blank,
+                         void* loss, void* grad, bool target_grad, void* target_grad_dev) {
+  GTNX_HOST_T("batch.ctc_loss_step");
+  ctc_step_validate(emissions, labels, lengths, n, T, C, loss, grad);
+  if (!ctc_step_fused_ok(labels, lengths, n, T, C, blank, emissions, grad))
+    throw_invalid("[gtnx_batch_ctc_loss_step] not a batch the one-launch step takes (gtnx_batch_ctc_loss_step_ok)");
+  Runtime& rt = Runtime::get();
+  int max_len = 0;
+  int64_t total = 0;
+  for (int i = 0; i < n; ++i) {
+    max_len = std::max(max_len, lengths[i]);
+    total += lengths[i];
+  }
+  const int max_n = 2 * max_len + 1, max_ns = band_row_stride(max_n, 1);
+  const size_t ent_bytes = align_up(sizeof(int) * 4 * size_t(n), 256);
+  PinnedMemP pin = rt.alloc_pinned(ent_bytes + sizeof(int) * size_t(total ? total : 1));
+  int* ent = pin->as<int>();
+  int* lab = pin->as<int>(ent_bytes);
+  if (total) std::memcpy(lab, labels, sizeof(int) * size_t(total));
+  int64_t lab_off = 0, arcs = 0;
+  double bytes = 0;
+  for (int i = 0; i < n; ++i) {
+    const int U = lengths[i], N = 2 * U + 1;
+    int64_t a = int64_t(N) + (N - 1);
+    for (int u = 1; u < U; ++u) a += labels[lab_off + u] != labels[lab_off + u - 1] ? 1 : 0;
+    ent[4 * i + 0] = int(lab_off);
+    ent[4 * i + 1] = U;
+    ent[4 * i + 2] = T;
+    ent[4 * i + 3] = int(arcs);
+    bytes += 12.0 * T * C + 8.0 * double(T + 1) * band_row_stride(N, 1) + (target_grad ? 4.0 * double(a) : 0.0);
+    lab_off += U;
+    arcs += a;
+  }
+  const size_t aoff_stride = align_up(4 * size_t(T) + 16, 32);
+  const size_t alpha_stride = align_up(size_t(T + 1) * size_t(max_ns), 64);
+  const size_t o_flags = align_up(sizeof(BandNode) * size_t(max_n), 64), o_snode = o_flags + align_up(size_t(max_n), 64),
+               o_slab = o_snode + align_up(4 * size_t(max_n), 64), rec_stride = o_slab + align_up(4 * size_t(max_n), 64);
+  size_t at = 0;
+  auto take = [&](size_t b) {
+    const size_t o = at;
+    at = align_up(at + b, 256);
+    return o;
+  };
+  const size_t o_score = take(4 * size_t(n)), o_norm = take(4 * size_t(n)), o_lse = take(4 * size_t(n) * size_t(T)),
+               o_aoff = take(8 * size_t(n) * aoff_stride), o_alpha = take(4 * size_t(n) * alpha_stride),
+               o_rec = take(size_t(n) * rec_stride),
+               o_tg = take(target_grad && !target_grad_dev ? 4 * size_t(arcs ? arcs : 1) : 0);
+  DevMemP arena = rt.alloc(at);
+  CtcStepDesc d{};
+  d.stage = ent;
+  d.labels = lab;
+  d.em = static_cast<const float*>(emissions);
+  d.grad = static_cast<float*>(grad);
+  d.loss = static_cast<float*>(loss);
+  d.tgrad = target_grad ? (target_grad_dev ? static_cast<float*>(target_grad_dev) : arena->as<float>(o_tg)) : nullptr;
+  d.rec = arena->as<char>(o_rec);
+  d.alpha = arena->as<float>(o_alpha);
+  d.aoff = arena->as<double>(o_aoff);
+  d.rowlse = arena->as<float>(o_lse);
+  d.score = arena->as<float>(o_score);
+  d.norm = arena->as<float>(o_norm);
+  d.em_stride = int64_t(T) * C;
+  d.rec_stride = int64_t(rec_stride);
+  d.alpha_stride = int64_t(alpha_stride);
+  d.aoff_stride = int64_t(aoff_stride);
+  d.o_flags = int(o_flags);
+  d.o_snode = int(o_snode);
+  d.o_slab = int(o_slab);
+  d.T = T;
+  d.C = C;
+  d.blank = blank;
+  d.lgrn = band_forward_lgrn(C);
+  {
+    GTNX_PROF("band_forward_score_grad", bytes);
+    launch_ctc_step(d, n, max_ns, target_grad, rt.stream());
+  }
 }
 
 
diff --git a/gtn_amd/csrc/batch.h b/gtn_amd/csrc/batch.h
--- a/gtn_amd/csrc/batch.h
+++ b/gtn_amd/csrc/batch.h
@@ -78,6 +78,10 @@
 
 BatchP batch_from_graphs(std::vector<Graph> gs);
 BatchP batch_ctc_targets(const int* labels, const int* lengths, int n, int blank, bool calc_grad);
+bool ctc_step_fused_ok(const int* labels, const int* lengths, int n, int T, int C, int blank, const void* emissions,
+                       const void* grad);
+void batch_ctc_loss_step(const void* emissions, const int* labels, const int* lengths, int n, int T, int C, int blank,
+                         void* loss, void* grad, bool target_grad, void* target_grad_dev);
 BatchP batch_asg_force_align(const int* labels, const int* lengths, int n, Graph& transitions, int n_labels);
 BatchP batch_linear(int n, int M, int C, bool calc_grad, const void* dev, bool borrow, const int* rows = nullptr);
 BatchP batch_compose(const BatchP& a, const BatchP& b, bool intersect);
diff --git a/gtn_amd/csrc/capi.cpp b/gtn_amd/csrc/capi.cpp
--- a/gtn_amd/csrc/capi.cpp
+++ b/gtn_amd/csrc/capi.cpp
@@ -769,6 +769,20 @@
                                               gtnx_batch_t* out) {
   return guard([&] { *out = HB(batch_ctc_targets(labels, lengths, n, blank, cg != 0)); });
 }
+GTNX_API gtnx_status_t gtnx_batch_ctc_loss_step(const void* emissions, const int* labels, const int* lengths, int n, int T,
+                                                int C, int blank, void* loss, void* grad, int target_grad,
+                                                void* target_grad_dev) {
+  return guard([&] {
+    batch_ctc_loss_step(emissions, labels, lengths, n, T, C, blank, loss, grad, target_grad != 0, target_grad_dev);
+  });
+}
+GTNX_API gtnx_status_t gtnx_batch_ctc_loss_step_ok(const int* labels, const int* lengths, int n, int T, int C, int blank,
+                                                   const void* emissions, const void* grad, int* ok) {
+  return guard([&] {
+    if (!ok) throw_invalid("[gtnx_batch_ctc_loss_step_ok] null result pointer");
+    *ok = ctc_step_fused_ok(labels, lengths, n, T, C, blank, emissions, grad) ? 1 : 0;
+  });
+}
 GTNX_API gtnx_status_t gtnx_batch_asg_force_align(const int* labels, const int* lengths, int n, gtnx_graph_t transitions,
                                                   int n_labels, gtnx_batch_t* out) {
   return guard([&] { *out = HB(batch_asg_force_align(labels, lengths, n, G(transitions), n_labels)); });
diff --git a/gtn_amd/csrc/ctc_step.hip b/gtn_amd/csrc/ctc_step.hip
--- /dev/null
+++ b/gtn_amd/csrc/ctc_step.hip
@@ -0,0 +1,175 @@
+#include <hip/hip_runtime.h>
+
+#include <algorithm>
+#include <atomic>
+#include <stdexcept>
+#include <type_traits>
+
+#include "kernels.h"
+
+namespace gtnx {
+namespace {
+
+#include "band_device.inc"
+
+__device__ float g_ctc_step_seeds[2] = {-1.0f, 1.0f};
+
+__device__ __forceinline__ BandPair step_pair(const CtcStepDesc& d, int b, const gtnx_i4 e) {
+  BandPair P;
+  const int U = e.y, N = 2 * U + 1;
+  GTNX_G char* rec = reinterpret_cast<GTNX_G char*>(d.rec) + int64_t(b) * d.rec_stride;
+  P.nodes = reinterpret_cast<const GTNX_G BandNode*>(rec);
+  P.nflags = reinterpret_cast<const GTNX_G uint8_t*>(rec + d.o_flags);
+  P.snode = reinterpret_cast<const GTNX_G int*>(rec + d.o_snode);
+  P.slab = reinterpret_cast<const GTNX_G int*>(rec + d.o_slab);
+  P.w = nullptr;
+  P.em = reinterpret_cast<const GTNX_G float*>(d.em) + int64_t(b) * d.em_stride;
+  P.em_copy = nullptr;
+  P.alpha = reinterpret_cast<GTNX_G float*>(d.alpha) + int64_t(b) * d.alpha_stride;
+  P.aoff = reinterpret_cast<GTNX_G double*>(d.aoff) + int64_t(b) * d.aoff_stride;
+  P.score = reinterpret_cast<GTNX_G float*>(d.score) + b;
+  P.rowlse = reinterpret_cast<GTNX_G float*>(d.rowlse) + int64_t(b) * d.T;
+  P.norm = reinterpret_cast<GTNX_G float*>(d.norm) + b;
+  P.delta = (const GTNX_G float*)g_ctc_step_seeds;
+  P.delta_norm = (const GTNX_G float*)(g_ctc_step_seeds + 1);
+  P.grad_em = reinterpret_cast<GTNX_G float*>(d.grad) + int64_t(b) * d.em_stride;
+  P.grad_fixed = d.tgrad ? reinterpret_cast<GTNX_G float*>(d.tgrad) + e.w : nullptr;
+  P.N = N;
+  P.T = e.z;
+  P.C = d.C;
+  P.NS = (N + 3) & ~3;
+  P.hot = U + 1 >= 8 ? d.blank : -1;
+  P.lgrn = d.lgrn;
+  P.n_lab = N;
+  P.bidx = b;
+  P.goff = e.w;
+  return P;
+}
+
+__device__ __forceinline__ BandPair uniform_pair(const BandPair& s) {
+  constexpr int NW = int(sizeof(BandPair) / 4);
+  static_assert(sizeof(BandPair) % 4 == 0, "a pair is whole words");
+  const int* src = reinterpret_cast<const int*>(&s);
+  int w[NW];
+#pragma unroll
+  for (int i = 0; i < NW; ++i) w[i] = __builtin_amdgcn_readfirstlane(src[i]);
+  BandPair P;
+  __builtin_memcpy(&P, w, sizeof(BandPair));
+  return P;
+}
+
+struct StepShared {
+  BandPair pair;
+  GTNX_G float* loss;
+  int lab_off, nsb;
+};
+
+template <bool GRADG_, int KF, int KB>
+__global__ __launch_bounds__(WGB, 6) void band_backward_kernel_step(CtcStepDesc d, int NSf, int NSb, int tail) {
+  constexpr int NPL = 1;
+  constexpr bool UNIT = true, VEC = true, BIG = false, GRADG = GRADG_;
+  extern __shared__ float lds_all[];
+  StepShared& S = *reinterpret_cast<StepShared*>(lds_all + tail);
+  {
+    extern __shared__ float lds[];
+    if (threadIdx.x == 0) {
+      const int b = blockIdx.x;
+      const gtnx_i4 e = reinterpret_cast<const GTNX_G gtnx_i4*>(d.stage)[b];
+      S.pair = step_pair(d, b, e);
+      S.lab_off = e.x;
+      S.loss = d.loss + b;
+      S.nsb = NSb;
+    }
+    __syncthreads();
+    const BandPair P = uniform_pair(S.pair);
+    CtcTargetArgs a;
+    a.labels = reinterpret_cast<const GTNX_G int*>(d.labels) + __builtin_amdgcn_readfirstlane(S.lab_off);
+    a.nodes = const_cast<GTNX_G BandNode*>(P.nodes);
+    a.nflags = const_cast<GTNX_G uint8_t*>(P.nflags);
+    a.snode = const_cast<GTNX_G int*>(P.snode);
+    a.slab = const_cast<GTNX_G int*>(P.slab);
+    a.n_arcs = nullptr;
+    a.N = P.N;
+    a.pad = 0;
+    int* tl = reinterpret_cast<int*>(lds);
+    ctc_target_records(a, d.blank, tl, tl + 264);
+  }
+  __builtin_amdgcn_fence(__ATOMIC_RELEASE, "workgroup");
+  __syncthreads();
+  __builtin_amdgcn_fence(__ATOMIC_ACQUIRE, "workgroup");
+  {
+    constexpr int K = KF;
+    const int NSmax = NSf;
+#define GTNX_BAND_PAIR uniform_pair(S.pair)
+#define GTNX_FWD_IDLE_FROM 8
+#include "band_forward_body.inc"
+#undef GTNX_FWD_IDLE_FROM
+#undef GTNX_BAND_PAIR
+  }
+  __builtin_amdgcn_fence(__ATOMIC_RELEASE, "workgroup");
+  __syncthreads();
+  __builtin_amdgcn_fence(__ATOMIC_ACQUIRE, "workgroup");
+  if (threadIdx.x == 0) {
+    const float nrm = S.pair.norm[0], sc = S.pair.score[0];
+    S.loss[0] = nrm - sc;
+  }
+  {
+    constexpr int K = KB;
+    const int NSmax = __builtin_amdgcn_readfirstlane(S.nsb);
+#define GTNX_BAND_PAIR uniform_pair(S.pair)
+#define GTNX_BWD_RS4_LEAN 1
+#include "band_backward_body.inc"
+#undef GTNX_BWD_RS4_LEAN
+#undef GTNX_BAND_PAIR
+  }
+}
+
+constexpr size_t LDS_TWO = 78 * 1024;
+
+template <bool GRADG, int KF, int KB>
+void launch_step3(const CtcStepDesc& d, int n, int nsf, int nsb, size_t lds, int tail, hipStream_t st) {
+  static std::atomic<uint64_t> done{0};
+  if (gtnx_first_on_device first{done})
+    (void)hipFuncSetAttribute(reinterpret_cast<const void*>(band_backward_kernel_step<GRADG, KF, KB>),
+                              hipFuncAttributeMaxDynamicSharedMemorySize, 160 * 1024 - 512);
+  hipLaunchKernelGGL((band_backward_kernel_step<GRADG, KF, KB>), dim3(n), dim3(WGB), lds, st, d, nsf, nsb, tail);
+}
+template <int KF, int KB>
+void launch_step2(const CtcStepDesc& d, int n, int nsf, int nsb, size_t lds, int tail, bool gradg, hipStream_t st) {
+  if (gradg) launch_step3<true, KF, KB>(d, n, nsf, nsb, lds, tail, st);
+  else launch_step3<false, KF, KB>(d, n, nsf, nsb, lds, tail, st);
+}
+
+struct StepCell {
+  int kf, kb, nsb;
+  int tail;
+  size_t lds;
+};
+StepCell step_cell(int C, int max_NS) {
+  StepCell c{0, 0, 0, 0, 0};
+  if (C < band_min_labels() || C % 4 != 0 || max_NS <= 0 || max_NS > 256) return c;
+  const int kf = band_block_rows(C, 0, false), kb = band_block_rows(C, max_NS, true);
+  if (kb == 0 || kf == 0 || kb * C > 1024 || kb * max_NS > 1024) return c;
+  if (!((kf == 8 && kb == 4) || (kf == 8 && kb == 2) || (kf == 4 && kb == 2))) return c;
+  const int nsb = kb == 4 ? (max_NS + 15) / 16 * 16 : max_NS;
+  const int tail = ((std::max(band_lds(C, kf, max_NS, false).total, band_lds(C, kb, nsb, true).total) + 3) & ~3) + 16;
+  const size_t lds = 4 * size_t(tail) + sizeof(StepShared) + 64;
+  if (lds > LDS_TWO) return c;
+  c = StepCell{kf, kb, nsb, tail, lds};
+  return c;
+}
+
+}
+
+bool ctc_step_cell(int C, int max_NS) { return step_cell(C, max_NS).kf != 0; }
+
+void launch_ctc_step(const CtcStepDesc& d, int n, int max_NS, bool gradg, hipStream_t st) {
+  if (n <= 0) return;
+  const StepCell c = step_cell(d.C, max_NS);
+  if (c.kf == 0) throw std::logic_error("ctc_step.hip: no cell for this shape");
+  if (c.kf == 8 && c.kb == 4) launch_step2<8, 4>(d, n, max_NS, c.nsb, c.lds, c.tail, gradg, st);
+  else if (c.kf == 8) launch_step2<8, 2>(d, n, max_NS, c.nsb, c.lds, c.tail, gradg, st);
+  else launch_step2<4, 2>(d, n, max_NS, c.nsb, c.lds, c.tail, gradg, st);
+}
+
+}
diff --git a/gtn_amd/csrc/kernels.h b/gtn_amd/csrc/kernels.h
--- a/gtn_amd/csrc/kernels.h
+++ b/gtn_amd/csrc/kernels.h
@@ -498,6 +498,26 @@
   int N, pad;
 };
 void launch_ctc_targets(const CtcTargetArgs* d_args, int n, int blank, hipStream_t st);
+struct CtcStepDesc {
+  const GTNX_G int* stage;
+  const GTNX_G int* labels;
+  const GTNX_G float* em;
+  GTNX_G float* grad;
+  GTNX_G float* loss;
+  GTNX_G float* tgrad;
+  GTNX_G char* rec;
+  GTNX_G float* alpha;
+  GTNX_G double* aoff;
+  GTNX_G float* rowlse;
+  GTNX_G float* score;
+  GTNX_G float* norm;
+  int64_t em_stride, rec_stride, alpha_stride, aoff_stride;
+  int o_flags, o_snode, o_slab;
+  int T, C, blank, lgrn;
+};
+int band_block_rows(int C, int max_NS, bool backward);
+bool ctc_step_cell(int C, int max_NS);
+void launch_ctc_step(const CtcStepDesc& d, int n, int max_NS, bool gradg, hipStream_t st);
 struct AsgFalArgs {
   const GTNX_G int* labels;
   const GTNX_G float* trans_w;
diff --git a/include/gtn/batch.h b/include/gtn/batch.h
--- a/include/gtn/batch.h
+++ b/include/gtn/batch.h
@@ -266,6 +266,17 @@
                                            outStride, frameTokensDevice, frameStride));
 }
 inline void backward(const Batch& a, bool retainGraph = false) { detail::check(gtnx_batch_backward(a.handle(), retainGraph)); }
-}
-
-}
+inline bool ctcLossStepOk(const int* labels, const int* lengths, int n, int T, int C, int blank, const void* emissionsDevice,
+                          const void* gradDevice) {
+  int ok = 0;
+  detail::check(gtnx_batch_ctc_loss_step_ok(labels, lengths, n, T, C, blank, emissionsDevice, gradDevice, &ok));
+  return ok != 0;
+}
+inline void ctcLossStep(const void* emissionsDevice, const int* labels, const int* lengths, int n, int T, int C, int blank,
+                        void* lossDevice, void* gradDevice, bool targetGrad = true, void* targetGradDevice = nullptr) {
+  detail::check(gtnx_batch_ctc_loss_step(emissionsDevice, labels, lengths, n, T, C, blank, lossDevice, gradDevice,
+                                         targetGrad ? 1 : 0, targetGradDevice));
+}
+}
+
+}
diff --git a/include/gtn_amd.h b/include/gtn_amd.h
--- a/include/gtn_amd.h
+++ b/include/gtn_amd.h
@@ -133,6 +133,10 @@
 gtnx_status_t gtnx_batch_from_graphs(const gtnx_graph_t* g, int n, gtnx_batch_t* out);
 gtnx_status_t gtnx_batch_ctc_targets(const int* labels, const int* lengths, int n, int blank, int calc_grad,
                                      gtnx_batch_t* out);
+gtnx_status_t gtnx_batch_ctc_loss_step(const void* emissions, const int* labels, const int* lengths, int n, int T, int C,
+                                       int blank, void* loss, void* grad, int target_grad, void* target_grad_dev);
+gtnx_status_t gtnx_batch_ctc_loss_step_ok(const int* labels, const int* lengths, int n, int T, int C, int blank,
+                                          const void* emissions, const void* grad, int* ok);
 gtnx_status_t gtnx_batch_asg_force_align(const int* labels, const int* lengths, int n, gtnx_graph_t transitions,
                                          int n_labels, gtnx_batch_t* out);
 gtnx_status_t gtnx_batch_linear(int n, int M, int N, int calc_grad, const void* device_weights, int borrow,
```

Measured after the change: 1.009 million losses/s, median of 6. 1.08x the previous value.
